# PengjieRen/CaSE_RG

Measured on AMD Instinct MI355X. Metric: train tokens/sec (query+passage) CaSE model, higher is better.
Workload: dtype bf16; 1 GPU; CaSE train step fwd+bwd+allreduce+clip+Adam+EMA, d_model=512, 6 encoder layers, 10 passages x 384 tok, query 64, answer 40, vocab 30522, per-GPU batch 32, dropout on; global_batch=32, parallelism=dp1

## Files before the change

case_rg_amd/_abi.py:

```python
import ctypes as C
import os

import torch

_HERE = os.path.dirname(os.path.abspath(__file__))
LIB_PATH = os.environ.get("CASE_HIP_LIB") or os.path.join(_HERE, "csrc", "libcase_hip.so")

ABI_VERSION = 600
F32, BF16 = 0, 1
WS_ATTENTION_SPLITKV, WS_ATTENTION_BWD, WS_OPTIM_SUMSQ, WS_ENCODER_CHAIN_PACK, WS_GEMM_DW_SLABS = 1, 2, 3, 4, 5
(FEAT_GEMM_256, FEAT_GEMM_SMALL, FEAT_ENCODER_CHAIN, FEAT_ATTN_SCORES, FEAT_ATTN_DECODE, FEAT_OPTIM, FEAT_ATTN_RESIDENT, FEAT_RESERVED_CUS,
 FEAT_GEMM_DW_SLABS, FEAT_DECODER_CHAIN, FEAT_ATTN_DECODE_MQA, FEAT_POINTER_DECODE, FEAT_POINTER_HEAD, FEAT_GEMM_LN, FEAT_STEP_STATE,
 FEAT_INTERACTION, FEAT_ATTN_DECODE_APPEND, FEAT_LINEAR_SKINNY, FEAT_BEAM_DECODE, FEAT_SAMPLE_DECODE, FEAT_POINTER_SCORE, FEAT_CONSENSUS, FEAT_NGRAM_BAN,
 FEAT_NGRAM_COUNTS, FEAT_RANK_METRICS, FEAT_POINTER_HEAD_WIDE, FEAT_DECODE_RULES, FEAT_TOKEN_LABELS) = (1 << i for i in range(28))
EPI_BIAS_COL, EPI_BIAS_ROW, EPI_GELU, EPI_RELU = 1, 2, 4, 8
EPI_RESIDUAL, EPI_MUL_DGELU, EPI_MUL_DRELU, EPI_ATOMIC, EPI_DROPOUT = 16, 32, 64, 128, 256

i32, i64, u64, f32, f64, ptr = C.c_int32, C.c_int64, C.c_uint64, C.c_float, C.c_double, C.c_void_p


class GemmDesc(C.Structure):
    _fields_ = [(n, i64) for n in ("M", "N", "K", "lda", "ldb", "ldc", "ld_aux", "batch1", "batch2",
                                   "sa1", "sa2", "sb1", "sb2", "sc1", "sc2", "saux1", "saux2")] + \
               [(n, i32) for n in ("a_kmajor", "b_kmajor", "in_dtype", "out_dtype", "epilogue", "split_k", "tile")] + \
               [("alpha", f32), ("drop_p", f32), ("seed", u64), ("offset", u64), ("state", ptr)]


class StepState(C.Structure):
    _fields_ = [("rng_base", u64), ("step_size", f32), ("bc2_sqrt", f32), ("lr", f32), ("step", i32), ("reserved", u64 * 5)]


class EncoderChainDesc(C.Structure):
    _fields_ = [("rows", i64), ("width", i32), ("variant", i32), ("eps_ln2", f32), ("eps_ln1_next", f32)]


class SoftmaxDesc(C.Structure):
    _fields_ = [("outer", i64), ("inner", i64), ("R", i64), ("C", i64), ("causal", i32), ("in_dtype", i32),
                ("out_dtype", i32), ("drop_p", f32), ("seed", u64), ("offset", u64), ("state", ptr)]


class AttnDesc(C.Structure):
    _fields_ = [(n, i64) for n in ("N", "heads", "Lq", "Lk", "head_dim", "ldq", "ldk", "ldv", "sq", "sk", "sv", "ldo", "so")] + \
               [("causal", i32), ("scale", f32), ("drop_p", f32), ("seed", u64), ("offset", u64), ("state", ptr)]


class InteractionDesc(C.Structure):
    _fields_ = [(n, i64) for n in ("n", "Lp", "Lq", "H", "eq_div")] + [("dtype", i32)]


class AttnProductDesc(C.Structure):
    _fields_ = [(n, i64) for n in ("N", "heads", "M", "Kc", "head_dim", "lda", "sa_seq", "sa_head", "ldb", "sb_seq", "sb_head",
                                   "ldc", "sc_seq", "sc_head")] + [("a_transposed", i32), ("alpha", f32)]


_RULE = [i64, i32, ptr, i32, i64, i64]

SIGNATURES = {
    "case_gemm": [C.POINTER(GemmDesc), ptr, ptr, ptr, ptr, ptr, ptr, ptr, ptr],
    "case_gemm_dw_bias": [C.POINTER(GemmDesc), ptr, ptr, ptr, ptr, ptr],
    "case_gemm_dw_slabs": [C.POINTER(GemmDesc), ptr, ptr, ptr, ptr, ptr, i64, ptr],
    "case_embed_pos_fwd": [ptr, ptr, ptr, ptr, i64, i64, i64, i64, f32, f32, u64, u64, ptr, i32, ptr],
    "case_embed_pos_bwd": [ptr, ptr, ptr, i64, i64, i64, f32, f32, u64, u64, ptr, i32, ptr],
    "case_scale_add_rows": [ptr, ptr, ptr, i64, i64, i64, f32, i32, ptr],
    "case_layernorm_fwd": [ptr, ptr, ptr, ptr, ptr, ptr, ptr, i64, i64, f32, i32, ptr],
    "case_layernorm_bwd": [ptr, ptr, ptr, ptr, ptr, ptr, ptr, ptr, ptr, ptr, i64, i64, i32, ptr],
    "case_layernorm_bwd_dropout": [ptr, ptr, ptr, ptr, ptr, ptr, ptr, ptr, ptr, i64, i64, f32, u64, u64, ptr, i32, ptr],
    "case_layernorm_bwd_concat5": [ptr] * 15 + [i64, i64, i32, ptr],
    "case_softmax_fwd": [C.POINTER(SoftmaxDesc), ptr, ptr, ptr, ptr, ptr, ptr],
    "case_softmax_bwd": [C.POINTER(SoftmaxDesc), ptr, ptr, ptr, ptr],
    "case_attention_supported": [i64],
    "case_attention_fwd": [C.POINTER(AttnDesc), ptr, ptr, ptr, ptr, ptr, ptr, ptr],
    "case_attention_splitkv_workspace": [C.POINTER(AttnDesc), i32, C.POINTER(i64)],
    "case_attention_fwd_splitkv": [C.POINTER(AttnDesc), ptr, ptr, ptr, ptr, ptr, ptr, ptr, i64, i32, ptr],
    "case_attention_bwd_supported": [i64],
    "case_attention_decode_supported": [i64],
    "case_attention_decode": [C.POINTER(AttnDesc), ptr, ptr, ptr, ptr, ptr, ptr],
    "case_attention_decode_append": [C.POINTER(AttnDesc), ptr, ptr, ptr, ptr, ptr, i64, i64, ptr, ptr, ptr],
    "case_attention_bwd": [C.POINTER(AttnDesc), ptr, ptr, ptr, ptr, ptr, ptr, ptr, ptr, ptr, ptr, ptr, ptr],
    "case_attention_scores_supported": [C.POINTER(AttnDesc)],
    "case_attention_scores_fwd": [C.POINTER(AttnDesc), ptr, ptr, ptr, ptr, ptr, ptr],
    "case_attention_scores_bwd": [C.POINTER(AttnDesc), ptr, ptr, ptr, ptr, ptr],
    "case_attention_product_supported": [C.POINTER(AttnProductDesc)],
    "case_attention_product": [C.POINTER(AttnProductDesc), ptr, ptr, ptr, ptr],
    "case_add": [ptr, ptr, ptr, i64, i32, ptr],
    "case_add_n": [C.POINTER(ptr), i32, ptr, i64, i32, ptr],
    "case_dropout": [ptr, ptr, i64, f32, u64, u64, ptr, i32, ptr],
    "case_mask_rows": [ptr, ptr, ptr, i64, i64, i32, ptr],
    "case_colsum": [ptr, ptr, i64, i64, i32, ptr],
    "case_cast": [ptr, ptr, i64, i32, i32, ptr],
    "case_scale_cols": [ptr, ptr, ptr, i64, i64, i32, ptr],
    "case_scale_cols_bwd": [ptr, ptr, ptr, ptr, ptr, i64, i64, i32, ptr],
    "case_rowdot_fwd": [ptr, ptr, ptr, ptr, i64, i64, i32, ptr],
    "case_linear_skinny": [ptr, ptr, i32, ptr, ptr, ptr, i64, i32, i32, ptr],
    "case_rowdot_bwd": [ptr, ptr, ptr, ptr, ptr, ptr, i64, i64, i32, ptr],
    "case_masked_mean_fwd": [ptr, ptr, ptr, i64, i64, i64, i32, ptr],
    "case_masked_mean_bwd": [ptr, ptr, ptr, i64, i64, i64, i32, ptr],
    "case_highway_gate_fwd": [ptr, ptr, i64, i64, i32, ptr],
    "case_highway_gate_bwd": [ptr, ptr, ptr, i64, i64, i32, ptr],
    "case_concat5_fwd": [ptr, ptr, ptr, ptr, ptr, i64, i64, i32, ptr],
    "case_concat5_bwd": [ptr, ptr, ptr, ptr, ptr, ptr, ptr, ptr, i64, i64, i32, ptr],
    "case_max_over_p_fwd": [ptr, ptr, ptr, i64, i64, i64, i32, ptr],
    "case_max_over_p_bwd": [ptr, ptr, ptr, i64, i64, i64, i32, ptr],
    "case_additive_scores_fwd": [ptr, ptr, ptr, ptr, i64, i64, i64, i64, i32, ptr],
    "case_additive_scores_bwd": [ptr, ptr, ptr, ptr, ptr, ptr, ptr, i64, i64, i64, i64, i32, ptr],
    "case_copy_scatter_fwd": [ptr, ptr, ptr, i64, i64, i64, i64, ptr],
    "case_copy_scatter_bwd": [ptr, ptr, ptr, i64, i64, i64, i64, ptr],
    "case_source_sort": [ptr, ptr, i64, i64, i64, ptr],
    "case_copy_scatter_sorted_fwd": [ptr, ptr, ptr, i64, i64, i64, i64, ptr],
    "case_nll_gather_fwd": [ptr, ptr, ptr, i64, i64, ptr],
    "case_nll_gather_bwd": [ptr, ptr, ptr, ptr, i64, i64, ptr],
    "case_row_argmax": [ptr, ptr, ptr, i64, i64, i64, ptr],
    "case_sentence_compact": [ptr, ptr, ptr, i64, i64, i64, i64, i64, ptr],
    "case_encoder_chain_pack": [ptr, ptr, ptr, ptr, ptr, ptr],
    "case_encoder_chain": [C.POINTER(EncoderChainDesc)] + [ptr] * 14,
    "case_set_reserved_cus": [i32],
    "case_attention_decode_mqa": [ptr, ptr, ptr, ptr, i64, i64, i64, i32, ptr, i64, ptr],
    "case_additive_key_exp": [ptr, ptr, i64, ptr],
    "case_pointer_attend_decode": [ptr] * 11 + [i64, i64, i64, ptr],
    "case_pointer_head_decode": [ptr] * 5 + [i32] + [ptr] * 4 + [i64, i64, i64, ptr],
    "case_pointer_head_beam": [ptr] * 5 + [i32] + [ptr] * 4 + [i64, i64, i64, i32, ptr],
    "case_pointer_head_sample": [ptr] * 5 + [i32] + [ptr] * 7 + [i64, i64, i64, f32, i32, f32, u64, u64, ptr, i64, i64, i64, i32, i32, ptr],
    "case_pointer_head_decode_wide": [ptr] * 5 + [i32] + [ptr] * 4 + [i64, i64, i64, ptr, i64, ptr, i64, i64, i32, i64, ptr],
    "case_pointer_head_beam_wide": [ptr] * 5 + [i32] + [ptr] * 4 + [i64, i64, i64, i32, ptr, i64, ptr, i64, i64, i32, i64, ptr],
    "case_pointer_head_sample_wide": [ptr] * 5 + [i32] + [ptr] * 7 + [i64, i64, i64, f32, i32, f32, u64, u64, ptr, i64, i64, i64, i32, i32,
                                      ptr, i64, ptr, i64, i64, i32, ptr],
    "case_pointer_head_score": [ptr] * 3 + [i64, ptr, ptr, i32, ptr, i64, ptr, ptr, i64, i64, i64, ptr],
    "case_beam_advance": [ptr] * 12 + [i64, i64, i64, i32, i64, ptr],
    "case_pointer_head_decode_ban": [ptr] * 5 + [i32] + [ptr] * 4 + [i64, i64, i64, ptr, i64, i64, i32, i64, ptr],
    "case_pointer_head_beam_ban": [ptr] * 5 + [i32] + [ptr] * 4 + [i64, i64, i64, i32, ptr, i64, i64, i32, i64, ptr],
    "case_pointer_head_sample_ban": [ptr] * 5 + [i32] + [ptr] * 7 + [i64, i64, i64, f32, i32, f32, u64, u64, ptr, i64, i64, i64, i32, i32,
                                     ptr, i64, i64, i32, ptr],
    "case_beam_advance_ban": [ptr] * 12 + [i64, i64, i64, i32, i64, ptr, ptr, i64, ptr],
    "case_ngram_ban": [ptr, ptr, ptr, i64, i64, i64, i64, i32, i64, ptr],
    "case_remove_duplicate_ids": [ptr, ptr, i64, i64, i32, i64, ptr],
    "case_pointer_head_decode_rules": [ptr] * 5 + [i32] + [ptr] * 4 + [i64, i64, i64, ptr, i64, i64, i32, i64] + _RULE + [ptr],
    "case_pointer_head_beam_rules": [ptr] * 5 + [i32] + [ptr] * 4 + [i64, i64, i64, i32, ptr, i64, i64, i32, i64] + _RULE + [ptr],
    "case_pointer_head_sample_rules": [ptr] * 5 + [i32] + [ptr] * 7 + [i64, i64, i64, f32, i32, f32, u64, u64, ptr, i64, i64, i64, i32, i32,
                                       ptr, i64, i64, i32] + _RULE + [ptr],
    "case_pointer_head_decode_wide_rules": [ptr] * 5 + [i32] + [ptr] * 4 + [i64, i64, i64, ptr, i64, ptr, i64, i64, i32, i64] + _RULE + [ptr],
    "case_pointer_head_beam_wide_rules": [ptr] * 5 + [i32] + [ptr] * 4 + [i64, i64, i64, i32, ptr, i64, ptr, i64, i64, i32, i64] + _RULE + [ptr],
    "case_pointer_head_sample_wide_rules": [ptr] * 5 + [i32] + [ptr] * 7 + [i64, i64, i64, f32, i32, f32, u64, u64, ptr, i64, i64, i64, i32, i32,
                                            ptr, i64, ptr, i64, i64, i32] + _RULE + [ptr],
    "case_row_rules": [ptr, ptr, i64, i64, i64] + _RULE + [ptr],
    "case_beam_advance_rules": [ptr] * 12 + [i64, i64, i64, i32, i64, ptr, ptr, i64, f32, ptr],
    "case_beam_gather": [ptr, ptr, i32, ptr, ptr, ptr, i64, i32, i64, i64, i64, ptr],
    "case_beam_backtrack": [ptr] * 8 + [i64, i32, i64, ptr],
    "case_lcs_pairs": [ptr] * 6 + [i64, i64, i64, i64, i64, ptr],
    "case_consensus_pick": [ptr] * 7 + [i64, i64, i64, ptr],
    "case_ngram_counts": [ptr] * 9 + [i64, i64, i64, i64, i64, i32, ptr],
    "case_bleu_scores": [ptr] * 7 + [i64, i64, i64, i32, i32, ptr],
    "case_rank_metrics": [ptr] * 8 + [i64, i64, i64, ptr],
    "case_token_labels": [ptr, ptr, ptr, i32, ptr, ptr, i64, i64, i64, i64, i64, i64, ptr],
    "case_token_select": [ptr] * 7 + [i64, i64, i32, ptr],
    "case_gemm_ln": [C.POINTER(GemmDesc), ptr, ptr, ptr, f32, ptr, ptr, ptr, ptr, ptr, ptr],
    "case_optim_sumsq": [ptr, ptr, i64, ptr, ptr, ptr],
    "case_optim_adam_ema": [ptr, ptr, i64, ptr, f32, f64, f64, f64, f64, ptr, ptr],
    "case_step_advance": [ptr, u64, f64, f64, ptr],
    "case_interaction_supported": [C.POINTER(InteractionDesc)],
    "case_interaction_fwd": [C.POINTER(InteractionDesc), ptr, ptr, ptr, ptr, ptr, ptr, ptr, ptr, ptr, ptr],
}


def _load():
    if not os.path.exists(LIB_PATH):
        raise ImportError(
            "case_rg_amd: %s is missing. Build it with `python -c 'import __graft_entry__ as g; g.build()'` "
            "(or `make -C case_rg_amd/csrc`). There is no CPU or eager fallback." % LIB_PATH)
    lib = C.CDLL(LIB_PATH)
    lib.case_version.restype = C.c_int
    if lib.case_version() != ABI_VERSION:
        raise ImportError("case_rg_amd: %s is ABI generation %d, this package binds %d -- rebuild it (make -C case_rg_amd/csrc)"
                          % (LIB_PATH, lib.case_version(), ABI_VERSION))
    for name, args in SIGNATURES.items():
        fn = getattr(lib, name)
        fn.argtypes = args
        fn.restype = C.c_int
    lib.case_optim_chunk_elems.restype = C.c_int
    lib.case_optim_chunk_elems.argtypes = []
    lib.case_encoder_chain_packed_bytes.restype = C.c_int64
    lib.case_encoder_chain_packed_bytes.argtypes = []
    lib.case_attention_bwd_scratch_floats.restype = C.c_int64
    lib.case_attention_bwd_scratch_floats.argtypes = [C.POINTER(AttnDesc)]
    lib.case_attention_decode_mqa_workspace.restype = C.c_int64
    lib.case_attention_decode_mqa_workspace.argtypes = [i64, i64, i32]
    lib.case_attention_decode_mqa_splits.restype = C.c_int32
    lib.case_attention_decode_mqa_splits.argtypes = [i64, i64]
    lib.case_abi_features.restype = C.c_uint32
# ... 30 lines not shown
```

case_rg_amd/csrc/api.hip:

```cpp
#include <stdarg.h>
#include <stdio.h>
#include <stdlib.h>

#include "common.h"

static thread_local char g_err[512] = "";

int case_set_error(int code, const char* fmt, ...) {
  va_list ap;
  va_start(ap, fmt);
  vsnprintf(g_err, sizeof(g_err), fmt, ap);
  va_end(ap);
  return code;
}

int case_check_launch(const char* what) {
  const hipError_t e = hipGetLastError();
  if (e == hipSuccess) return CASE_OK;
  return case_set_error(CASE_E_LAUNCH, "%s: %s", what, hipGetErrorString(e));
}

extern "C" int case_version(void) { return CASE_ABI_VERSION; }
extern "C" uint32_t case_abi_features(void) {
  return CASE_FEAT_GEMM_256 | CASE_FEAT_GEMM_SMALL | CASE_FEAT_ENCODER_CHAIN | CASE_FEAT_ATTN_SCORES | CASE_FEAT_ATTN_DECODE | CASE_FEAT_OPTIM |
         CASE_FEAT_ATTN_RESIDENT | CASE_FEAT_RESERVED_CUS | CASE_FEAT_GEMM_DW_SLABS | CASE_FEAT_ATTN_DECODE_MQA | CASE_FEAT_POINTER_DECODE | CASE_FEAT_POINTER_HEAD | CASE_FEAT_GEMM_LN | CASE_FEAT_STEP_STATE | CASE_FEAT_INTERACTION | CASE_FEAT_ATTN_DECODE_APPEND | CASE_FEAT_LINEAR_SKINNY |
         CASE_FEAT_BEAM_DECODE | CASE_FEAT_SAMPLE_DECODE | CASE_FEAT_POINTER_SCORE | CASE_FEAT_CONSENSUS | CASE_FEAT_NGRAM_BAN | CASE_FEAT_NGRAM_COUNTS | CASE_FEAT_RANK_METRICS | CASE_FEAT_POINTER_HEAD_WIDE |
         CASE_FEAT_DECODE_RULES | CASE_FEAT_TOKEN_LABELS;
}
extern "C" const char* case_last_error(void) { return g_err; }

static int g_reserved_cus = [] {
  const char* e = getenv("CASE_RESERVE_CUS");
  return e ? atoi(e) : 0;
}();
extern "C" int case_set_reserved_cus(int n) {
  if (n < 0 || n > 128) return case_set_error(CASE_E_ARG, "case_set_reserved_cus: %d out of range (0 .. 128)", n);
  g_reserved_cus = n;
  return CASE_OK;
}
extern "C" int case_get_reserved_cus(void) { return g_reserved_cus; }
int case_device_cus() {
  static int cus = 0;
  if (!cus) {
    int dev = 0, n = 0;
    (void)hipGetDevice(&dev);
    (void)hipDeviceGetAttribute(&n, hipDeviceAttributeMultiprocessorCount, dev);
    cus = n > 0 ? n : 256;
  }
  return cus;
}
int case_persistent_cus() {
  int c = case_device_cus() - g_reserved_cus;
  c = c / 8 * 8;
  return c > 8 ? c : 8;
}
extern "C" int case_sizeof_opt_tensor(void) { return (int)sizeof(CaseOptTensor); }
```

case_rg_amd/csrc/attn_pointer.hip:

```cpp
#include "common.h"

namespace {

template <bool FAST>
__device__ __forceinline__ float tanh_t(float x) {
  if constexpr (FAST) {
    const float e = __expf(2.f * x);
    return 1.f - __fdividef(2.f, e + 1.f);
  } else {
    return tanhf(x);
  }
}

constexpr float TANH_PRESCALE = 2.8853900817779268f;
constexpr float EXP2_CLAMP = 62.f;
__device__ __forceinline__ float exp2_factor(float xs) { return __builtin_amdgcn_exp2f(fminf(fmaxf(xs, -EXP2_CLAMP), EXP2_CLAMP)); }
__device__ __forceinline__ float half_sigmoid_prod(float ew, float eu) { return __builtin_amdgcn_rcpf(fmaf(ew, eu, 1.f)); }

constexpr int AJ = 64;
constexpr int AH = 64;
constexpr int ATW = 8;

template <typename T, bool FAST>
__global__ __launch_bounds__(256) void additive_fwd_kernel(const float* __restrict__ wq, const T* __restrict__ uh,
                                                           const float* __restrict__ v, float* __restrict__ s, int64_t Tn,
                                                           int64_t S, int64_t H) {
  __shared__ float U[AJ][AH + 1];
  __shared__ float W[4 * ATW][AH];
  __shared__ float V[AH];
  const int64_t b = blockIdx.y, j0 = (int64_t)blockIdx.x * AJ;
  const int lane = threadIdx.x & 63, wave = threadIdx.x >> 6;
  for (int64_t tc = (int64_t)blockIdx.z * 4 * ATW; tc < Tn; tc += (int64_t)gridDim.z * 4 * ATW) {
    constexpr float PS = FAST ? TANH_PRESCALE : 1.f;
    float acc[ATW];
#pragma unroll
    for (int i = 0; i < ATW; ++i) acc[i] = 0.f;
    float vsum = 0.f;
    for (int64_t hc = 0; hc < H; hc += AH) {
      __syncthreads();
      for (int e = threadIdx.x; e < AJ * AH; e += 256) {
        const int jj = e / AH, hh = e % AH;
        const int64_t j = j0 + jj, h = hc + hh;
        const float uv = (j < S && h < H) ? PS * Elem<T>::ld(uh + (b * S + j) * H + h) : 0.f;
        U[jj][hh] = FAST ? exp2_factor(uv) : uv;
      }
      for (int e = threadIdx.x; e < 4 * ATW * AH; e += 256) {
        const int tt = e / AH, hh = e % AH;
        const int64_t t = tc + tt, h = hc + hh;
        const float wv = (t < Tn && h < H) ? PS * wq[(b * Tn + t) * H + h] : 0.f;
        W[tt][hh] = FAST ? exp2_factor(wv) : wv;
      }
      if (threadIdx.x < AH) V[threadIdx.x] = (hc + threadIdx.x < H) ? v[hc + threadIdx.x] : 0.f;
      __syncthreads();
#pragma unroll 4
      for (int hh = 0; hh < AH; ++hh) {
        const float u = U[lane][hh], vv = V[hh];
        if constexpr (FAST) {
          vsum += vv;
#pragma unroll
          for (int i = 0; i < ATW; ++i) acc[i] += vv * half_sigmoid_prod(W[wave * ATW + i][hh], u);
        } else {
#pragma unroll
          for (int i = 0; i < ATW; ++i) acc[i] += vv * tanh_t<FAST>(W[wave * ATW + i][hh] + u);
        }
      }
    }
    const int64_t j = j0 + lane;
    if (j < S) {
#pragma unroll
      for (int i = 0; i < ATW; ++i) {
        const int64_t t = tc + wave * ATW + i;
        if (t < Tn) s[(b * Tn + t) * S + j] = FAST ? vsum - 2.f * acc[i] : acc[i];
      }
    }
  }
}

template <typename T, bool FAST, int TT, int NCH>
__global__ __launch_bounds__(256) void additive_fwd_rowwise_kernel(const float* __restrict__ wq, const T* __restrict__ uh,
                                                                   const float* __restrict__ v, float* __restrict__ s,
                                                                   int64_t Tn, int64_t S, int64_t H) {
  constexpr int E = Vec16<T>::N;
  const int64_t b = blockIdx.y;
  const int lane = threadIdx.x & 63;
  const int64_t wave = (int64_t)blockIdx.x * 4 + (threadIdx.x >> 6), nwaves = (int64_t)gridDim.x * 4;
  float wreg[NCH][TT][E], vreg[NCH][E];
#pragma unroll
  for (int c = 0; c < NCH; ++c) {
    const int64_t h0 = ((int64_t)c * 64 + lane) * E;
#pragma unroll
    for (int e = 0; e < E; ++e) {
      vreg[c][e] = h0 < H ? v[h0 + e] : 0.f;
#pragma unroll
      for (int t = 0; t < TT; ++t) wreg[c][t][e] = (h0 < H && t < Tn) ? wq[(b * Tn + t) * H + h0 + e] : 0.f;
    }
  }
  for (int64_t j = wave; j < S; j += nwaves) {
    float acc[TT];
#pragma unroll
    for (int t = 0; t < TT; ++t) acc[t] = 0.f;
#pragma unroll
    for (int c = 0; c < NCH; ++c) {
      const int64_t h0 = ((int64_t)c * 64 + lane) * E;
      if (h0 < H) {
        float u[E];
        Vec16<T>::load(uh + (b * S + j) * H + h0, u);
#pragma unroll
        for (int e = 0; e < E; ++e)
#pragma unroll
          for (int t = 0; t < TT; ++t) acc[t] += vreg[c][e] * tanh_t<FAST>(wreg[c][t][e] + u[e]);
      }
    }
#pragma unroll
    for (int t = 0; t < TT; ++t) {
      const float r = wave_sum(acc[t]);
      if (lane == 0 && t < Tn) s[(b * Tn + t) * S + j] = r;
    }
  }
}

constexpr int BJ = 16;
constexpr int BTC = 32;

template <typename T, bool FAST>
__global__ __launch_bounds__(256) void additive_bwd_uh_kernel(const float* __restrict__ ds, const float* __restrict__ wq,
                                                              const T* __restrict__ uh, const float* __restrict__ v,
                                                              float* __restrict__ d_uh, float* __restrict__ d_v, int64_t Tn,
                                                              int64_t S, int64_t H) {
  __shared__ float DS[BTC][BJ];
  const int64_t b = blockIdx.z, j0 = (int64_t)blockIdx.x * BJ, h = (int64_t)blockIdx.y * 256 + threadIdx.x;
  const bool h_ok = h < H;
  float u[BJ], acc[BJ];
#pragma unroll
  for (int jj = 0; jj < BJ; ++jj) {
    const int64_t j = j0 + jj;
    u[jj] = (h_ok && j < S) ? (FAST ? TANH_PRESCALE : 1.f) * Elem<T>::ld(uh + (b * S + j) * H + h) : 0.f;
    if constexpr (FAST) u[jj] = exp2_factor(u[jj]);
    acc[jj] = 0.f;
  }
  float dv = 0.f, gsum = 0.f;
  for (int64_t tc = 0; tc < Tn; tc += BTC) {
    __syncthreads();
    for (int e = threadIdx.x; e < BTC * BJ; e += 256) {
      const int tt = e / BJ, jj = e % BJ;
      const int64_t t = tc + tt, j = j0 + jj;
      DS[tt][jj] = (t < Tn && j < S) ? ds[(b * Tn + t) * S + j] : 0.f;
    }
    __syncthreads();
    const int tmax = (int)((Tn - tc) < BTC ? (Tn - tc) : BTC);
    for (int tt = 0; tt < tmax; ++tt) {
      float w = h_ok ? (FAST ? TANH_PRESCALE : 1.f) * wq[(b * Tn + tc + tt) * H + h] : 0.f;
      if constexpr (FAST) w = exp2_factor(w);
#pragma unroll
      for (int jj = 0; jj < BJ; ++jj) {
        const float g = DS[tt][jj];
        if constexpr (FAST) {
          const float r = half_sigmoid_prod(w, u[jj]);
          const float gr = g * r;
          acc[jj] += gr - gr * r;
          dv += gr;
          gsum += g;
        } else {
          const float th = tanh_t<FAST>(w + u[jj]);
          acc[jj] += g * (1.f - th * th);
          dv += g * th;
        }
      }
    }
  }
  if (h_ok) {
    const float vh = FAST ? 4.f * v[h] : v[h];
#pragma unroll
    for (int jj = 0; jj < BJ; ++jj) {
      const int64_t j = j0 + jj;
      if (j < S) d_uh[(b * S + j) * H + h] = vh * acc[jj];
    }
    atomicAdd(d_v + h, FAST ? gsum - 2.f * dv : dv);
  }
}

constexpr int CT = 8;
constexpr int CJC = 64;

template <typename T, bool FAST>
__global__ __launch_bounds__(256) void additive_bwd_wq_kernel(const float* __restrict__ ds, const float* __restrict__ wq,
                                                              const T* __restrict__ uh, const float* __restrict__ v,
                                                              float* __restrict__ d_wq, int64_t Tn, int64_t S, int64_t H,
                                                              int tblocks, int64_t j_per) {
  __shared__ float DS[CT][CJC];
  const int64_t b = blockIdx.z, t0 = (int64_t)(blockIdx.x % tblocks) * CT, h = (int64_t)blockIdx.y * 256 + threadIdx.x;
  const int64_t j_begin = (int64_t)(blockIdx.x / tblocks) * j_per, j_end = (j_begin + j_per < S) ? j_begin + j_per : S;
  const bool split = j_per < S;
  const bool h_ok = h < H;
  float w[CT], acc[CT];
#pragma unroll
  for (int tt = 0; tt < CT; ++tt) {
    const int64_t t = t0 + tt;
    w[tt] = (h_ok && t < Tn) ? (FAST ? TANH_PRESCALE : 1.f) * wq[(b * Tn + t) * H + h] : 0.f;
    if constexpr (FAST) w[tt] = exp2_factor(w[tt]);
    acc[tt] = 0.f;
  }
  for (int64_t jc = j_begin; jc < j_end; jc += CJC) {
    __syncthreads();
    for (int e = threadIdx.x; e < CT * CJC; e += 256) {
      const int tt = e / CJC, jj = e % CJC;
      const int64_t t = t0 + tt, j = jc + jj;
      DS[tt][jj] = (t < Tn && j < j_end) ? ds[(b * Tn + t) * S + j] : 0.f;
    }
    __syncthreads();
    const int jmax = (int)((j_end - jc) < CJC ? (j_end - jc) : CJC);
    for (int jj = 0; jj < jmax; ++jj) {
      float u = h_ok ? (FAST ? TANH_PRESCALE : 1.f) * Elem<T>::ld(uh + (b * S + jc + jj) * H + h) : 0.f;
      if constexpr (FAST) u = exp2_factor(u);
#pragma unroll
      for (int tt = 0; tt < CT; ++tt) {
        if constexpr (FAST) {
          const float r = half_sigmoid_prod(w[tt], u);
          const float gr = DS[tt][jj] * r;
          acc[tt] += gr - gr * r;
        } else {
          const float th = tanh_t<FAST>(w[tt] + u);
          acc[tt] += DS[tt][jj] * (1.f - th * th);
        }
      }
    }
  }
  if (h_ok) {
    const float vh = FAST ? 4.f * v[h] : v[h];
#pragma unroll
    for (int tt = 0; tt < CT; ++tt) {
      const int64_t t = t0 + tt;
      if (t < Tn) {
        if (split) atomicAdd(d_wq + (b * Tn + t) * H + h, vh * acc[tt]);
        else d_wq[(b * Tn + t) * H + h] = vh * acc[tt];
      }
    }
  }
}

constexpr float EXP_CLAMP = 43.f;
constexpr int PA_WAVES = 16, PA_H = 512;

__global__ __launch_bounds__(256) void additive_key_exp_kernel(const float* __restrict__ uh, bf16_t* __restrict__ eu, int64_t n8) {
  for (int64_t i = (int64_t)blockIdx.x * 256 + threadIdx.x; i < n8; i += (int64_t)gridDim.x * 256) {
    const float4 a = reinterpret_cast<const float4*>(uh)[2 * i], b = reinterpret_cast<const float4*>(uh)[2 * i + 1];
    const float x[8] = {a.x, a.y, a.z, a.w, b.x, b.y, b.z, b.w};
    float y[8];
#pragma unroll
    for (int e = 0; e < 8; ++e) y[e] = __expf(fminf(fmaxf(2.f * x[e], -EXP_CLAMP), EXP_CLAMP));
    Vec16<bf16_t>::store(eu + 8 * i, y);
  }
}

__device__ __forceinline__ float row_sum4(float r0, float r1, float r2, float r3) {
  const auto a = __builtin_amdgcn_permlane32_swap(__float_as_uint(r0), __float_as_uint(r2), false, false);
  const auto b = __builtin_amdgcn_permlane32_swap(__float_as_uint(r1), __float_as_uint(r3), false, false);
  const float A = __uint_as_float(a[0]) + __uint_as_float(a[1]);
  const float B = __uint_as_float(b[0]) + __uint_as_float(b[1]);
  const auto c = __builtin_amdgcn_permlane16_swap(__float_as_uint(A), __float_as_uint(B), false, false);
  float t = __uint_as_float(c[0]) + __uint_as_float(c[1]);
  t += __uint_as_float(__builtin_amdgcn_update_dpp(0, __float_as_uint(t), 0x128, 0xf, 0xf, false));
  t += __uint_as_float(__builtin_amdgcn_update_dpp(0, __float_as_uint(t), 0x124, 0xf, 0xf, false));
  t += __uint_as_float(__builtin_amdgcn_update_dpp(0, __float_as_uint(t), 0x122, 0xf, 0xf, false));
  t += __uint_as_float(__builtin_amdgcn_update_dpp(0, __float_as_uint(t), 0x121, 0xf, 0xf, false));
  return t;
}

#ifndef CASE_STREAM_DEFAULT_POLICY
typedef unsigned int pa_u32x4 __attribute__((ext_vector_type(4)));
__device__ __forceinline__ uint4 pa_nt_load(const void* p) {
  const pa_u32x4 v = __builtin_nontemporal_load(reinterpret_cast<const pa_u32x4*>(p));
  return make_uint4(v[0], v[1], v[2], v[3]);
}
#define PA_STREAM_LOAD(P) pa_nt_load(P)
#else
#define PA_STREAM_LOAD(P) (*reinterpret_cast<const uint4*>(P))
#endif
__global__ __launch_bounds__(64 * PA_WAVES) void pointer_attend_decode_kernel(
    const float* __restrict__ wq, const float* __restrict__ wq_add, const bf16_t* __restrict__ eu, const float* __restrict__ v, const bf16_t* __restrict__ mem,
    const uint8_t* __restrict__ col_valid, const uint8_t* __restrict__ row_valid, const float* __restrict__ prior, bf16_t* __restrict__ ctx,
    float* __restrict__ p_out, float* __restrict__ copy_out, const int64_t S) {
  extern __shared__ __attribute__((aligned(16))) float pa_smem[];
  float* sc = pa_smem;
  float* red = pa_smem + ((S + 3) & ~(int64_t)3);
  const int lane = threadIdx.x & 63, wave = threadIdx.x >> 6;
  const int64_t b = blockIdx.x;
  const uint8_t* cv = col_valid ? col_valid + b * S : nullptr;
  const bool row_ok = row_valid ? row_valid[b] != 0 : true;
  float ew[8], vv[8];
  {
    float w8[8];
    Vec16<float>::load(wq + b * PA_H + 8 * lane, *reinterpret_cast<float(*)[4]>(w8));
    Vec16<float>::load(wq + b * PA_H + 8 * lane + 4, *reinterpret_cast<float(*)[4]>(w8 + 4));
    if (wq_add) {
      float c8[8];
      Vec16<float>::load(wq_add + b * PA_H + 8 * lane, *reinterpret_cast<float(*)[4]>(c8));
      Vec16<float>::load(wq_add + b * PA_H + 8 * lane + 4, *reinterpret_cast<float(*)[4]>(c8 + 4));
#pragma unroll
      for (int e = 0; e < 8; ++e) w8[e] += c8[e];
    }
    Vec16<float>::load(v + 8 * lane, *reinterpret_cast<float(*)[4]>(vv));
    Vec16<float>::load(v + 8 * lane + 4, *reinterpret_cast<float(*)[4]>(vv + 4));
#pragma unroll
    for (int e = 0; e < 8; ++e) ew[e] = __expf(fminf(fmaxf(2.f * w8[e], -EXP_CLAMP), EXP_CLAMP));
  }
  float vs = 0.f;
#pragma unroll
  for (int e = 0; e < 8; ++e) vs += vv[e];
  vs = wave_sum(vs);
  const bf16_t* eub = eu + b * S * PA_H + 8 * lane;
  uint4 raw[4], nxt[4];
  bool ok[4], nok[4];
#define PA_LOAD(R, OK, J0)                                                     \
  _Pragma("unroll") for (int u = 0; u < 4; ++u) {                              \
    const int64_t j = (J0) + u * PA_WAVES;                                     \
    OK[u] = j < S && (!cv || cv[j]);                         \
    if (OK[u]) R[u] = PA_STREAM_LOAD(eub + j * PA_H);                          \
  }
  PA_LOAD(raw, ok, (int64_t)wave)
// ... 895 lines not shown
    __threadfence_block();
    __syncthreads();
  }
}

__global__ void nll_fwd_kernel(const float* __restrict__ dist, const int64_t* __restrict__ target,
                               float* __restrict__ per_row, int64_t rows, int64_t V) {
  for (int64_t r = (int64_t)blockIdx.x * blockDim.x + threadIdx.x; r < rows; r += (int64_t)gridDim.x * blockDim.x) {
    const int64_t y = target[r];
    per_row[r] = (y > 0 && y < V) ? -logf(dist[r * V + y] + 1e-8f) : 0.f;
  }
}

__global__ void nll_bwd_kernel(const float* __restrict__ dist, const int64_t* __restrict__ target,
                               const float* __restrict__ g_row, float* __restrict__ d_dist, int64_t rows, int64_t V) {
  for (int64_t r = (int64_t)blockIdx.x * blockDim.x + threadIdx.x; r < rows; r += (int64_t)gridDim.x * blockDim.x) {
    const int64_t y = target[r];
    if (y > 0 && y < V) d_dist[r * V + y] = -g_row[r] / (dist[r * V + y] + 1e-8f);
  }
}

__global__ __launch_bounds__(256) void row_argmax_kernel(const float* __restrict__ x, int64_t* __restrict__ idx,
                                                         float* __restrict__ val, int64_t rows, int64_t cols, int64_t ld) {
  __shared__ float sv[4];
  __shared__ int64_t si[4];
  for (int64_t r = blockIdx.x; r < rows; r += gridDim.x) {
    float best = -INFINITY;
    int64_t bi = cols;
    for (int64_t c = threadIdx.x; c < cols; c += 256) {
      const float vv = x[r * ld + c];
      if (vv > best || (vv == best && c < bi)) {
        best = vv;
        bi = c;
      }
    }
#pragma unroll
    for (int o = 32; o > 0; o >>= 1) {
      const float ob = __shfl_xor(best, o, 64);
      const int64_t oi = __shfl_xor(bi, o, 64);
      if (ob > best || (ob == best && oi < bi)) {
        best = ob;
        bi = oi;
      }
    }
    __syncthreads();
    if ((threadIdx.x & 63) == 0) {
      sv[threadIdx.x >> 6] = best;
      si[threadIdx.x >> 6] = bi;
    }
    __syncthreads();
    if (threadIdx.x == 0) {
      for (int w = 1; w < 4; ++w)
        if (sv[w] > best || (sv[w] == best && si[w] < bi)) {
          best = sv[w];
          bi = si[w];
        }
      idx[r] = bi < cols ? bi : 0;
      if (val) val[r] = best;
    }
  }
}

}

extern "C" int case_additive_scores_fwd(const float* wq, const void* uh, const float* v, float* s, int64_t B, int64_t T,
                                        int64_t S, int64_t H, int32_t dtype, case_stream_t stream) {
  CASE_REQUIRE(wq && uh && v && s && B > 0 && T > 0 && S > 0 && H > 0 && B < 65536, "case_additive_scores_fwd: bad argument");
  hipStream_t st = (hipStream_t)stream;
  const int ev = dtype == CASE_F32 ? 4 : 8;
  if (T <= 2 && H % ev == 0 && H <= 2 * 64 * ev && (uintptr_t)uh % 16 == 0) {
    const dim3 g((unsigned)((S + 15) / 16 < 64 ? (S + 15) / 16 : 64), (unsigned)B);
    const bool one = H <= 64 * ev;
#define ROWWISE(TY, FAST, TT, NCH) hipLaunchKernelGGL((additive_fwd_rowwise_kernel<TY, FAST, TT, NCH>), g, dim3(256), 0, st, wq, (const TY*)uh, v, s, T, S, H)
    if (dtype == CASE_F32) {
      if (T == 1) { if (one) ROWWISE(float, false, 1, 1); else ROWWISE(float, false, 1, 2); }
      else { if (one) ROWWISE(float, false, 2, 1); else ROWWISE(float, false, 2, 2); }
    } else {
      if (T == 1) { if (one) ROWWISE(bf16_t, true, 1, 1); else ROWWISE(bf16_t, true, 1, 2); }
      else { if (one) ROWWISE(bf16_t, true, 2, 1); else ROWWISE(bf16_t, true, 2, 2); }
    }
#undef ROWWISE
    return case_check_launch("case_additive_scores_fwd");
  }
  const int64_t jb = (S + AJ - 1) / AJ, tchunks = (T + 4 * ATW - 1) / (4 * ATW);
  const dim3 grid((unsigned)jb, (unsigned)B, (unsigned)(jb * B < 512 ? tchunks : 1));
  if (dtype == CASE_F32)
    hipLaunchKernelGGL((additive_fwd_kernel<float, false>), grid, dim3(256), 0, st, wq, (const float*)uh, v, s, T, S, H);
  else
    hipLaunchKernelGGL((additive_fwd_kernel<bf16_t, true>), grid, dim3(256), 0, st, wq, (const bf16_t*)uh, v, s, T, S, H);
  return case_check_launch("case_additive_scores_fwd");
}

extern "C" int case_additive_scores_bwd(const float* ds, const float* wq, const void* uh, const float* v, float* d_wq,
                                        float* d_uh, float* d_v, int64_t B, int64_t T, int64_t S, int64_t H, int32_t dtype,
                                        case_stream_t stream) {
  CASE_REQUIRE(ds && wq && uh && v && d_wq && d_uh && d_v && B > 0 && T > 0 && S > 0 && H > 0 && B < 65536,
               "case_additive_scores_bwd: bad argument");
  const unsigned hb = (unsigned)((H + 255) / 256);
  const int tblocks = (int)((T + CT - 1) / CT);
  const int64_t base_wgs = (int64_t)tblocks * hb * B, j_chunks = (S + CJC - 1) / CJC;
  int64_t sch = base_wgs >= 2048 ? 1 : (2048 + base_wgs - 1) / base_wgs;
  if (sch > j_chunks) sch = j_chunks;
  const int64_t j_per = ((j_chunks + sch - 1) / sch) * CJC;
  sch = (S + j_per - 1) / j_per;
  const dim3 g1((unsigned)((S + BJ - 1) / BJ), hb, (unsigned)B), g2((unsigned)(tblocks * sch), hb, (unsigned)B);
  hipStream_t st = (hipStream_t)stream;
  if (sch > 1 && hipMemsetAsync(d_wq, 0, (size_t)(B * T * H) * sizeof(float), st) != hipSuccess)
    return case_set_error(CASE_E_LAUNCH, "case_additive_scores_bwd: hipMemsetAsync failed");
  if (dtype == CASE_F32) {
    hipLaunchKernelGGL((additive_bwd_uh_kernel<float, false>), g1, dim3(256), 0, st, ds, wq, (const float*)uh, v, d_uh, d_v, T, S, H);
    hipLaunchKernelGGL((additive_bwd_wq_kernel<float, false>), g2, dim3(256), 0, st, ds, wq, (const float*)uh, v, d_wq, T, S, H, tblocks, j_per);
  } else {
    hipLaunchKernelGGL((additive_bwd_uh_kernel<bf16_t, true>), g1, dim3(256), 0, st, ds, wq, (const bf16_t*)uh, v, d_uh, d_v, T, S, H);
    hipLaunchKernelGGL((additive_bwd_wq_kernel<bf16_t, true>), g2, dim3(256), 0, st, ds, wq, (const bf16_t*)uh, v, d_wq, T, S, H, tblocks, j_per);
  }
  return case_check_launch("case_additive_scores_bwd");
}

extern "C" int case_additive_key_exp(const float* uh, void* eu, int64_t n, case_stream_t stream) {
  CASE_REQUIRE(uh && eu && n > 0 && n % 8 == 0 && (uintptr_t)uh % 16 == 0 && (uintptr_t)eu % 16 == 0, "case_additive_key_exp: bad argument");
  hipLaunchKernelGGL(additive_key_exp_kernel, dim3(grid_for(n / 8, 256, 1, 256 * 32)), dim3(256), 0, (hipStream_t)stream, uh,
                     reinterpret_cast<bf16_t*>(eu), n / 8);
  return case_check_launch("case_additive_key_exp");
}

extern "C" int case_pointer_attend_decode(const float* wq, const float* wq_add, const void* eu, const float* v, const void* value, const uint8_t* col_valid,
                                          const uint8_t* row_valid, const float* prior, void* ctx, float* p, float* copy, int64_t B, int64_t S,
                                          int64_t H, case_stream_t stream) {
  CASE_REQUIRE(wq && eu && v && value && ctx && p && B > 0 && S > 0 && B < (1ll << 31) && (copy != nullptr) == (prior != nullptr),
               "case_pointer_attend_decode: bad argument");
  if (H != PA_H || S > 28000)
    return case_set_error(CASE_E_UNSUPPORTED, "case_pointer_attend_decode: built for H = %d and S <= 28000 (run case_additive_scores_fwd + "
                                              "case_softmax_fwd + case_gemm)", PA_H);
  for (const void* q : {(const void*)wq, (const void*)wq_add, eu, (const void*)v, value})
    CASE_REQUIRE((reinterpret_cast<uintptr_t>(q) & 15) == 0, "case_pointer_attend_decode: tensors must be 16-byte aligned");
  const size_t lds = (size_t)(((S + 3) & ~(int64_t)3) + PA_WAVES * PA_H) * sizeof(float);
  static bool attr = false;
  if (!attr) {
    if (hipFuncSetAttribute(reinterpret_cast<const void*>(&pointer_attend_decode_kernel), hipFuncAttributeMaxDynamicSharedMemorySize, 160 * 1024) !=
        hipSuccess)
      return case_set_error(CASE_E_LAUNCH, "case_pointer_attend_decode: cannot reserve LDS");
    attr = true;
  }
  hipLaunchKernelGGL(pointer_attend_decode_kernel, dim3((unsigned)B), dim3(64 * PA_WAVES), lds, (hipStream_t)stream, wq, wq_add,
                     reinterpret_cast<const bf16_t*>(eu), v, reinterpret_cast<const bf16_t*>(value), col_valid, row_valid, prior,
                     reinterpret_cast<bf16_t*>(ctx), p, copy, S);
  return case_check_launch("case_pointer_attend_decode");
}

template <typename Args>
static int pointer_head_fill(Args& a, const char* who, const float* logits, const float* mix_logits, const uint32_t* keys, const float* const* copies,
                             const int64_t* lens, int32_t nmem, int64_t R, int64_t V, int64_t S, int64_t max_v, const char* instead) {
  CASE_REQUIRE(logits && mix_logits && keys && copies && lens && R > 0 && V > 0 && S > 0 && nmem >= 1 && R < (1ll << 31), "%s: bad argument", who);
  if (nmem > PH_MAX_MEM || V > max_v || S > 32768)
    return case_set_error(CASE_E_UNSUPPORTED, "%s: built for <= %d memories, V <= %lld, S <= 32768%s", who, PH_MAX_MEM, (long long)max_v, instead);
  a.logits = logits;
  a.mix_logits = mix_logits;
  a.keys = keys;
  int64_t total = 0;
  for (int m = 0; m < PH_MAX_MEM; ++m) {
    a.copy[m] = m < nmem ? copies[m] : nullptr;
    a.len[m] = m < nmem ? lens[m] : 0;
    total += a.len[m];
    CASE_REQUIRE(m >= nmem || (copies[m] && lens[m] > 0), "%s: null copy weights", who);
  }
  CASE_REQUIRE(total == S, "%s: the memories hold %lld positions, the source map %lld", who, (long long)total, (long long)S);
  a.V = V;
  a.S = S;
  a.nmem = nmem;
  return CASE_OK;
}

constexpr int64_t PH_MAX_V = 36000, PS_MAX_V = 131071;
constexpr int64_t PW_MAX_DIST_V = 1ll << 24;

static int pointer_head_args(HeadArgs& a, const char* who, const float* logits, const float* mix_logits, const uint32_t* keys,
                             const float* const* copies, const int64_t* lens, int32_t nmem, float* gen, float* dist, int64_t B, int64_t V, int64_t S,
                             bool wide = false) {
  const int rc = pointer_head_fill(a, who, logits, mix_logits, keys, copies, lens, nmem, B, V, S, wide ? PS_MAX_V : PH_MAX_V,
                                   wide ? "" : " (run the softmax / scatter / argmax launches)");
  if (rc != CASE_OK) return rc;
  a.gen = gen;
  a.dist = dist;
  a.ids = nullptr;
  a.top = nullptr;
  a.row_ws = nullptr;
  a.row_stride = 0;
  return CASE_OK;
}

static size_t pointer_head_lds(int64_t V) { return (size_t)(((V + 3) & ~(int64_t)3) + (PH_THREADS + 4) + PH_THREADS + 64) * 4; }

static int pointer_head_workspace(HeadArgs& a, const char* who, float* row_ws, int64_t row_stride, int64_t V) {
  CASE_REQUIRE(row_ws && row_stride >= V && row_stride % 4 == 0 && (reinterpret_cast<uintptr_t>(row_ws) & 15) == 0,
               "%s: the row workspace must be 16-byte aligned f32 [rows, row_stride], row_stride >= V and a multiple of 4", who);
  a.row_ws = row_ws;
  a.row_stride = row_stride;
  return CASE_OK;
}
// ... 550 lines not shown
```

case_rg_amd/csrc/common.h:

```cpp
#pragma once
#include <hip/hip_runtime.h>
#include <stdint.h>

#include "case_hip.h"

typedef unsigned short bf16_t;

int case_set_error(int code, const char* fmt, ...);
int case_check_launch(const char* what);
int case_device_cus();
int case_persistent_cus();

#define CASE_REQUIRE(cond, ...)                          \
  do {                                                   \
    if (!(cond)) return case_set_error(CASE_E_ARG, __VA_ARGS__); \
  } while (0)

__device__ __forceinline__ float bf16_to_f32(bf16_t v) { return __uint_as_float(((uint32_t)v) << 16); }
typedef float case_f32x2 __attribute__((ext_vector_type(2)));
typedef __bf16 case_bf16x2 __attribute__((ext_vector_type(2)));
__device__ __forceinline__ uint32_t f32x2_to_bf16x2(float lo, float hi) {
  const case_f32x2 v = {lo, hi};
  const case_bf16x2 b = __builtin_convertvector(v, case_bf16x2);
  return *reinterpret_cast<const uint32_t*>(&b);
// ... 25 lines not shown
    *reinterpret_cast<float4*>(p) = make_float4(v[0], v[1], v[2], v[3]);
  }
};
template <> struct Vec16<bf16_t> {
  static constexpr int N = 8;
  typedef uint4 raw;
  static __device__ __forceinline__ void unpack(const uint4& t, float (&v)[8]) {
    const uint32_t w[4] = {t.x, t.y, t.z, t.w};
#pragma unroll
    for (int i = 0; i < 4; ++i) {
      v[2 * i] = __uint_as_float(w[i] << 16);
      v[2 * i + 1] = __uint_as_float(w[i] & 0xffff0000u);
    }
  }
#ifdef CASE_VEC16_NT
  static __device__ __forceinline__ void load(const bf16_t* p, float (&v)[8]) {
    typedef unsigned int u32x4_nt __attribute__((ext_vector_type(4)));
    const u32x4_nt t = __builtin_nontemporal_load(reinterpret_cast<const u32x4_nt*>(p));
    unpack(make_uint4(t[0], t[1], t[2], t[3]), v);
  }
#else
  static __device__ __forceinline__ void load(const bf16_t* p, float (&v)[8]) { unpack(*reinterpret_cast<const uint4*>(p), v); }
#endif
  static __device__ __forceinline__ void store(bf16_t* p, const float (&v)[8]) {
    uint32_t w[4];
#pragma unroll
    for (int i = 0; i < 4; ++i) w[i] = f32x2_to_bf16x2(v[2 * i], v[2 * i + 1]);
    *reinterpret_cast<uint4*>(p) = make_uint4(w[0], w[1], w[2], w[3]);
  }
};

template <typename T> struct Vec8;
template <> struct Vec8<bf16_t> {
  static constexpr int N = 4;
  typedef uint2 raw;
  static __device__ __forceinline__ void unpack(const uint2& t, float (&v)[4]) {
    v[0] = __uint_as_float(t.x << 16); v[1] = __uint_as_float(t.x & 0xffff0000u);
    v[2] = __uint_as_float(t.y << 16); v[3] = __uint_as_float(t.y & 0xffff0000u);
  }
  static __device__ __forceinline__ void load(const bf16_t* p, float (&v)[4]) { unpack(*reinterpret_cast<const uint2*>(p), v); }
  static __device__ __forceinline__ void store(bf16_t* p, const float (&v)[4]) {
    *reinterpret_cast<uint2*>(p) = make_uint2(f32x2_to_bf16x2(v[0], v[1]), f32x2_to_bf16x2(v[2], v[3]));
  }
};

__device__ __forceinline__ float wave_sum(float v) {
#pragma unroll
  for (int o = 32; o > 0; o >>= 1) v += __shfl_xor(v, o, 64);
  return v;
}
__device__ __forceinline__ float wave_max(float v) {
#pragma unroll
  for (int o = 32; o > 0; o >>= 1) v = fmaxf(v, __shfl_xor(v, o, 64));
  return v;
}

__device__ __forceinline__ float block_sum(float v, float* red) {
  const int lane = threadIdx.x & 63, w = threadIdx.x >> 6, nw = (blockDim.x + 63) >> 6;
  v = wave_sum(v);
  __syncthreads();
  if (lane == 0) red[w] = v;
  __syncthreads();
  float t = (lane < nw) ? red[lane] : 0.f;
  t = wave_sum(t);
  return t;
}
__device__ __forceinline__ float block_max(float v, float* red) {
  const int lane = threadIdx.x & 63, w = threadIdx.x >> 6, nw = (blockDim.x + 63) >> 6;
  v = wave_max(v);
  __syncthreads();
  if (lane == 0) red[w] = v;
  __syncthreads();
  float t = (lane < nw) ? red[lane] : -INFINITY;
  t = wave_max(t);
  return t;
}

__device__ __forceinline__ uint64_t rng_base_of(const CaseStepState* st) {
  if (st == nullptr) return 0;
  typedef const __attribute__((address_space(4))) uint64_t* const_u64_ptr;
  return *(const_u64_ptr)(uintptr_t)st;
}

__device__ __forceinline__ uint32_t rng_hash(uint64_t seed, uint64_t pair) {
  const uint32_t lo = (uint32_t)pair, hi = (uint32_t)(pair >> 32);
  uint32_t h = lo ^ ((hi << 16) | (hi >> 16)) ^ (uint32_t)seed;
  h *= 0x9E3779B1u;
  h ^= (h >> 15) ^ (uint32_t)(seed >> 32);
  h *= 0x85EBCA77u;
  h ^= h >> 13;
  return h;
}
__device__ __forceinline__ float rng_uniform(uint64_t seed, uint64_t idx) {
  const uint32_t h = rng_hash(seed, idx >> 1);
  return (float)((idx & 1) ? (h >> 16) : (h & 0xffffu)) * (1.0f / 65536.0f);
}
__device__ __forceinline__ void rng_uniform2(uint64_t seed, uint64_t idx_even, float& u0, float& u1) {
  const uint32_t h = rng_hash(seed, idx_even >> 1);
  u0 = (float)(h & 0xffffu) * (1.0f / 65536.0f);
  u1 = (float)(h >> 16) * (1.0f / 65536.0f);
}
__device__ __forceinline__ float rng_uniform24(uint64_t seed, uint64_t counter) {
  return (float)(rng_hash(seed, counter) >> 8) * (1.0f / 16777216.0f);
}
__device__ __forceinline__ void dropout8(float (&x)[8], uint64_t seed, uint64_t idx0, float p, float scale) {
  if ((idx0 & 1) == 0) {
#pragma unroll
    for (int e = 0; e < 8; e += 2) {
      float u0, u1;
      rng_uniform2(seed, idx0 + e, u0, u1);
      x[e] = u0 >= p ? x[e] * scale : 0.f;
      x[e + 1] = u1 >= p ? x[e + 1] * scale : 0.f;
    }
  } else {
#pragma unroll
    for (int e = 0; e < 8; ++e) x[e] = rng_uniform(seed, idx0 + e) >= p ? x[e] * scale : 0.f;
  }
}

constexpr uint32_t RNG_C1 = 0x9E3779B1u, RNG_C2 = 0x85EBCA77u;
__device__ __forceinline__ uint32_t rng_row_key(uint64_t seed, uint64_t offset_plus_row) { return rng_hash(seed, offset_plus_row); }
__device__ __forceinline__ uint32_t rng_pair_bits_pre(uint32_t key, uint32_t jc1) {
  const uint32_t h = (key ^ jc1) * RNG_C2;
  return h ^ (h >> 16);
}
__device__ __forceinline__ uint32_t rng_pair_bits(uint32_t key, uint32_t pair) { return rng_pair_bits_pre(key, pair * RNG_C1); }
__device__ __forceinline__ uint32_t rng_threshold(float p) { return (uint32_t)ceilf(p * 65536.f); }
__device__ __forceinline__ bool attn_keep(uint32_t key, uint32_t col, uint32_t thr) {
  const uint32_t h = rng_pair_bits(key, col >> 1);
  return ((col & 1) ? (h >> 16) : (h & 0xffffu)) >= thr;
}
__device__ __forceinline__ void attn_dropout8(float (&x)[8], uint32_t key, uint32_t c0, uint32_t thr, float scale) {
#pragma unroll
  for (int e = 0; e < 8; e += 2) {
    const uint32_t h = rng_pair_bits(key, (c0 + e) >> 1);
    x[e] = (h & 0xffffu) >= thr ? x[e] * scale : 0.f;
    x[e + 1] = (h >> 16) >= thr ? x[e + 1] * scale : 0.f;
  }
}

struct GeluTerms {
  float cdf, pdf;
};
__device__ __forceinline__ GeluTerms gelu_terms(float x) {
  const float z = fabsf(x) * 0.70710678118654752f;
  const float t = __builtin_amdgcn_rcpf(fmaf(0.3275911f, z, 1.f));
  const float e = __expf(-z * z);
  float p = fmaf(1.061405429f, t, -1.453152027f);
  p = fmaf(p, t, 1.421413741f);
  p = fmaf(p, t, -0.284496736f);
  p = fmaf(p, t, 0.254829592f);
  const float q = 0.5f * p * t * e;
  GeluTerms r;
  r.cdf = x >= 0.f ? 1.f - q : q;
  r.pdf = 0.39894228040143268f * e;
  return r;
}
__device__ __forceinline__ float gelu_f(float x) { return x * gelu_terms(x).cdf; }
__device__ __forceinline__ float dgelu_f(float x) {
  const GeluTerms g = gelu_terms(x);
  return g.cdf + x * g.pdf;
}

static inline int grid_for(int64_t n, int block, int per_thread = 1, int cap = 256 * 8) {
  int64_t g = (n + (int64_t)block * per_thread - 1) / ((int64_t)block * per_thread);
  if (g < 1) g = 1;
  if (g > cap) g = cap;
  return (int)g;
}
```

case_rg_amd/csrc/elementwise.hip:

```cpp
#include "common.h"

namespace {

constexpr int EW_THREADS = 256;

template <typename T>
__global__ void add_kernel(const T* __restrict__ a, const T* __restrict__ b, T* __restrict__ o, int64_t n) {
  for (int64_t i = (int64_t)blockIdx.x * blockDim.x + threadIdx.x; i < n; i += (int64_t)gridDim.x * blockDim.x)
    Elem<T>::st(o + i, Elem<T>::ld(a + i) + Elem<T>::ld(b + i));
}

template <typename T>
__global__ void dropout_kernel(const T* __restrict__ x, T* __restrict__ y, int64_t n, float p, uint64_t seed,
                               uint64_t offset, const CaseStepState* state) {
  offset += rng_base_of(state);
  const float scale = 1.f / (1.f - p);
  for (int64_t i = (int64_t)blockIdx.x * blockDim.x + threadIdx.x; i < n; i += (int64_t)gridDim.x * blockDim.x)
    Elem<T>::st(y + i, rng_uniform(seed, offset + (uint64_t)i) >= p ? Elem<T>::ld(x + i) * scale : 0.f);
}

template <typename T>
__global__ void mask_rows_kernel(const T* __restrict__ x, const uint8_t* __restrict__ valid, T* __restrict__ y,
                                 int64_t rows, int64_t cols) {
  const int64_t n = rows * cols;
  const bool in_place = x == y;
  for (int64_t i = (int64_t)blockIdx.x * blockDim.x + threadIdx.x; i < n; i += (int64_t)gridDim.x * blockDim.x) {
    const bool ok = valid[i / cols] != 0;
    if (in_place) {
      if (!ok) Elem<T>::st(y + i, 0.f);
    } else {
      Elem<T>::st(y + i, ok ? Elem<T>::ld(x + i) : 0.f);
    }
  }
}

template <typename T>
__global__ __launch_bounds__(256) void colsum_kernel(const T* __restrict__ x, float* __restrict__ out, int64_t rows,
                                                     int64_t cols, int row_splits) {
  __shared__ float part[4][64];
  const int cx = threadIdx.x & 63, ry = threadIdx.x >> 6;
  const int64_t col = (int64_t)(blockIdx.x / row_splits) * 64 + cx;
  const int split = blockIdx.x % row_splits;
  float s = 0.f;
  if (col < cols)
    for (int64_t r = (int64_t)split * 4 + ry; r < rows; r += (int64_t)row_splits * 4) s += Elem<T>::ld(x + r * cols + col);
  part[ry][cx] = s;
  __syncthreads();
  if (ry == 0 && col < cols) atomicAdd(out + col, part[0][cx] + part[1][cx] + part[2][cx] + part[3][cx]);
}

template <typename T>
__global__ __launch_bounds__(256) void colsum_vec_kernel(const T* __restrict__ x, float* __restrict__ out, int64_t rows,
                                                         int64_t cols, int row_splits) {
  constexpr int E = Vec16<T>::N;
  __shared__ float part[8][32 * E + 1];
  const int cx = threadIdx.x & 31, ry = threadIdx.x >> 5;
  const int64_t col = ((int64_t)(blockIdx.x / row_splits) * 32 + cx) * E;
  const int split = blockIdx.x % row_splits;
  float s[E];
#pragma unroll
  for (int e = 0; e < E; ++e) s[e] = 0.f;
  if (col < cols)
    for (int64_t r = (int64_t)split * 8 + ry; r < rows; r += (int64_t)row_splits * 8) {
      float v[E];
      Vec16<T>::load(x + r * cols + col, v);
#pragma unroll
      for (int e = 0; e < E; ++e) s[e] += v[e];
    }
#pragma unroll
  for (int e = 0; e < E; ++e) part[ry][cx * E + e] = s[e];
  __syncthreads();
  for (int c = threadIdx.x; c < 32 * E; c += 256) {
    const int64_t gc = (int64_t)(blockIdx.x / row_splits) * 32 * E + c;
    if (gc < cols) {
      float t = 0.f;
#pragma unroll
      for (int r = 0; r < 8; ++r) t += part[r][c];
      atomicAdd(out + gc, t);
    }
  }
}

template <typename T>
__global__ void add_vec_kernel(const T* __restrict__ a, const T* __restrict__ b, T* __restrict__ o, int64_t nvec) {
  constexpr int E = Vec16<T>::N;
  for (int64_t i = (int64_t)blockIdx.x * blockDim.x + threadIdx.x; i < nvec; i += (int64_t)gridDim.x * blockDim.x) {
    float x[E], y[E];
    Vec16<T>::load(a + i * E, x);
    Vec16<T>::load(b + i * E, y);
#pragma unroll
    for (int e = 0; e < E; ++e) x[e] += y[e];
    Vec16<T>::store(o + i * E, x);
  }
}

struct AddNArgs {
  const void* src[8];
  int n;
};
template <typename T>
__global__ void add_n_vec_kernel(const AddNArgs a, T* __restrict__ o, int64_t nvec) {
  constexpr int E = Vec16<T>::N;
  for (int64_t i = (int64_t)blockIdx.x * blockDim.x + threadIdx.x; i < nvec; i += (int64_t)gridDim.x * blockDim.x) {
    float acc[E], y[E];
    Vec16<T>::load(reinterpret_cast<const T*>(a.src[0]) + i * E, acc);
#pragma unroll
    for (int j = 1; j < 8; ++j) {
      if (j < a.n) {
        Vec16<T>::load(reinterpret_cast<const T*>(a.src[j]) + i * E, y);
#pragma unroll
        for (int e = 0; e < E; ++e) acc[e] += y[e];
      }
    }
    Vec16<T>::store(o + i * E, acc);
  }
}

template <typename T>
__global__ void dropout_vec_kernel(const T* __restrict__ x, T* __restrict__ y, int64_t nvec, float p, uint64_t seed,
                                   uint64_t offset, const CaseStepState* state) {
  offset += rng_base_of(state);
  constexpr int E = Vec16<T>::N;
  const float scale = 1.f / (1.f - p);
  for (int64_t i = (int64_t)blockIdx.x * blockDim.x + threadIdx.x; i < nvec; i += (int64_t)gridDim.x * blockDim.x) {
    float v[E];
    Vec16<T>::load(x + i * E, v);
    const uint64_t idx0 = offset + (uint64_t)(i * E);
    if ((idx0 & 1) == 0) {
#pragma unroll
      for (int e = 0; e < E; e += 2) {
        float u0, u1;
        rng_uniform2(seed, idx0 + e, u0, u1);
        v[e] = u0 >= p ? v[e] * scale : 0.f;
        v[e + 1] = u1 >= p ? v[e + 1] * scale : 0.f;
      }
    } else {
#pragma unroll
      for (int e = 0; e < E; ++e) v[e] = rng_uniform(seed, idx0 + e) >= p ? v[e] * scale : 0.f;
    }
    Vec16<T>::store(y + i * E, v);
  }
}

template <typename T>
__global__ void mask_rows_vec_kernel(const T* __restrict__ x, const uint8_t* __restrict__ valid, T* __restrict__ y,
                                     int64_t rows, int64_t cols) {
  constexpr int E = Vec16<T>::N;
  const int64_t vpr = cols / E, nvec = rows * vpr;
  const bool in_place = x == y;
  for (int64_t i = (int64_t)blockIdx.x * blockDim.x + threadIdx.x; i < nvec; i += (int64_t)gridDim.x * blockDim.x) {
    const bool ok = valid[i / vpr] != 0;
    if (in_place && ok) continue;
    float v[E];
    if (ok) Vec16<T>::load(x + i * E, v);
    else {
#pragma unroll
      for (int e = 0; e < E; ++e) v[e] = 0.f;
    }
    Vec16<T>::store(y + i * E, v);
  }
}

template <typename T>
__global__ __launch_bounds__(256) void rowdot_fwd_kernel(const T* __restrict__ x, const float* __restrict__ w,
                                                         const float* __restrict__ b, float* __restrict__ y, int64_t rows,
                                                         int64_t cols) {
  const int lane = threadIdx.x & 63;
  const int64_t wave = (int64_t)blockIdx.x * 4 + (threadIdx.x >> 6), nwaves = (int64_t)gridDim.x * 4;
  for (int64_t r = wave; r < rows; r += nwaves) {
    float acc = 0.f;
    for (int64_t c = lane; c < cols; c += 64) acc += Elem<T>::ld(x + r * cols + c) * w[c];
    acc = wave_sum(acc);
    if (lane == 0) y[r] = acc + (b ? b[0] : 0.f);
  }
}

struct SkinnyArgs {
  const void* x[4];
  int64_t width[4];
  const float* w; const float* b; float* y;
  int64_t rows, cols;
  int nseg, nout;
};
template <typename T, bool VEC>
__global__ __launch_bounds__(256) void linear_skinny_kernel(const SkinnyArgs a) {
  const int lane = threadIdx.x & 63;
  const int64_t wave = (int64_t)blockIdx.x * 4 + (threadIdx.x >> 6), nwaves = (int64_t)gridDim.x * 4;
  constexpr int NV = Vec16<T>::N;
  for (int64_t r = wave; r < a.rows; r += nwaves) {
    float acc[8] = {0.f, 0.f, 0.f, 0.f, 0.f, 0.f, 0.f, 0.f};
    int64_t off = 0;
#pragma unroll
    for (int k = 0; k < 4; ++k) {
      if (k < a.nseg) {
        const T* xr = reinterpret_cast<const T*>(a.x[k]) + r * a.width[k];
        if constexpr (VEC) {
#pragma unroll 2
          for (int64_t c = (int64_t)lane * NV; c < a.width[k]; c += 64 * NV) {
            float xv[NV];
            Vec16<T>::load(xr + c, xv);
#pragma unroll
            for (int o = 0; o < 8; ++o) {
              if (o < a.nout) {
                const float* wr = a.w + o * a.cols + off + c;
#pragma unroll
                for (int q = 0; q < NV / 4; ++q) {
                  const float4 wv = *reinterpret_cast<const float4*>(wr + 4 * q);
                  acc[o] = fmaf(xv[4 * q], wv.x, acc[o]);
                  acc[o] = fmaf(xv[4 * q + 1], wv.y, acc[o]);
                  acc[o] = fmaf(xv[4 * q + 2], wv.z, acc[o]);
                  acc[o] = fmaf(xv[4 * q + 3], wv.w, acc[o]);
                }
              }
            }
          }
        } else {
          for (int64_t c = lane; c < a.width[k]; c += 64) {
            const float xv = Elem<T>::ld(xr + c);
#pragma unroll
            for (int o = 0; o < 8; ++o)
              if (o < a.nout) acc[o] = fmaf(xv, a.w[o * a.cols + off + c], acc[o]);
// ... 24 lines not shown
  float s = 0.f, sb = 0.f;
  if (col < cols) {
    const float wc = w[col];
    for (int64_t r = (int64_t)split * 4 + ry; r < rows; r += (int64_t)row_splits * 4) {
      const float gr = g[r];
      s += gr * Elem<T>::ld(x + r * cols + col);
      sb += gr;
      if (dx) Elem<T>::st(dx + r * cols + col, gr * wc);
    }
  }
  part[ry][cx] = s;
  __syncthreads();
  if (ry == 0 && col < cols) atomicAdd(dw + col, part[0][cx] + part[1][cx] + part[2][cx] + part[3][cx]);
  if (db && col == 0) {
    __syncthreads();
    part[ry][0] = sb;
    __syncthreads();
    if (ry == 0 && cx == 0) atomicAdd(db, part[0][0] + part[1][0] + part[2][0] + part[3][0]);
  }
}

static inline bool al16(const void* p) { return ((uintptr_t)p % 16) == 0; }

template <typename TS, typename TD>
__global__ void cast_kernel(const TS* __restrict__ x, TD* __restrict__ y, int64_t n) {
  for (int64_t i = (int64_t)blockIdx.x * blockDim.x + threadIdx.x; i < n; i += (int64_t)gridDim.x * blockDim.x)
    Elem<TD>::st(y + i, Elem<TS>::ld(x + i));
}

template <typename T>
__global__ void scale_cols_kernel(const T* __restrict__ x, const float* __restrict__ w, T* __restrict__ y, int64_t rows,
                                  int64_t cols) {
  const int64_t n = rows * cols;
  for (int64_t i = (int64_t)blockIdx.x * blockDim.x + threadIdx.x; i < n; i += (int64_t)gridDim.x * blockDim.x)
    Elem<T>::st(y + i, Elem<T>::ld(x + i) * w[i % cols]);
}

template <typename T>
__global__ __launch_bounds__(256) void scale_cols_bwd_kernel(const T* __restrict__ dy, const T* __restrict__ x,
                                                             const float* __restrict__ w, T* __restrict__ dx,
                                                             float* __restrict__ dw, int64_t rows, int64_t cols,
                                                             int row_splits) {
  __shared__ float part[4][64];
  const int cx = threadIdx.x & 63, ry = threadIdx.x >> 6;
  const int64_t col = (int64_t)(blockIdx.x / row_splits) * 64 + cx;
  const int split = blockIdx.x % row_splits;
  float s = 0.f;
  if (col < cols) {
    const float wc = w[col];
    for (int64_t r = (int64_t)split * 4 + ry; r < rows; r += (int64_t)row_splits * 4) {
      const float g = Elem<T>::ld(dy + r * cols + col);
      s += g * Elem<T>::ld(x + r * cols + col);
      Elem<T>::st(dx + r * cols + col, g * wc);
    }
  }
  part[ry][cx] = s;
  __syncthreads();
  if (ry == 0 && col < cols) atomicAdd(dw + col, part[0][cx] + part[1][cx] + part[2][cx] + part[3][cx]);
}

template <typename T>
__global__ void scale_add_rows_kernel(const T* __restrict__ x, const float* __restrict__ pe, T* __restrict__ y,
                                      int64_t rows, int64_t seq_len, int64_t H, float scale) {
  const int64_t n = rows * H;
  for (int64_t i = (int64_t)blockIdx.x * blockDim.x + threadIdx.x; i < n; i += (int64_t)gridDim.x * blockDim.x) {
    const int64_t r = i / H, c = i % H;
    Elem<T>::st(y + i, Elem<T>::ld(x + i) * scale + (pe ? pe[(r % seq_len) * H + c] : 0.f));
  }
}

template <typename T>
__global__ void embed_pos_fwd_kernel(const int64_t* __restrict__ ids, const float* __restrict__ table,
                                     const float* __restrict__ pe, T* __restrict__ out, int64_t rows, int64_t seq_len,
                                     int64_t H, int64_t vocab, float scale, float drop_p, uint64_t seed, uint64_t offset,
                                     const CaseStepState* state) {
  offset += rng_base_of(state);
  const int64_t n = rows * H;
  const float ks = drop_p > 0.f ? 1.f / (1.f - drop_p) : 1.f;
  for (int64_t i = (int64_t)blockIdx.x * blockDim.x + threadIdx.x; i < n; i += (int64_t)gridDim.x * blockDim.x) {
    const int64_t r = i / H, c = i % H;
    int64_t id = ids[r];
    if (id < 0 || id >= vocab) id = 0;
    float v = table[id * H + c] * scale + pe[(r % seq_len) * H + c];
    if (drop_p > 0.f) v = rng_uniform(seed, offset + (uint64_t)i) >= drop_p ? v * ks : 0.f;
    Elem<T>::st(out + i, v);
  }
}

template <typename T>
__global__ __launch_bounds__(256) void embed_pos_fwd_vec_kernel(const int64_t* __restrict__ ids, const float* __restrict__ table,
                                                                const float* __restrict__ pe, T* __restrict__ out, unsigned chunks,
                                                                unsigned seq_len, unsigned H8, int64_t vocab, float scale, float drop_p,
                                                                uint64_t seed, uint64_t offset, const CaseStepState* state) {
  offset += rng_base_of(state);
  const float ks = drop_p > 0.f ? 1.f / (1.f - drop_p) : 1.f;
  for (unsigned ci = blockIdx.x * 256u + threadIdx.x; ci < chunks; ci += gridDim.x * 256u) {
    const unsigned r = ci / H8, c = (ci - r * H8) * 8u;
    int64_t id = ids[r];
    if (id < 0 || id >= vocab) id = 0;
    const float* tp = table + id * (int64_t)(H8 * 8u) + c;
    const float* pp = pe + (int64_t)(r % seq_len) * (H8 * 8u) + c;
    const float4 t0 = *reinterpret_cast<const float4*>(tp), t1 = *reinterpret_cast<const float4*>(tp + 4);
    const float4 p0 = *reinterpret_cast<const float4*>(pp), p1 = *reinterpret_cast<const float4*>(pp + 4);
    float v[8] = {fmaf(t0.x, scale, p0.x), fmaf(t0.y, scale, p0.y), fmaf(t0.z, scale, p0.z), fmaf(t0.w, scale, p0.w),
                  fmaf(t1.x, scale, p1.x), fmaf(t1.y, scale, p1.y), fmaf(t1.z, scale, p1.z), fmaf(t1.w, scale, p1.w)};
    if (drop_p > 0.f) dropout8(v, seed, offset + (uint64_t)r * (H8 * 8u) + c, drop_p, ks);
    T* op = out + (int64_t)r * (H8 * 8u) + c;
    if constexpr (sizeof(T) == 2) {
      uint4 w;
      w.x = f32x2_to_bf16x2(v[0], v[1]); w.y = f32x2_to_bf16x2(v[2], v[3]);
      w.z = f32x2_to_bf16x2(v[4], v[5]); w.w = f32x2_to_bf16x2(v[6], v[7]);
      *reinterpret_cast<uint4*>(op) = w;
    } else {
      *reinterpret_cast<float4*>(op) = make_float4(v[0], v[1], v[2], v[3]);
      *reinterpret_cast<float4*>(op + 4) = make_float4(v[4], v[5], v[6], v[7]);
    }
  }
}

template <typename T>
__global__ void embed_pos_bwd_kernel(const int64_t* __restrict__ ids, const T* __restrict__ d_out,
                                     float* __restrict__ d_table, int64_t rows, int64_t H, int64_t vocab, float scale,
                                     float drop_p, uint64_t seed, uint64_t offset, const CaseStepState* state) {
  offset += rng_base_of(state);
  const int64_t n = rows * H;
  const float ks = drop_p > 0.f ? 1.f / (1.f - drop_p) : 1.f;
  for (int64_t i = (int64_t)blockIdx.x * blockDim.x + threadIdx.x; i < n; i += (int64_t)gridDim.x * blockDim.x) {
    const int64_t r = i / H, c = i % H;
    const int64_t id = ids[r];
    if (id <= 0 || id >= vocab) continue;
    float g = Elem<T>::ld(d_out + i);
    if (drop_p > 0.f) g = rng_uniform(seed, offset + (uint64_t)i) >= drop_p ? g * ks : 0.f;
    atomicAdd(d_table + id * H + c, g * scale);
  }
}

template <typename T>
__global__ void masked_mean_fwd_kernel(const T* __restrict__ x, const uint8_t* __restrict__ valid, T* __restrict__ out,
                                       int64_t n, int64_t L, int64_t H) {
  const int64_t total = n * H;
  for (int64_t i = (int64_t)blockIdx.x * blockDim.x + threadIdx.x; i < total; i += (int64_t)gridDim.x * blockDim.x) {
    const int64_t s = i / H, c = i % H;
    float acc = 0.f, cnt = 0.f;
    for (int64_t l = 0; l < L; ++l)
      if (valid[s * L + l]) {
        acc += Elem<T>::ld(x + (s * L + l) * H + c);
        cnt += 1.f;
      }
    Elem<T>::st(out + i, acc / cnt);
  }
}

template <typename T>
__global__ void masked_mean_bwd_kernel(const T* __restrict__ d_out, const uint8_t* __restrict__ valid,
                                       T* __restrict__ dx, int64_t n, int64_t L, int64_t H) {
  const int64_t total = n * L * H;
  for (int64_t i = (int64_t)blockIdx.x * blockDim.x + threadIdx.x; i < total; i += (int64_t)gridDim.x * blockDim.x) {
    const int64_t c = i % H, sl = i / H, s = sl / L;
    float cnt = 0.f;
    for (int64_t l = 0; l < L; ++l) cnt += valid[s * L + l] ? 1.f : 0.f;
    Elem<T>::st(dx + i, valid[sl] ? Elem<T>::ld(d_out + s * H + c) / cnt : 0.f);
  }
}

template <typename T>
__global__ __launch_bounds__(256) void masked_mean_fwd_vec_kernel(const T* __restrict__ x, const uint8_t* __restrict__ valid,
                                                                  T* __restrict__ out, int64_t L, int64_t H) {
  constexpr int E = Vec16<T>::N;
  __shared__ float part[4][64][E + 1];
  __shared__ float cnts[4];
  const int lane = threadIdx.x & 63, w = threadIdx.x >> 6;
  const int64_t s = blockIdx.x, c0 = ((int64_t)blockIdx.y * 64 + lane) * E;
  const bool in = c0 < H;
  float acc[E];
#pragma unroll
  for (int e = 0; e < E; ++e) acc[e] = 0.f;
  float cnt = 0.f;
  for (int64_t l = w; l < L; l += 4) {
    if (!valid[s * L + l]) continue;
    cnt += 1.f;
    if (in) {
      float v[E];
      Vec16<T>::load(x + (s * L + l) * H + c0, v);
#pragma unroll
      for (int e = 0; e < E; ++e) acc[e] += v[e];
    }
  }
#pragma unroll
  for (int e = 0; e < E; ++e) part[w][lane][e] = acc[e];
  if (lane == 0) cnts[w] = cnt;
  __syncthreads();
  if (w == 0 && in) {
    const float n = cnts[0] + cnts[1] + cnts[2] + cnts[3];
    float v[E];
#pragma unroll
    for (int e = 0; e < E; ++e) v[e] = (part[0][lane][e] + part[1][lane][e] + part[2][lane][e] + part[3][lane][e]) / n;
    Vec16<T>::store(out + s * H + c0, v);
  }
}

template <typename T>
__global__ __launch_bounds__(256) void masked_mean_bwd_vec_kernel(const T* __restrict__ d_out, const uint8_t* __restrict__ valid,
                                                                  T* __restrict__ dx, int64_t L, int64_t H) {
  constexpr int E = Vec16<T>::N;
  __shared__ float red[32];
  const int lane = threadIdx.x & 63, w = threadIdx.x >> 6;
  const int64_t s = blockIdx.x, c0 = ((int64_t)blockIdx.y * 64 + lane) * E;
  float cnt = 0.f;
  for (int64_t l = threadIdx.x; l < L; l += 256) cnt += valid[s * L + l] ? 1.f : 0.f;
  cnt = block_sum(cnt, red);
  if (c0 >= H) return;
  float g[E], z[E];
  Vec16<T>::load(d_out + s * H + c0, g);
#pragma unroll
  for (int e = 0; e < E; ++e) { g[e] /= cnt; z[e] = 0.f; }
// ... 437 lines not shown
```

case_rg_amd/csrc/gemm8w.inc:

```
namespace gemm_t8w {

using gemm_w4::Epilogue;

constexpr int TM = 256, TN = 256, BKE = 64, NTHR = 512;
constexpr int OPB = 32768, STAGE = 2 * OPB, EXTRA = 32768, LDS_BYTES = 2 * STAGE + EXTRA;
constexpr int STRIP = 8192;

#pragma clang diagnostic push
#pragma clang diagnostic ignored "-Winline-asm"
typedef __attribute__((ext_vector_type(4))) int i32x4;
__device__ __forceinline__ void dma16(i32x4 rsrc, unsigned voff, unsigned soff, unsigned lds_addr) {
  asm volatile("s_mov_b32 m0, %0\n\ts_nop 0\n\tbuffer_load_dwordx4 %1, %2, %3 offen lds" ::"s"(lds_addr), "v"(voff), "s"(rsrc),
               "s"(soff)
               : "memory", "m0");
}
#pragma clang diagnostic pop
__device__ __forceinline__ i32x4 make_rsrc(const void* p) {
  i32x4 r;
  r[0] = __builtin_amdgcn_readfirstlane((int)(size_t)p);
  r[1] = __builtin_amdgcn_readfirstlane((int)(((size_t)p) >> 32) & 0xffff);
  r[2] = -1;
  r[3] = 0x00020000;
  return r;
}
// ... 26 lines not shown
      v1 = (unsigned)(r1 * ld * 2 + (((l & 7) ^ ((r1 >> 1) & 7)) * 16));
    } else {
      const int j = l >> 3, f = ((j >> 1) & 1) + 2 * (wave & 1);
      v0 = (unsigned)((wave * 8 + j) * ld * 2 + (((l & 7) ^ (2 * f)) * 16));
      v1 = v0 + 128;
    }
  }
  static __device__ __forceinline__ unsigned half_goff(int64_t ld) { return KMAJOR ? 256u : (unsigned)(128 * ld * 2); }
  static __device__ __forceinline__ unsigned kt_goff(int64_t ld) { return KMAJOR ? (unsigned)(64 * ld * 2) : 128u; }
  static __device__ __forceinline__ unsigned piece0(unsigned wv) { return KMAJOR ? wv * 1024 : wv * 2048; }
  static __device__ __forceinline__ unsigned piece1(unsigned wv) { return KMAJOR ? 8192 + wv * 1024 : wv * 2048 + 1024; }
  static __device__ __forceinline__ const char* origin(const bf16_t* op, int64_t ld, int64_t mn0, int64_t k0) {
    return reinterpret_cast<const char*>(KMAJOR ? op + k0 * ld + mn0 : op + mn0 * ld + k0);
  }

  int base[KMAJOR ? 4 : 2];
  __device__ __forceinline__ void init(int l) {
    if constexpr (!KMAJOR) {
      const int r = l & 15, s = r >> 1;
      base[0] = r * 128 + ((((l >> 4) + 0) ^ s) * 16);
      base[1] = r * 128 + ((((l >> 4) + 4) ^ s) * 16);
    } else {
      const int g = l >> 4, q = (l & 15) >> 2, t = l & 3, f = (q >> 1) + 2 * (g & 1);
#pragma unroll
      for (int x = 0; x < 4; ++x) base[x] = g * 1024 + q * 128 + (((x ^ f) * 2 + (t >> 1)) * 16) + (t & 1) * 8;
    }
  }
  __device__ __forceinline__ bf16x8 frag_at(const char* img, int lane_base, int c, int kh) const {
    if constexpr (!KMAJOR) {
      return *reinterpret_cast<const bf16x8*>(img + c * 2048 + base[kh]);
    } else {
      typedef __attribute__((address_space(3))) s16x4 lds_s16x4;
      const char* p = img + kh * 4096 + lane_base;
      const s16x4 lo = __builtin_amdgcn_ds_read_tr16_b64_v4i16((lds_s16x4*)(p));
      const s16x4 hi = __builtin_amdgcn_ds_read_tr16_b64_v4i16((lds_s16x4*)(p + 512));
      bf16x8 r;
      r[0] = lo[0]; r[1] = lo[1]; r[2] = lo[2]; r[3] = lo[3];
      r[4] = hi[0]; r[5] = hi[1]; r[6] = hi[2]; r[7] = hi[3];
      return r;
    }
  }
  __device__ __forceinline__ int lane_base_of(bool upper, int i) const {
    if constexpr (!KMAJOR) return 0;
    else return upper ? base[2 + i] : base[i];
  }
  __device__ __forceinline__ bf16x8 frag(const char* img, int c, int kh) const {
    if constexpr (!KMAJOR) {
      return *reinterpret_cast<const bf16x8*>(img + c * 2048 + base[kh]);
    } else {
      typedef __attribute__((address_space(3))) s16x4 lds_s16x4;
      const char* p = img + ((c >> 2) & 1) * 8192 + kh * 4096 + base[c & 3];
      const s16x4 lo = __builtin_amdgcn_ds_read_tr16_b64_v4i16((lds_s16x4*)(p));
      const s16x4 hi = __builtin_amdgcn_ds_read_tr16_b64_v4i16((lds_s16x4*)(p + 512));
      bf16x8 r;
      r[0] = lo[0]; r[1] = lo[1]; r[2] = lo[2]; r[3] = lo[3];
      r[4] = hi[0]; r[5] = hi[1]; r[6] = hi[2]; r[7] = hi[3];
      return r;
    }
  }
};


struct Tile {
  int64_t m0, n0;
  int kt_begin, kt_end, split;
};

#define G8_FENCE() { asm volatile("" ::: "memory"); __builtin_amdgcn_sched_barrier(0); }
#define G8_BARRIER() { G8_FENCE() __builtin_amdgcn_s_barrier(); G8_FENCE() }

#ifndef CASE_STREAM_DEFAULT_POLICY
#define G8_AUX_POLICY 2
#else
#define G8_AUX_POLICY 0
#endif
template <int ECT, typename OutT>
__device__ __forceinline__ void drain_pass(const Args& g, const int epi_rt, const float* strip, const int le, const int p,
                                           const int64_t row_w, const int64_t col_w, const float (&bc)[8], const u32x4 (&ax)[4],
                                           const __amdgpu_buffer_rsrc_t rc, const __amdgpu_buffer_rsrc_t ro) {
  const int E = ECT >= 0 ? ECT : epi_rt;
  const int cc = (le & 7) * 8;
  const bool need_aux = E & (CASE_EPI_RESIDUAL | CASE_EPI_MUL_DGELU | CASE_EPI_MUL_DRELU);
  const float drop_scale = (E & CASE_EPI_DROPOUT) ? 1.f / (1.f - g.drop_p) : 1.f;
  const int vc = (int)(((le >> 3) * g.ldc + cc) * (int64_t)sizeof(OutT));
  const int va = (int)(((le >> 3) * g.ld_aux + cc) * 2);
  float v[4][8];
#pragma unroll
  for (int s = 0; s < 4; ++s) {
    const int rr = s * 8 + (le >> 3);
    const int s0 = ((le & 7) * 2) ^ (rr & 15), s1 = ((le & 7) * 2 + 1) ^ (rr & 15);
    const f32x4 lo = *reinterpret_cast<const f32x4*>(strip + rr * 64 + s0 * 4);
    const f32x4 hi = *reinterpret_cast<const f32x4*>(strip + rr * 64 + s1 * 4);
    v[s][0] = lo[0]; v[s][1] = lo[1]; v[s][2] = lo[2]; v[s][3] = lo[3];
    v[s][4] = hi[0]; v[s][5] = hi[1]; v[s][6] = hi[2]; v[s][7] = hi[3];
  }
#pragma unroll
  for (int s = 0; s < 4; ++s) {
    const int rb = p * 32 + s * 8;
    const int64_t row = row_w + rb + (le >> 3);
    float* x = v[s];
    float a8[8];
    if (need_aux) {
#pragma unroll
      for (int i = 0; i < 4; ++i) {
        a8[2 * i] = __uint_as_float(ax[s][i] << 16);
        a8[2 * i + 1] = __uint_as_float(ax[s][i] & 0xffff0000u);
      }
    }
    const float br = (E & CASE_EPI_BIAS_ROW) ? g.bias_row[row] : 0.f;
#pragma unroll
    for (int e = 0; e < 8; ++e) x[e] = g.alpha * x[e] + ((E & CASE_EPI_BIAS_COL) ? bc[e] : 0.f) + br;
    if (E & CASE_EPI_GELU) {
      if (g.aux_out) {
        u32x4 w;
#pragma unroll
        for (int i = 0; i < 4; ++i) w[i] = f32x2_to_bf16x2(x[2 * i], x[2 * i + 1]);
        __builtin_amdgcn_raw_buffer_store_b128(w, ro, va + (int)(rb * g.ld_aux * 2), 0, G8_AUX_POLICY);
      }
#pragma unroll
      for (int e = 0; e < 8; ++e) x[e] = gelu_f(x[e]);
    }
    if (E & CASE_EPI_RELU) {
#pragma unroll
      for (int e = 0; e < 8; ++e) x[e] = fmaxf(x[e], 0.f);
    }
    if (E & CASE_EPI_MUL_DGELU) {
#pragma unroll
      for (int e = 0; e < 8; ++e) x[e] *= dgelu_f(a8[e]);
    }
    if (E & CASE_EPI_MUL_DRELU) {
#pragma unroll
      for (int e = 0; e < 8; ++e) x[e] = a8[e] > 0.f ? x[e] : 0.f;
    }
    if (E & CASE_EPI_DROPOUT) {
      const uint64_t idx0 = g.offset + rng_base_of(g.state) + (uint64_t)(row * g.N + col_w + cc);
      dropout8(v[s], g.seed, idx0, g.drop_p, drop_scale);
    }
    if (E & CASE_EPI_RESIDUAL) {
#pragma unroll
      for (int e = 0; e < 8; ++e) x[e] += a8[e];
    }
    const int sc = (int)(rb * g.ldc * (int64_t)sizeof(OutT));
    if constexpr (sizeof(OutT) == 2) {
      u32x4 w;
#pragma unroll
      for (int i = 0; i < 4; ++i) w[i] = f32x2_to_bf16x2(x[2 * i], x[2 * i + 1]);
      __builtin_amdgcn_raw_buffer_store_b128(w, rc, vc + sc, 0, 0);
    } else {
      u32x4 w0, w1;
#pragma unroll
      for (int i = 0; i < 4; ++i) { w0[i] = __float_as_uint(x[i]); w1[i] = __float_as_uint(x[4 + i]); }
      __builtin_amdgcn_raw_buffer_store_b128(w0, rc, vc + sc, 0, 0);
      __builtin_amdgcn_raw_buffer_store_b128(w1, rc, vc + sc + 16, 0, 0);
    }
  }
}

template <int ECT, typename OutT>
__device__ __forceinline__ void epilogue_tile(const Args& g, const int epi_rt, float* strip, const int le, const int64_t row_w,
                                              const int64_t col_w, const f32x4 (&acc)[8][4], void* const cbase) {
  const int E = ECT >= 0 ? ECT : epi_rt;
  const bool need_aux = E & (CASE_EPI_RESIDUAL | CASE_EPI_MUL_DGELU | CASE_EPI_MUL_DRELU);
  float bc[8] = {0.f, 0.f, 0.f, 0.f, 0.f, 0.f, 0.f, 0.f};
  if (E & CASE_EPI_BIAS_COL) Epilogue<bf16_t, OutT>::load8(g.bias_col + col_w + (le & 7) * 8, bc);
  const __amdgpu_buffer_rsrc_t rc =
      __builtin_amdgcn_make_buffer_rsrc(uniform_ptr(reinterpret_cast<OutT*>(cbase) + row_w * g.ldc + col_w), 0, -1, 0x00020000);
  const bf16_t* auxp = g.aux ? (const bf16_t*)uniform_ptr(reinterpret_cast<const bf16_t*>(g.aux) + row_w * g.ld_aux + col_w) : nullptr;
  bf16_t* auxo = g.aux_out ? (bf16_t*)uniform_ptr(reinterpret_cast<bf16_t*>(g.aux_out) + row_w * g.ld_aux + col_w) : nullptr;
  const __amdgpu_buffer_rsrc_t ra = __builtin_amdgcn_make_buffer_rsrc((void*)auxp, 0, auxp ? -1 : 0, 0x00020000);
  const __amdgpu_buffer_rsrc_t ro = __builtin_amdgcn_make_buffer_rsrc((void*)auxo, 0, auxo ? -1 : 0, 0x00020000);
  const int va = (int)(((le >> 3) * g.ld_aux + (le & 7) * 8) * 2);
  const int lr = le & 15, lg = le >> 4;
#pragma unroll
  for (int p = 0; p < 4; ++p) {
    u32x4 ax[4];
    if (need_aux) {
#pragma unroll
      for (int s = 0; s < 4; ++s) ax[s] = __builtin_amdgcn_raw_buffer_load_b128(ra, va + (int)((p * 32 + s * 8) * g.ld_aux * 2), 0, G8_AUX_POLICY);
    }
#pragma unroll
    for (int ii = 0; ii < 2; ++ii)
#pragma unroll
      for (int j = 0; j < 4; ++j)
        *reinterpret_cast<f32x4*>(strip + (ii * 16 + lr) * 64 + (((j * 4 + lg) ^ lr) * 4)) = acc[2 * p + ii][j];
    asm volatile("" ::: "memory");
    __builtin_amdgcn_sched_barrier(0);
    drain_pass<ECT, OutT>(g, epi_rt, strip, le, p, row_w, col_w, bc, ax, rc, ro);
    asm volatile("" ::: "memory");
    __builtin_amdgcn_sched_barrier(0);
  }
}

template <int ECT, typename OutT>
__device__ __forceinline__ void epilogue_regs(const Args& g, const int epi_rt, const int le, const int64_t row_w, const int64_t col_w,
                                              const f32x4 (&acc)[8][4], void* const cbase) {
  const int E = ECT >= 0 ? ECT : epi_rt;
  const bool need_aux = E & (CASE_EPI_RESIDUAL | CASE_EPI_MUL_DGELU | CASE_EPI_MUL_DRELU);
  const float drop_scale = (E & CASE_EPI_DROPOUT) ? 1.f / (1.f - g.drop_p) : 1.f;
  const int lr = le & 15, lg = le >> 4;
  const int c0 = ((lg & 1) << 4) | ((lg >> 1) << 3);
  float bc[2][8];
#pragma unroll
  for (int p = 0; p < 2; ++p) {
    if (E & CASE_EPI_BIAS_COL) Epilogue<bf16_t, OutT>::load8(g.bias_col + col_w + c0 + 32 * p, bc[p]);
    else {
#pragma unroll
      for (int e = 0; e < 8; ++e) bc[p][e] = 0.f;
    }
  }
  const __amdgpu_buffer_rsrc_t rc =
      __builtin_amdgcn_make_buffer_rsrc(uniform_ptr(reinterpret_cast<OutT*>(cbase) + row_w * g.ldc + col_w), 0, -1, 0x00020000);
  const bf16_t* auxp = g.aux ? (const bf16_t*)uniform_ptr(reinterpret_cast<const bf16_t*>(g.aux) + row_w * g.ld_aux + col_w) : nullptr;
  bf16_t* auxo = g.aux_out ? (bf16_t*)uniform_ptr(reinterpret_cast<bf16_t*>(g.aux_out) + row_w * g.ld_aux + col_w) : nullptr;
  const __amdgpu_buffer_rsrc_t ra = __builtin_amdgcn_make_buffer_rsrc((void*)auxp, 0, auxp ? -1 : 0, 0x00020000);
  const __amdgpu_buffer_rsrc_t ro = __builtin_amdgcn_make_buffer_rsrc((void*)auxo, 0, auxo ? -1 : 0, 0x00020000);
  const int vc = (int)((lr * g.ldc + c0) * (int64_t)sizeof(OutT));
  const int va = (int)((lr * g.ld_aux + c0) * 2);
  u32x4 ax[4];
#define G8_AUX_LOAD(DST, IB)                                                                                          \
  _Pragma("unroll") for (int q = 0; q < 4; ++q)                                                                       \
    DST[q] = __builtin_amdgcn_raw_buffer_load_b128(ra, va + (int)((((IB) + (q >> 1)) * 16 * g.ld_aux + 32 * (q & 1)) * 2), 0, 0);
#pragma unroll
  for (int ib = 0; ib < 8; ib += 2) {
    if (need_aux) { G8_AUX_LOAD(ax, ib) }
#pragma unroll
    for (int q = 0; q < 4; ++q) {
      const int i = ib + (q >> 1), p = q & 1;
      float x[8];
#pragma unroll
      for (int e = 0; e < 4; ++e) {
        const auto sw = __builtin_amdgcn_permlane16_swap(__float_as_uint(acc[i][2 * p][e]), __float_as_uint(acc[i][2 * p + 1][e]), false, false);
        x[e] = __uint_as_float(sw[0]);
        x[4 + e] = __uint_as_float(sw[1]);
      }
      const int64_t row = row_w + 16 * i + lr;
      const int cc = c0 + 32 * p;
      float a8[8];
      if (need_aux) {
#pragma unroll
        for (int t = 0; t < 4; ++t) {
          a8[2 * t] = __uint_as_float(ax[q][t] << 16);
          a8[2 * t + 1] = __uint_as_float(ax[q][t] & 0xffff0000u);
        }
      }
      const float br = (E & CASE_EPI_BIAS_ROW) ? g.bias_row[row] : 0.f;
#pragma unroll
      for (int e = 0; e < 8; ++e) x[e] = g.alpha * x[e] + ((E & CASE_EPI_BIAS_COL) ? bc[p][e] : 0.f) + br;
      const int so = (int)((16 * i * g.ld_aux + 32 * p) * 2);
      if (E & CASE_EPI_GELU) {
        if (g.aux_out) {
          u32x4 w;
#pragma unroll
          for (int t = 0; t < 4; ++t) w[t] = f32x2_to_bf16x2(x[2 * t], x[2 * t + 1]);
          __builtin_amdgcn_raw_buffer_store_b128(w, ro, va + so, 0, 0);
        }
#pragma unroll
        for (int e = 0; e < 8; ++e) x[e] = gelu_f(x[e]);
      }
      if (E & CASE_EPI_RELU) {
#pragma unroll
        for (int e = 0; e < 8; ++e) x[e] = fmaxf(x[e], 0.f);
      }
      if (E & CASE_EPI_MUL_DGELU) {
#pragma unroll
        for (int e = 0; e < 8; ++e) x[e] *= dgelu_f(a8[e]);
      }
      if (E & CASE_EPI_MUL_DRELU) {
#pragma unroll
        for (int e = 0; e < 8; ++e) x[e] = a8[e] > 0.f ? x[e] : 0.f;
      }
      if (E & CASE_EPI_DROPOUT) {
        const uint64_t idx0 = g.offset + rng_base_of(g.state) + (uint64_t)(row * g.N + col_w + cc);
        dropout8(x, g.seed, idx0, g.drop_p, drop_scale);
      }
      if (E & CASE_EPI_RESIDUAL) {
#pragma unroll
        for (int e = 0; e < 8; ++e) x[e] += a8[e];
      }
      const int sc = (int)((16 * i * g.ldc + 32 * p) * (int64_t)sizeof(OutT));
      if constexpr (sizeof(OutT) == 2) {
        u32x4 w;
#pragma unroll
        for (int t = 0; t < 4; ++t) w[t] = f32x2_to_bf16x2(x[2 * t], x[2 * t + 1]);
        __builtin_amdgcn_raw_buffer_store_b128(w, rc, vc + sc, 0, 0);
      } else {
        u32x4 w0, w1;
#pragma unroll
        for (int t = 0; t < 4; ++t) { w0[t] = __float_as_uint(x[t]); w1[t] = __float_as_uint(x[4 + t]); }
        __builtin_amdgcn_raw_buffer_store_b128(w0, rc, vc + sc, 0, 0);
        __builtin_amdgcn_raw_buffer_store_b128(w1, rc, vc + sc + 16, 0, 0);
      }
    }
  }
#undef G8_AUX_LOAD
}

#ifdef G8_CLOCK_STAMPS
__device__ unsigned long long g_clock_stamps[4];
#endif
template <typename OutT, bool AK, bool BK_, int ATOMIC>
__global__ __launch_bounds__(NTHR, 2) void gemm8w_kernel(const Args g, const int epi, const int tiles_m, const int tiles_n,
                                                         const int ntiles) {
  extern __shared__ __attribute__((aligned(16))) char smem[];
  const int tid = threadIdx.x, l = tid & 63, wave = tid >> 6, wr = wave >> 2, wc = wave & 3;
  const unsigned lds0 = (unsigned)(size_t)(__attribute__((address_space(3))) char*)smem;
  const unsigned wv = __builtin_amdgcn_readfirstlane(wave);

  const int xcd = blockIdx.x & 7, idx = blockIdx.x >> 3;
  const int nwx = ((int)gridDim.x - xcd + 7) >> 3;
  const int q = ntiles >> 3, r = ntiles & 7;
  const int first = xcd < r ? xcd * (q + 1) : r * (q + 1) + (xcd - r) * q, count = q + (xcd < r ? 1 : 0);
  if (idx >= count) return;
#ifdef G8_CLOCK_STAMPS
  if (blockIdx.x == 0 && tid == 0) {
    g_clock_stamps[0] = __builtin_amdgcn_s_memtime();
    g_clock_stamps[1] = __builtin_amdgcn_s_memrealtime();
  }
#endif

  const int kt_total = (int)(g.K / BKE);
  auto decode = [&](int pid) {
    Tile t;
    const int per_slab = tiles_m * tiles_n;
    const int in_slab = pid % per_slab, split = pid / per_slab;
    constexpr int GM = 4;
    const int group = in_slab / (GM * tiles_n), first_m = group * GM, gm = min(GM, tiles_m - first_m);
    const int tm = first_m + (in_slab - group * GM * tiles_n) % gm, tn = (in_slab - group * GM * tiles_n) / gm;
    t.m0 = (int64_t)tm * TM;
    t.n0 = (int64_t)tn * TN;
    t.split = split;
    t.kt_begin = split * g.k_tiles_per_split;
    t.kt_end = min(t.kt_begin + g.k_tiles_per_split, kt_total);
    return t;
  };

  unsigned va0, va1, vb0, vb1;
  Op<AK>::dma_voff(wave, l, g.lda, va0, va1);
  Op<BK_>::dma_voff(wave, l, g.ldb, vb0, vb1);
  const unsigned hga = Op<AK>::half_goff(g.lda), hgb = Op<BK_>::half_goff(g.ldb);
  const unsigned kga = Op<AK>::kt_goff(g.lda), kgb = Op<BK_>::kt_goff(g.ldb);
  const unsigned pa0 = Op<AK>::piece0(wv), pa1 = Op<AK>::piece1(wv), pb0 = Op<BK_>::piece0(wv), pb1 = Op<BK_>::piece1(wv);
  const bf16_t* Ag = reinterpret_cast<const bf16_t*>(g.A);
  const bf16_t* Bg = reinterpret_cast<const bf16_t*>(g.B);
  Op<AK> fa;
  Op<BK_> fb;
  fa.init(l);
  fb.init(l);

#ifdef G8_TIMING_ONLY_L2_RESIDENT
#define G8_KT(KT) ((KT) & 7)
#else
#define G8_KT(KT) (KT)
#endif
#define ISSUE_A(S, H, KT)                                                       \
  {                                                                             \
    const unsigned sb = lds0 + (S) * STAGE + (H) * 16384;                       \
// ... 293 lines not shown
```

case_rg_amd/csrc/gemm_impl.inc:

```
namespace GEMM_NS {

constexpr int BM = 128, BN = 128, NTHREADS = GEMM_NTHREADS;
constexpr int CHUNKS = 1024 / NTHREADS;
constexpr int MI = 512 / NTHREADS;
constexpr int MIN_WAVES = NTHREADS / 128;
constexpr int ROWB = 128;
constexpr int RM_STRIDE = ROWB + 16;
constexpr int OP_BYTES = 20480;
constexpr int STAGE_BYTES = 2 * OP_BYTES;

template <typename T> struct KM;
template <> struct KM<bf16_t> { static constexpr int row_stride = 256 + 64; };
template <> struct KM<float> { static constexpr int row_stride = 512 + 16; };


template <typename T, bool VEC>
__device__ __forceinline__ u32x4 load_chunk(const T* __restrict__ base, int64_t ld, int64_t lead, int64_t lead_max,
                                            int64_t c0, int64_t c_max, bool& ok) {
  constexpr int EPT = 16 / sizeof(T);
  ok = lead < lead_max && c0 < c_max;
  if constexpr (VEC) {
    return *reinterpret_cast<const u32x4*>(base + (ok ? lead * ld + c0 : 0));
  } else {
    T tmp[EPT];
// ... 166 lines not shown
#pragma unroll
        for (int i = 0; i < MI; ++i)
#pragma unroll
          for (int j = 0; j < 2; ++j)
            acc[i][j] = __builtin_amdgcn_mfma_f32_32x32x2f32(a[i][e], b[j][e], acc[i][j], 0, 0, 0);
    }
  }
}

template <typename T, bool AK, bool BK_, bool VEC, bool FULL>
__device__ __forceinline__ void k_loop(f32x16 (&acc)[MI][2], char* smem, const T* __restrict__ A, const T* __restrict__ B,
                                       const Args& g, int64_t m0, int64_t n0, int kt_begin, int kt_end, int wr, int wc) {
  constexpr int BKE = ROWB / sizeof(T);
  u32x4 ra0[CHUNKS], rb0[CHUNKS], ra1[CHUNKS], rb1[CHUNKS];
  unsigned oka0, okb0, oka1 = 0, okb1 = 0;
  Loader<T, AK> lda_;
  Loader<T, BK_> ldb_;
  if constexpr (VEC) {
    lda_.init(A, g.lda, m0, g.M, (int64_t)kt_begin * BKE);
    ldb_.init(B, g.ldb, n0, g.N, (int64_t)kt_begin * BKE);
  }
#define LOAD_A(R, KT) (VEC ? lda_.template load<FULL>(R, (int64_t)(KT) * BKE, g.K) : stage_load<T, AK, false>(R, A, g.lda, m0, g.M, (int64_t)(KT) * BKE, g.K))
#define LOAD_B(R, KT) (VEC ? ldb_.template load<FULL>(R, (int64_t)(KT) * BKE, g.K) : stage_load<T, BK_, false>(R, B, g.ldb, n0, g.N, (int64_t)(KT) * BKE, g.K))
  oka0 = LOAD_A(ra0, kt_begin);
  okb0 = LOAD_B(rb0, kt_begin);
  stage_store<T, AK, FULL>(ra0, oka0, smem);
  stage_store<T, BK_, FULL>(rb0, okb0, smem + OP_BYTES);
  if (kt_begin + 1 < kt_end) {
    oka0 = LOAD_A(ra0, kt_begin + 1);
    okb0 = LOAD_B(rb0, kt_begin + 1);
  }
  __syncthreads();
  int cur = 0;
#define GEMM_STEP(KT, FARC, NEXTC, WAITN, RA_NEXT, RB_NEXT, OKA_NEXT, OKB_NEXT, RA_FAR, RB_FAR, OKA_FAR, OKB_FAR)  \
  {                                                                                                                \
    if (FARC) {                                                                                                    \
      OKA_FAR = LOAD_A(RA_FAR, (KT) + 2);                                                                          \
      OKB_FAR = LOAD_B(RB_FAR, (KT) + 2);                                                                          \
    }                                                                                                              \
    const char* la = smem + cur * STAGE_BYTES;                                                                     \
    mma_tile<T, AK, BK_>(acc, la, la + OP_BYTES, wr, wc);                                                          \
    if (NEXTC) {                                                                                                   \
      char* nx = smem + (cur ^ 1) * STAGE_BYTES;                                                                   \
      stage_store<T, AK, FULL>(RA_NEXT, OKA_NEXT, nx);                                                             \
      stage_store<T, BK_, FULL>(RB_NEXT, OKB_NEXT, nx + OP_BYTES);                                                 \
    }                                                                                                              \
    __syncthreads();                                                                                               \
    cur ^= 1;                                                                                                      \
  }
  int kt = kt_begin;
  for (; kt + 3 < kt_end; kt += 2) {
    GEMM_STEP(kt, true, true, 8, ra0, rb0, oka0, okb0, ra1, rb1, oka1, okb1)
    GEMM_STEP(kt + 1, true, true, 8, ra1, rb1, oka1, okb1, ra0, rb0, oka0, okb0)
  }
  const int left = kt_end - kt;
  if (left == 3) {
    GEMM_STEP(kt, true, true, 8, ra0, rb0, oka0, okb0, ra1, rb1, oka1, okb1)
    GEMM_STEP(kt + 1, false, true, 0, ra1, rb1, oka1, okb1, ra0, rb0, oka0, okb0)
    GEMM_STEP(kt + 2, false, false, 0, ra0, rb0, oka0, okb0, ra1, rb1, oka1, okb1)
  } else if (left == 2) {
    GEMM_STEP(kt, false, true, 0, ra0, rb0, oka0, okb0, ra1, rb1, oka1, okb1)
    GEMM_STEP(kt + 1, false, false, 0, ra1, rb1, oka1, okb1, ra0, rb0, oka0, okb0)
  } else if (left == 1) {
    GEMM_STEP(kt, false, false, 0, ra0, rb0, oka0, okb0, ra1, rb1, oka1, okb1)
  }
#undef GEMM_STEP
#undef LOAD_A
#undef LOAD_B
}

constexpr int CT_STRIDE = 132;
static_assert(BM * CT_STRIDE * 4 <= 2 * STAGE_BYTES, "staged C tile must fit in the K-loop buffers");

__device__ __forceinline__ void stage_acc(float* ctile, const f32x16& a, int r0, int c0) {
  float* base = ctile + r0 * CT_STRIDE + c0;
#pragma unroll
  for (int e = 0; e < 16; ++e) base[((e & 3) + 8 * (e >> 2)) * CT_STRIDE] = a[e];
}

template <typename T, typename OutT>
struct Epilogue {
  OutT* C; const T* aux; T* aux_out; const float* bias_row; const float* bias_col;
  int64_t ldc, ld_aux, M, N;
  float alpha, drop_p, drop_scale;
  uint64_t seed, rng_base;
  int epi;
  __device__ __forceinline__ void emit(float accv, int64_t row, int64_t col, float bias_c) const {
    if (row >= M || col >= N) return;
    float v = alpha * accv + bias_c;
    if (epi & CASE_EPI_BIAS_ROW) v += bias_row[row];
    if (epi & CASE_EPI_GELU) {
      if (aux_out) Elem<T>::st(aux_out + row * ld_aux + col, v);
      v = gelu_f(v);
    }
    if (epi & CASE_EPI_RELU) v = fmaxf(v, 0.f);
    if (epi & CASE_EPI_MUL_DGELU) v *= dgelu_f(Elem<T>::ld(aux + row * ld_aux + col));
    if (epi & CASE_EPI_MUL_DRELU) v = Elem<T>::ld(aux + row * ld_aux + col) > 0.f ? v : 0.f;
    if (epi & CASE_EPI_DROPOUT) v = rng_uniform(seed, rng_base + (uint64_t)(row * N + col)) >= drop_p ? v * drop_scale : 0.f;
    if (epi & CASE_EPI_RESIDUAL) v += Elem<T>::ld(aux + row * ld_aux + col);
    OutT* dst = C + row * ldc + col;
    if constexpr (sizeof(OutT) == 4) {
      if (epi & CASE_EPI_ATOMIC) atomicAdd(reinterpret_cast<float*>(dst), v);
      else *reinterpret_cast<float*>(dst) = v;
    } else {
      Elem<OutT>::st(dst, v);
    }
  }
  __device__ __forceinline__ void tile(const f32x16& a, int64_t row0, int64_t col) const {
    const float bc = ((epi & CASE_EPI_BIAS_COL) && col < N) ? bias_col[col] : 0.f;
    emit(a[0], row0 + 0, col, bc);   emit(a[1], row0 + 1, col, bc);   emit(a[2], row0 + 2, col, bc);   emit(a[3], row0 + 3, col, bc);
    emit(a[4], row0 + 8, col, bc);   emit(a[5], row0 + 9, col, bc);   emit(a[6], row0 + 10, col, bc);  emit(a[7], row0 + 11, col, bc);
    emit(a[8], row0 + 16, col, bc);  emit(a[9], row0 + 17, col, bc);  emit(a[10], row0 + 18, col, bc); emit(a[11], row0 + 19, col, bc);
    emit(a[12], row0 + 24, col, bc); emit(a[13], row0 + 25, col, bc); emit(a[14], row0 + 26, col, bc); emit(a[15], row0 + 27, col, bc);
  }
  __device__ __forceinline__ void chunk8(float (&v)[8], int64_t row, int64_t col, bool vec) const {
    const bool full = vec && col + 8 <= N;
    if (full) {
      float ax[8];
      const bool need_aux = epi & (CASE_EPI_RESIDUAL | CASE_EPI_MUL_DGELU | CASE_EPI_MUL_DRELU);
      if (need_aux) load8(aux + row * ld_aux + col, ax);
      float bc[8];
      if (epi & CASE_EPI_BIAS_COL) {
        const f32x4 b0 = *reinterpret_cast<const f32x4*>(bias_col + col), b1 = *reinterpret_cast<const f32x4*>(bias_col + col + 4);
        bc[0] = b0[0]; bc[1] = b0[1]; bc[2] = b0[2]; bc[3] = b0[3]; bc[4] = b1[0]; bc[5] = b1[1]; bc[6] = b1[2]; bc[7] = b1[3];
      }
      const float br = (epi & CASE_EPI_BIAS_ROW) ? bias_row[row] : 0.f;
#pragma unroll
      for (int e = 0; e < 8; ++e) v[e] = alpha * v[e] + ((epi & CASE_EPI_BIAS_COL) ? bc[e] : 0.f) + br;
      if (epi & CASE_EPI_GELU) {
        if (aux_out) store8(aux_out + row * ld_aux + col, v);
#pragma unroll
        for (int e = 0; e < 8; ++e) v[e] = gelu_f(v[e]);
      }
      if (epi & CASE_EPI_RELU) {
#pragma unroll
        for (int e = 0; e < 8; ++e) v[e] = fmaxf(v[e], 0.f);
      }
      if (epi & CASE_EPI_MUL_DGELU) {
#pragma unroll
        for (int e = 0; e < 8; ++e) v[e] *= dgelu_f(ax[e]);
      }
      if (epi & CASE_EPI_MUL_DRELU) {
#pragma unroll
        for (int e = 0; e < 8; ++e) v[e] = ax[e] > 0.f ? v[e] : 0.f;
      }
      if (epi & CASE_EPI_DROPOUT) {
        dropout8(v, seed, rng_base + (uint64_t)(row * N + col), drop_p, drop_scale);
      }
      if (epi & CASE_EPI_RESIDUAL) {
#pragma unroll
        for (int e = 0; e < 8; ++e) v[e] += ax[e];
      }
      store8(C + row * ldc + col, v);
    } else {
#pragma unroll
      for (int e = 0; e < 8; ++e)
        emit(v[e], row, col + e, ((epi & CASE_EPI_BIAS_COL) && col + e < N) ? bias_col[col + e] : 0.f);
    }
  }
  __device__ __forceinline__ void store_tile(const float* ctile, int64_t m0, int64_t n0, bool vec) const {
#pragma unroll 2
    for (int i = 0; i < 2048 / NTHREADS; ++i) {
      const int c = threadIdx.x + i * NTHREADS;
      const int r = c >> 4, cc = (c & 15) * 8;
      const int64_t row = m0 + r, col = n0 + cc;
      if (row >= M || col >= N) continue;
      const f32x4 lo = *reinterpret_cast<const f32x4*>(ctile + r * CT_STRIDE + cc);
      const f32x4 hi = *reinterpret_cast<const f32x4*>(ctile + r * CT_STRIDE + cc + 4);
      float v[8] = {lo[0], lo[1], lo[2], lo[3], hi[0], hi[1], hi[2], hi[3]};
      chunk8(v, row, col, vec);
    }
  }
  static __device__ __forceinline__ void load8(const float* p, float (&o)[8]) {
    const f32x4 a = *reinterpret_cast<const f32x4*>(p), b = *reinterpret_cast<const f32x4*>(p + 4);
    o[0] = a[0]; o[1] = a[1]; o[2] = a[2]; o[3] = a[3]; o[4] = b[0]; o[5] = b[1]; o[6] = b[2]; o[7] = b[3];
  }
  static __device__ __forceinline__ void load8(const bf16_t* p, float (&o)[8]) {
    const u32x4 w = *reinterpret_cast<const u32x4*>(p);
#pragma unroll
    for (int i = 0; i < 4; ++i) {
      o[2 * i] = __uint_as_float(w[i] << 16);
      o[2 * i + 1] = __uint_as_float(w[i] & 0xffff0000u);
    }
  }
  static __device__ __forceinline__ void store8(float* p, const float (&v)[8]) {
    f32x4 a = {v[0], v[1], v[2], v[3]}, b = {v[4], v[5], v[6], v[7]};
    *reinterpret_cast<f32x4*>(p) = a;
    *reinterpret_cast<f32x4*>(p + 4) = b;
  }
  static __device__ __forceinline__ void store8(bf16_t* p, const float (&v)[8]) {
    u32x4 w;
#pragma unroll
    for (int i = 0; i < 4; ++i) w[i] = f32x2_to_bf16x2(v[2 * i], v[2 * i + 1]);
    *reinterpret_cast<u32x4*>(p) = w;
  }
};

template <typename T, typename OutT, bool AK, bool BK_, bool VEC>
__global__ __launch_bounds__(NTHREADS, MIN_WAVES) void gemm_kernel(const Args g, const int epi) {
  extern __shared__ __attribute__((aligned(16))) char smem[];
  constexpr int BKE = ROWB / sizeof(T);

  int pid = blockIdx.x;
  {
    const int nwg = g.nwg, q = nwg >> 3, r = nwg & 7, xcd = pid & 7, idx = pid >> 3;
    pid = (xcd < r ? xcd * (q + 1) : r * (q + 1) + (xcd - r) * q) + idx;
  }
  const int per_slab = g.tiles_m * g.tiles_n;
  const int in_slab = pid % per_slab;
  int rest = pid / per_slab;
  constexpr int GM = 8;
  const int group = in_slab / (GM * g.tiles_n);
  const int first_m = group * GM;
  const int gm = min(GM, g.tiles_m - first_m);
  const int tm = first_m + (in_slab - group * GM * g.tiles_n) % gm;
  const int tn = (in_slab - group * GM * g.tiles_n) / gm;
  const int split = rest % g.split_k;
  const int64_t batch = rest / g.split_k;
  const int64_t b1 = batch / g.batch2, b2 = batch % g.batch2;

  const T* A = reinterpret_cast<const T*>(g.A) + b1 * g.sa1 + b2 * g.sa2;
  const T* B = reinterpret_cast<const T*>(g.B) + b1 * g.sb1 + b2 * g.sb2;
  const int64_t m0 = (int64_t)tm * BM, n0 = (int64_t)tn * BN;
  const int kt_begin = split * g.k_tiles_per_split;
  const int kt_total = (int)((g.K + BKE - 1) / BKE);
  int kt_end = kt_begin + g.k_tiles_per_split;
  if (kt_end > kt_total) kt_end = kt_total;

  const int wave = threadIdx.x >> 6, wr = wave >> 1, wc = wave & 1;
  f32x16 acc[MI][2];
#pragma unroll
  for (int i = 0; i < MI; ++i)
#pragma unroll
    for (int j = 0; j < 2; ++j)
#pragma unroll
      for (int e = 0; e < 16; ++e) acc[i][j][e] = 0.f;

  if (kt_begin < kt_end) {
    const bool full = VEC && (m0 + BM <= g.M) && (n0 + BN <= g.N) && (g.K % BKE == 0) &&
                      (uint64_t)g.lda * (uint64_t)(AK ? BKE : BM) * sizeof(T) < (1ull << 32) &&
                      (uint64_t)g.ldb * (uint64_t)(BK_ ? BKE : BN) * sizeof(T) < (1ull << 32);
    if (full) k_loop<T, AK, BK_, VEC, true>(acc, smem, A, B, g, m0, n0, kt_begin, kt_end, wr, wc);
    else k_loop<T, AK, BK_, VEC, false>(acc, smem, A, B, g, m0, n0, kt_begin, kt_end, wr, wc);
  }

  const int lane = threadIdx.x & 63;
  Epilogue<T, OutT> ep;
  ep.C = reinterpret_cast<OutT*>(g.C) + b1 * g.sc1 + b2 * g.sc2;
  ep.aux = g.aux ? reinterpret_cast<const T*>(g.aux) + b1 * g.saux1 + b2 * g.saux2 : nullptr;
  ep.aux_out = g.aux_out ? reinterpret_cast<T*>(g.aux_out) + b1 * g.saux1 + b2 * g.saux2 : nullptr;
  ep.bias_row = g.bias_row ? g.bias_row + batch * g.M : nullptr;
  ep.bias_col = g.bias_col;
  ep.ldc = g.ldc; ep.ld_aux = g.ld_aux; ep.M = g.M; ep.N = g.N;
  ep.alpha = g.alpha; ep.drop_p = g.drop_p; ep.seed = g.seed;
  ep.rng_base = g.offset + rng_base_of(g.state) + (uint64_t)(batch * g.M * g.N);
  ep.drop_scale = (epi & CASE_EPI_DROPOUT) ? 1.f / (1.f - g.drop_p) : 1.f;
  ep.epi = (split == 0) ? epi : (epi & ~(CASE_EPI_BIAS_COL | CASE_EPI_BIAS_ROW));
  if (epi & CASE_EPI_ATOMIC) {
    const int64_t col_base = n0 + wc * 64 + (lane & 31), row_base = m0 + wr * (32 * MI) + 4 * (lane >> 5);
    ep.tile(acc[0][0], row_base, col_base);
    ep.tile(acc[0][1], row_base, col_base + 32);
    if constexpr (MI == 2) {
      ep.tile(acc[MI - 1][0], row_base + 32, col_base);
      ep.tile(acc[MI - 1][1], row_base + 32, col_base + 32);
    }
    return;
  }
  float* ctile = reinterpret_cast<float*>(smem);
  {
    const int c0 = wc * 64 + (lane & 31), r0 = wr * (32 * MI) + 4 * (lane >> 5);
    stage_acc(ctile, acc[0][0], r0, c0);
    stage_acc(ctile, acc[0][1], r0, c0 + 32);
    if constexpr (MI == 2) {
      stage_acc(ctile, acc[MI - 1][0], r0 + 32, c0);
      stage_acc(ctile, acc[MI - 1][1], r0 + 32, c0 + 32);
    }
  }
  __syncthreads();
  ep.store_tile(ctile, m0, n0, g.vec_c != 0);
}

template <typename T, typename OutT>
int launch(const Args& a, int epi, bool ak, bool bk, hipStream_t s) {
  const dim3 grid(a.nwg), block(NTHREADS);
  const size_t lds = 2 * STAGE_BYTES;
#define GO1(AKV, BKV, VV)                                                                                  \
  do {                                                                                                     \
    static bool attr_set = false;                                                                          \
    if (!attr_set) {                                                                                       \
      (void)hipFuncSetAttribute(reinterpret_cast<const void*>(&gemm_kernel<T, OutT, AKV, BKV, VV>),        \
                                hipFuncAttributeMaxDynamicSharedMemorySize, (int)lds);                     \
      attr_set = true;                                                                                     \
    }                                                                                                      \
    hipLaunchKernelGGL((gemm_kernel<T, OutT, AKV, BKV, VV>), grid, block, lds, s, a, epi);                 \
  } while (0)
#define GO(AKV, BKV)                                                                                       \
  do {                                                                                                     \
    if (a.vec_a && a.vec_b) GO1(AKV, BKV, true);                                                           \
    else GO1(AKV, BKV, false);                                                                             \
  } while (0)
  if (!ak && !bk) GO(false, false);
  else if (!ak && bk) GO(false, true);
  else if (ak && !bk) GO(true, false);
  else GO(true, true);
#undef GO1
#undef GO
  return case_check_launch("case_gemm");
}

}
```

case_rg_amd/csrc/gemm_small.inc:

```
namespace gemm_sm {

using gemm_t8w::dma16;
using gemm_t8w::i32x4;
using gemm_t8w::make_rsrc;
using gemm_t8w::Op;

constexpr int TM = 64, TN = 64, BKE = 64, NTHR = 256, MAXKT = 10;
constexpr int IMG = 8192, KT_BYTES = 2 * IMG;

template <bool KMAJOR>
__device__ __forceinline__ void piece_voff(int p, int l, int64_t ld, unsigned& v) {
  if constexpr (!KMAJOR) {
    const int r = p * 8 + (l >> 3);
    v = (unsigned)(r * ld * 2 + (((l & 7) ^ ((r >> 1) & 7)) * 16));
  } else {
    const int j = l >> 3, f = ((j >> 1) & 1) + 2 * (p & 1);
    v = (unsigned)((p * 8 + j) * ld * 2 + (((l & 7) ^ (2 * f)) * 16));
  }
}

template <typename OutT, bool AK, bool BK_, bool LN = false>
__global__ __launch_bounds__(NTHR) void gemm_small_kernel(const Args g, const int epi, const int tiles_m, const int tiles_n) {
  extern __shared__ __attribute__((aligned(16))) char smem[];
  const int tid = threadIdx.x, l = tid & 63, wave = tid >> 6, wr = wave >> 1, wc = wave & 1;
// ... 53 lines not shown
#pragma unroll
    for (int u = 0; u < 16; ++u) {
      const int kt = 2 * qd + (u >> 3), c = u & 7;
      Vec16<bf16_t>::load(reinterpret_cast<const bf16_t*>(smem + kt * KT_BYTES + r * 128 + ((c ^ sw) << 4)), v[u]);
#pragma unroll
      for (int e = 0; e < 8; ++e) sum += v[u][e];
    }
    sum += __shfl_xor(sum, 1, 64);
    sum += __shfl_xor(sum, 2, 64);
    const float mu = sum * (1.f / 512.f);
    float sq = 0.f;
#pragma unroll
    for (int u = 0; u < 16; ++u)
#pragma unroll
      for (int e = 0; e < 8; ++e) sq += (v[u][e] - mu) * (v[u][e] - mu);
    sq += __shfl_xor(sq, 1, 64);
    sq += __shfl_xor(sq, 2, 64);
    const float rs = rsqrtf(sq * (1.f / 512.f) + g.ln_eps);
    bf16_t* lo = (tn == 0 && g.ln_out) ? reinterpret_cast<bf16_t*>(g.ln_out) + (m0 + r) * 512 : nullptr;
#pragma unroll
    for (int u = 0; u < 16; ++u) {
      const int kt = 2 * qd + (u >> 3), c = u & 7, f = kt * 64 + c * 8;
      float gm[8], bt[8], o[8];
      Vec16<float>::load(gb + f, *reinterpret_cast<float(*)[4]>(gm));
      Vec16<float>::load(gb + f + 4, *reinterpret_cast<float(*)[4]>(gm + 4));
      Vec16<float>::load(gb + 512 + f, *reinterpret_cast<float(*)[4]>(bt));
      Vec16<float>::load(gb + 512 + f + 4, *reinterpret_cast<float(*)[4]>(bt + 4));
#pragma unroll
      for (int e = 0; e < 8; ++e) o[e] = (v[u][e] - mu) * rs * gm[e] + bt[e];
      Vec16<bf16_t>::store(reinterpret_cast<bf16_t*>(smem + kt * KT_BYTES + r * 128 + ((c ^ sw) << 4)), o);
      if (lo) Vec16<bf16_t>::store(lo + f, o);
    }
    __builtin_amdgcn_s_waitcnt(0xc07f);
  }
  for (int kt = 0; kt < nk; ++kt) {
    if constexpr (LN) {
      if (kt == 0) {
        asm volatile("" ::: "memory");
        __builtin_amdgcn_sched_barrier(0);
        __builtin_amdgcn_s_barrier();
        asm volatile("" ::: "memory");
        __builtin_amdgcn_sched_barrier(0);
      }
    } else
    switch (nk - 1 - kt) {
      case 0: __builtin_amdgcn_s_waitcnt(0x0f70); break;
      case 1: __builtin_amdgcn_s_waitcnt(0x0f74); break;
      case 2: __builtin_amdgcn_s_waitcnt(0x0f78); break;
      case 3: __builtin_amdgcn_s_waitcnt(0x0f7c); break;
      case 4: __builtin_amdgcn_s_waitcnt(0x4f70); break;
      case 5: __builtin_amdgcn_s_waitcnt(0x4f74); break;
      case 6: __builtin_amdgcn_s_waitcnt(0x4f78); break;
      case 7: __builtin_amdgcn_s_waitcnt(0x4f7c); break;
      case 8: __builtin_amdgcn_s_waitcnt(0x8f70); break;
      default: __builtin_amdgcn_s_waitcnt(0x8f74); break;
    }
    if constexpr (!LN) {
      asm volatile("" ::: "memory");
      __builtin_amdgcn_sched_barrier(0);
      __builtin_amdgcn_s_barrier();
      asm volatile("" ::: "memory");
      __builtin_amdgcn_sched_barrier(0);
    }
    const char* st = smem + kt * KT_BYTES;
    bf16x8 a[2][2], b[2][2];
#pragma unroll
    for (int i = 0; i < 2; ++i)
#pragma unroll
      for (int kh = 0; kh < 2; ++kh) {
        a[i][kh] = fa.frag_at(st, la[i], wr * 2 + i, kh);
        b[i][kh] = fb.frag_at(st + IMG, lb[i], wc * 2 + i, kh);
      }
#pragma unroll
    for (int kh = 0; kh < 2; ++kh)
#pragma unroll
      for (int i = 0; i < 2; ++i)
#pragma unroll
        for (int j = 0; j < 2; ++j) acc[i][j] = __builtin_amdgcn_mfma_f32_16x16x32_bf16(a[i][kh], b[j][kh], acc[i][j], 0, 0, 0);
  }

  gemm_w4::Epilogue<bf16_t, OutT> E;
  E.C = reinterpret_cast<OutT*>(g.C); E.aux = reinterpret_cast<const bf16_t*>(g.aux); E.aux_out = reinterpret_cast<bf16_t*>(g.aux_out);
  E.bias_row = g.bias_row; E.bias_col = g.bias_col; E.ldc = g.ldc; E.ld_aux = g.ld_aux; E.M = g.M; E.N = g.N;
  E.alpha = g.alpha; E.drop_p = g.drop_p; E.drop_scale = (epi & CASE_EPI_DROPOUT) ? 1.f / (1.f - g.drop_p) : 1.f;
  E.seed = g.seed; E.rng_base = g.offset + rng_base_of(g.state); E.epi = epi;
#pragma unroll
  for (int i = 0; i < 2; ++i)
#pragma unroll
    for (int j = 0; j < 2; ++j) {
      const int64_t col = n0 + wc * 32 + j * 16 + (l & 15);
      const float bc = (epi & CASE_EPI_BIAS_COL) ? g.bias_col[col] : 0.f;
#pragma unroll
      for (int e = 0; e < 4; ++e) E.emit(acc[i][j][e], m0 + wr * 32 + i * 16 + 4 * (l >> 4) + e, col, bc);
    }
}

template <typename OutT, bool LN>
int launch(const Args& a, int epi, bool ak, bool bk, hipStream_t s) {
  const int tiles_m = (int)(a.M / TM), tiles_n = (int)(a.N / TN);
  const int64_t nwg = (int64_t)tiles_m * tiles_n * a.split_k;
  const int lds = a.k_tiles_per_split * KT_BYTES + (LN ? 4096 : 0);
  const dim3 grid((unsigned)nwg), block(NTHR);
#define GO(AKV, BKV)                                                                                       \
  do {                                                                                                     \
    if (lds > 65536 && hipFuncSetAttribute(reinterpret_cast<const void*>(&gemm_small_kernel<OutT, AKV, BKV, LN>), \
                                           hipFuncAttributeMaxDynamicSharedMemorySize, LN ? 8 * KT_BYTES + 4096 : MAXKT * KT_BYTES) != hipSuccess) \
      return case_set_error(CASE_E_LAUNCH, "case_gemm: cannot reserve %d bytes of LDS", LN ? 8 * KT_BYTES + 4096 : MAXKT * KT_BYTES); \
    hipLaunchKernelGGL((gemm_small_kernel<OutT, AKV, BKV, LN>), grid, block, lds, s, a, epi, tiles_m, tiles_n); \
  } while (0)
  if constexpr (LN) {
    if (!bk) GO(false, false);
    else GO(false, true);
  } else {
    if (!ak && !bk) GO(false, false);
    else if (!ak && bk) GO(false, true);
    else if (ak && !bk) GO(true, false);
    else GO(true, true);
  }
#undef GO
  return case_check_launch("case_gemm");
}

}
```

case_rg_amd/csrc/rowops.hip:

```cpp
#include <stdlib.h>

#ifndef CASE_STREAM_DEFAULT_POLICY
#define CASE_VEC16_NT
#endif
#include "common.h"

namespace {

constexpr int LN_THREADS = 256;
constexpr int LN_MAXPT = 16;

template <typename T>
__global__ __launch_bounds__(LN_THREADS) void ln_fwd_kernel(const T* __restrict__ x, const T* __restrict__ x2,
                                                            const float* __restrict__ gamma,
                                                            const float* __restrict__ beta, T* __restrict__ y,
                                                            float* __restrict__ mean, float* __restrict__ rstd,
                                                            int64_t rows, int64_t cols, float eps) {
  __shared__ float red[32];
  for (int64_t r = blockIdx.x; r < rows; r += gridDim.x) {
    const T* xr = x + r * cols;
    const T* x2r = x2 ? x2 + r * cols : nullptr;
    float s = 0.f;
    for (int64_t c = threadIdx.x; c < cols; c += LN_THREADS) s += Elem<T>::ld(xr + c) + (x2r ? Elem<T>::ld(x2r + c) : 0.f);
    const float mu = block_sum(s, red) / (float)cols;
// ... 182 lines not shown
    for (int i = 0; i < NV; ++i) {
      const int64_t c = ((int64_t)i * 64 + lane) * E;
      if (c < cols) {
        float o[E];
#pragma unroll
        for (int e = 0; e < E; ++e) o[e] = rs * (gy[i][e] - m1 - xh[i][e] * m2);
        if (dx_add) {
          float w[E];
          Vec16<T>::load(dx_add + r * cols + c, w);
#pragma unroll
          for (int e = 0; e < E; ++e) o[e] += w[e];
        }
        Vec16<T>::store(dx + r * cols + c, o);
      }
    }
  }
  for (int w = 1; w < 4; ++w) {
    if (wid == w) {
#pragma unroll
      for (int i = 0; i < NV; ++i) {
        const int64_t c = ((int64_t)i * 64 + lane) * E;
        if (c < cols) {
#pragma unroll
          for (int e = 0; e < E; ++e) {
            part[c + e] = ag[i][e];
            part[cols + c + e] = ab[i][e];
          }
        }
      }
    }
    __syncthreads();
    if (wid == 0) {
#pragma unroll
      for (int i = 0; i < NV; ++i) {
        const int64_t c = ((int64_t)i * 64 + lane) * E;
        if (c < cols) {
#pragma unroll
          for (int e = 0; e < E; ++e) {
            ag[i][e] += part[c + e];
            ab[i][e] += part[cols + c + e];
          }
        }
      }
    }
    __syncthreads();
  }
  if (wid == 0) {
#pragma unroll
    for (int i = 0; i < NV; ++i) {
      const int64_t c = ((int64_t)i * 64 + lane) * E;
      if (c < cols) {
#pragma unroll
        for (int e = 0; e < E; ++e) {
          atomicAdd(d_gamma + c + e, ag[i][e]);
          atomicAdd(d_beta + c + e, ab[i][e]);
        }
      }
    }
  }
}

struct LnDrop {
  void* out;
  float p;
  uint64_t seed, offset;
  const CaseStepState* state;
};
template <typename T, typename V = Vec16<T>>
__device__ __forceinline__ void ln_store_dropped(const LnDrop& dr, int64_t idx, const float (&o)[V::N]) {
  constexpr int E = V::N;
  float q[E];
  if constexpr (sizeof(T) == 2) {
#pragma unroll
    for (int i = 0; i < E; i += 2) {
      const uint32_t w = f32x2_to_bf16x2(o[i], o[i + 1]);
      q[i] = __uint_as_float(w << 16);
      q[i + 1] = __uint_as_float(w & 0xffff0000u);
    }
  } else {
#pragma unroll
    for (int e = 0; e < E; ++e) q[e] = o[e];
  }
  const float scale = 1.f / (1.f - dr.p);
#pragma unroll
  for (int e = 0; e < E; e += 2) {
    float u0, u1;
    rng_uniform2(dr.seed, dr.offset + rng_base_of(dr.state) + (uint64_t)(idx + e), u0, u1);
    q[e] = u0 >= dr.p ? q[e] * scale : 0.f;
    q[e + 1] = u1 >= dr.p ? q[e + 1] * scale : 0.f;
  }
  V::store(reinterpret_cast<T*>(dr.out) + idx, q);
}

template <typename T, int NV, bool HAS_X2, bool HAS_ADD, bool DROP2 = false, typename V = Vec16<T>>
__global__ __launch_bounds__(256) void ln_bwd_vec_kernel(const T* __restrict__ dy, const T* __restrict__ x,
                                                         const T* __restrict__ x2, const float* __restrict__ gamma,
                                                         const float* __restrict__ mean, const float* __restrict__ rstd,
                                                         T* __restrict__ dx, const T* __restrict__ dx_add,
                                                         float* __restrict__ d_gamma, float* __restrict__ d_beta, int64_t rows,
                                                         int64_t cols, const LnDrop dr = LnDrop()) {
  constexpr int E = V::N;
  typedef typename V::raw raw_t;
  extern __shared__ float part[];
  const int lane = threadIdx.x & 63, wid = threadIdx.x >> 6;
  const int64_t wave = (int64_t)blockIdx.x * 4 + wid, nwaves = (int64_t)gridDim.x * 4;
  float ag[NV][E], ab[NV][E], g[NV][E];
#pragma unroll
  for (int i = 0; i < NV; ++i) {
    const int64_t c = ((int64_t)i * 64 + lane) * E;
#pragma unroll
    for (int e = 0; e < E; ++e) {
      ag[i][e] = ab[i][e] = 0.f;
      g[i][e] = gamma[c + e];
    }
  }
  struct Raw {
    raw_t x[NV], d[NV], x2[HAS_X2 ? NV : 1], add[HAS_ADD ? NV : 1];
    float mu, rs;
  };
  auto request = [&](Raw& w, int64_t r) {
    const int64_t base = r * cols + (int64_t)lane * E;
    w.mu = mean[r];
    w.rs = rstd[r];
#pragma unroll
    for (int i = 0; i < NV; ++i) {
      const int64_t o = base + (int64_t)i * 64 * E;
      w.x[i] = *reinterpret_cast<const raw_t*>(x + o);
      w.d[i] = *reinterpret_cast<const raw_t*>(dy + o);
      if constexpr (HAS_X2) w.x2[i] = *reinterpret_cast<const raw_t*>(x2 + o);
      if constexpr (HAS_ADD) w.add[i] = *reinterpret_cast<const raw_t*>(dx_add + o);
    }
  };
  auto normalised = [&](const Raw& w, int i, float (&xh)[E]) {
    V::unpack(w.x[i], xh);
    if constexpr (HAS_X2) {
      float t[E];
      V::unpack(w.x2[i], t);
#pragma unroll
      for (int e = 0; e < E; ++e) xh[e] += t[e];
    }
#pragma unroll
    for (int e = 0; e < E; ++e) xh[e] = (xh[e] - w.mu) * w.rs;
  };
  Raw cur, nxt;
  request(cur, wave < rows ? wave : rows - 1);
  for (int64_t r = wave; r < rows; r += nwaves) {
    request(nxt, r + nwaves < rows ? r + nwaves : rows - 1);
    float s1 = 0.f, s2 = 0.f;
#pragma unroll
    for (int i = 0; i < NV; ++i) {
      float xh[E], d[E];
      normalised(cur, i, xh);
      V::unpack(cur.d[i], d);
#pragma unroll
      for (int e = 0; e < E; ++e) {
        const float gy = d[e] * g[i][e];
        s1 += gy;
        s2 = fmaf(gy, xh[e], s2);
        ag[i][e] = fmaf(d[e], xh[e], ag[i][e]);
        ab[i][e] += d[e];
      }
    }
    const float m1 = wave_sum(s1) / (float)cols, m2 = wave_sum(s2) / (float)cols;
#pragma unroll
    for (int i = 0; i < NV; ++i) {
      float xh[E], d[E], o[E];
      normalised(cur, i, xh);
      V::unpack(cur.d[i], d);
#pragma unroll
      for (int e = 0; e < E; ++e) o[e] = cur.rs * fmaf(-xh[e], m2, fmaf(d[e], g[i][e], -m1));
      if constexpr (HAS_ADD) {
        float w[E];
// ... 773 lines not shown
```

case_rg_amd/ops.py:

```python
import collections
import math
import ctypes as C
import os

import torch
from torch.autograd import Function

from . import _abi as A
from . import config, paramcache

_DT = {torch.float32: A.F32, torch.bfloat16: A.BF16}


def _code(t):
    try:
        return _DT[t.dtype]
    except KeyError:
        raise TypeError("case_rg_amd: unsupported activation dtype %s" % t.dtype)


_raw_stream, _cur_device = getattr(torch._C, "_cuda_getCurrentRawStream", None), getattr(torch._C, "_cuda_getDevice", None)


def _stream():
# ... 1500 lines not shown
        dEq_parts.append(bg(a, dA1t, Lq, H, Lp, Lq, H, xk=True, yk=True))
        dEp_parts.append(bg(bt, dB1t, Lp, H, Lq, Lp, H, xk=True, yk=True))
        dUa = torch.empty(n, Lp, Lq, dtype=torch.float32, device=dev)
        sd = _softmax_desc(n, 1, Lp, Lq, False, A.F32, _DT[dt], None)
        A.call("case_softmax_bwd", sd, _ptr(dA), _ptr(a), _ptr(dUa), st)
        dUb = torch.empty(n, Lq, Lp, dtype=torch.float32, device=dev)
        sd = _softmax_desc(n, 1, Lq, Lp, False, A.F32, _DT[dt], None)
        A.call("case_softmax_bwd", sd, _ptr(dBt), _ptr(bt), _ptr(dUb), st)
        dU32 = dUa + dUb.transpose(1, 2)
        dU = dU32.to(dt)
        dEpw = bg(dU, Eqx, Lp, H, Lq, Lq, H, yk=True)
        epw = torch.empty_like(Ep3)
        A.call("case_scale_cols", _ptr(Ep3), _ptr(w3), _ptr(epw), n * Lp, H, _code(Ep3), st)
        dEq_parts.append(bg(dU, epw, Lq, H, Lp, Lq, H, xk=True, yk=True))
        dEp_s = torch.empty_like(Ep3)
        dw1, dw2, dw3 = _zeros_like_shapes(dev, (H,), (H,), (H,))
        A.call("case_scale_cols_bwd", _ptr(dEpw), _ptr(Ep3), _ptr(w3), _ptr(dEp_s), _ptr(dw3), n * Lp, H, _code(Ep3), st)
        dEp_parts.append(dEp_s)
        dap, dcq = dU32.sum(dim=2).reshape(-1).contiguous(), dU32.sum(dim=1).reshape(-1).contiguous()
        dEp_r, dEq_r = torch.empty_like(Ep3), torch.empty_like(Eqx)
        A.call("case_rowdot_bwd", _ptr(dap), _ptr(Ep3), _ptr(w2), _ptr(dEp_r), _ptr(dw2), None, n * Lp, H, _code(Ep3), st)
        A.call("case_rowdot_bwd", _ptr(dcq), _ptr(Eqx), _ptr(w1), _ptr(dEq_r), _ptr(dw1), None, n * Lq, H, _code(Eqx), st)
        dEp_parts.append(dEp_r)
        dEq_parts.append(dEq_r)
        dEp = add_n(dEp_parts).view(Ep.shape)
        dEq = add_n(dEq_parts).view(B, P, Lq, H)
        if nq != P:
            dEq = dEq.float().sum(dim=1, keepdim=True).to(dt)
        dw = torch.cat([dw1, dw2, dw3]).view(w.shape)
        return dEq, dEp, dw, None, None


def interaction_train_supported(Eq, Ep):
    return INTERACTION_TRAIN and interaction_supported(Eq, Ep, False)


class MaxOverPFn(Function):
    @staticmethod
    def forward(ctx, x):
        B, P = x.shape[0], x.shape[1]
        x = x if x.is_contiguous() else x.contiguous()
        inner = x.numel() // (B * P)
        out = torch.empty(B, 1, *x.shape[2:], dtype=x.dtype, device=x.device)
        arg = torch.empty(B * inner, dtype=torch.int32, device=x.device)
        A.call("case_max_over_p_fwd", _ptr(x), _ptr(out), _ptr(arg), B, P, inner, _code(x), _stream())
        ctx.save_for_backward(arg)
        ctx.shape = x.shape
        return out

    @staticmethod
    def backward(ctx, g):
        (arg,) = ctx.saved_tensors
        B, P = ctx.shape[0], ctx.shape[1]
        g = g if g.is_contiguous() else g.contiguous()
        dx = torch.empty(ctx.shape, dtype=g.dtype, device=g.device)
        A.call("case_max_over_p_bwd", _ptr(g), _ptr(arg), _ptr(dx), B, P, dx.numel() // (B * P), _code(g), _stream())
        return dx


def max_over_p(x):
    return MaxOverPFn.apply(x)


class AdditiveScoresFn(Function):
    @staticmethod
    def forward(ctx, wq, uh, v):
        B, T, H = wq.shape
        S = uh.shape[1]
        wq = wq.float().contiguous()
        uh = uh if uh.is_contiguous() else uh.contiguous()
        vv = v.detach().float().contiguous()
        s = torch.empty(B, T, S, dtype=torch.float32, device=wq.device)
        A.call("case_additive_scores_fwd", _ptr(wq), _ptr(uh), _ptr(vv), _ptr(s), B, T, S, H, _code(uh), _stream())
        ctx.save_for_backward(wq, uh, vv)
        return s

    @staticmethod
    def backward(ctx, ds):
        wq, uh, vv = ctx.saved_tensors
        B, T, H = wq.shape
        S = uh.shape[1]
        ds = ds.float().contiguous()
        d_wq = torch.empty_like(wq)
        d_uh = torch.empty(B, S, H, dtype=torch.float32, device=wq.device)
        d_v = _zeros_like_shapes(wq.device, (H,))[0]
        A.call("case_additive_scores_bwd", _ptr(ds), _ptr(wq), _ptr(uh), _ptr(vv), _ptr(d_wq), _ptr(d_uh), _ptr(d_v), B, T, S, H,
               _code(uh), _stream())
        return d_wq, cast(d_uh, uh.dtype), d_v


def additive_scores(wq, uh, v):
    return AdditiveScoresFn.apply(wq, uh, v)


POINTER_FUSED = os.environ.get("CASE_POINTER_FUSED", "auto")
POINTER_FUSED_MIN_BATCH = 96


def pointer_decode_supported(memory):
    return (POINTER_FUSED != "off" and torch.is_tensor(memory) and memory.is_cuda and memory.dtype == torch.bfloat16 and memory.dim() == 3
            and memory.shape[2] == 512 and memory.shape[1] <= 28000 and memory.shape[0] >= POINTER_FUSED_MIN_BATCH
            and not torch.is_grad_enabled()
            and bool(A.lib.case_abi_features() & A.FEAT_POINTER_DECODE))


def additive_key_exp(uh):
    uh = uh.detach()
    uh = uh if uh.is_contiguous() else uh.contiguous()
    eu = torch.empty(uh.shape, dtype=torch.bfloat16, device=uh.device)
    A.call("case_additive_key_exp", _ptr(uh), _ptr(eu), uh.numel(), _stream())
    return eu


def pointer_attend_decode(wq, eu, v, value, col_valid=None, row_valid=None, prior=None, wq_add=None):
    B, S, H = value.shape
    wq = wq.reshape(B, H)
    wq = wq if wq.is_contiguous() else wq.contiguous()
    if wq_add is not None:
        wq_add = wq_add.reshape(B, H)
        if wq_add.dtype != torch.float32 or not wq_add.is_contiguous():
            raise TypeError("pointer_attend_decode: wq_add must be a contiguous f32 [B, H]")
    ctx = torch.empty(B, H, dtype=torch.bfloat16, device=value.device)
    p = torch.empty(B, S, dtype=torch.float32, device=value.device)
    copy = torch.empty_like(p) if prior is not None else None
    if prior is not None:
        prior = prior.reshape(B, S).float()
        prior = prior if prior.is_contiguous() else prior.contiguous()
    A.call("case_pointer_attend_decode", _ptr(wq), _ptr(wq_add), _ptr(eu), _ptr(v), _ptr(value), _ptr(_u8(col_valid)), _ptr(_u8(row_valid)), _ptr(prior),
           _ptr(ctx), _ptr(p), _ptr(copy), B, S, H, _stream())
    return ctx, p, copy


POINTER_HEAD = os.environ.get("CASE_POINTER_HEAD", "auto")
HEAD_LDS_MAX_V = 36000
HEAD_WIDE_MAX_V = 131071
SAMPLE_WIDE_MAX_V = 1 << 24


def pointer_head_wide_supported():
    return bool(A.lib.case_abi_features() & A.FEAT_POINTER_HEAD_WIDE)


def pointer_head_supported(source_map, V, nmem):
    return (POINTER_HEAD != "off" and isinstance(source_map, SortedSource) and 1 <= nmem <= 4
            and (V <= HEAD_LDS_MAX_V or (V <= HEAD_WIDE_MAX_V and pointer_head_wide_supported()))
            and not torch.is_grad_enabled()
            and bool(A.lib.case_abi_features() & A.FEAT_POINTER_HEAD))


def head_row_form(V, row="auto", who="pointer_head"):
    if row not in ("auto", "lds", "global"):
        raise ValueError("%s: row must be 'auto', 'lds' or 'global' (got %r)" % (who, row))
    if row == "lds" and V > HEAD_LDS_MAX_V:
        raise ValueError("%s: row='lds' holds V <= %d in LDS (V %d)" % (who, HEAD_LDS_MAX_V, V))
    if row == "auto":
        row = "lds" if V <= HEAD_LDS_MAX_V else "global"
    if row == "global" and not pointer_head_wide_supported():
        raise RuntimeError("%s: this build of the library lacks the wide heads (CASE_FEAT_POINTER_HEAD_WIDE)" % who)
    return row


def _row_workspace(rows, V, dev):
    stride = (V + 3) & ~3
    return torch.empty(rows, stride, dtype=torch.float32, device=dev), stride


def _ban_operands_wide(ban, rows, who):
    return (None, 0, 0, 0, -1) if ban is None else _ban_operands(ban, rows, who)


LINEAR_SKINNY = os.environ.get("CASE_LINEAR_SKINNY", "auto")
# ... 656 lines not shown
```

include/case_hip.h:

```cpp
#ifndef CASE_HIP_H
#define CASE_HIP_H

#include <stddef.h>
#include <stdint.h>

#ifdef __cplusplus
extern "C" {
#endif

typedef void* case_stream_t;

typedef enum { CASE_F32 = 0, CASE_BF16 = 1 } case_dtype_t;

enum {
  CASE_OK = 0,
  CASE_E_ARG = -1,
  CASE_E_UNSUPPORTED = -2,
  CASE_E_LAUNCH = -3
};

#define CASE_ABI_VERSION 600
int case_version(void);
enum {
  CASE_FEAT_GEMM_256 = 1u << 0,
  CASE_FEAT_GEMM_SMALL = 1u << 1,
  CASE_FEAT_ENCODER_CHAIN = 1u << 2,
  CASE_FEAT_ATTN_SCORES = 1u << 3,
  CASE_FEAT_ATTN_DECODE = 1u << 4,
  CASE_FEAT_OPTIM = 1u << 5,
  CASE_FEAT_ATTN_RESIDENT = 1u << 6,
  CASE_FEAT_RESERVED_CUS = 1u << 7,
  CASE_FEAT_GEMM_DW_SLABS = 1u << 8,
  CASE_FEAT_DECODER_CHAIN = 1u << 9,
  CASE_FEAT_ATTN_DECODE_MQA = 1u << 10,
  CASE_FEAT_POINTER_DECODE = 1u << 11,
  CASE_FEAT_POINTER_HEAD = 1u << 12,
  CASE_FEAT_GEMM_LN = 1u << 13,
  CASE_FEAT_STEP_STATE = 1u << 14,
  CASE_FEAT_INTERACTION = 1u << 15,
  CASE_FEAT_ATTN_DECODE_APPEND = 1u << 16,
  CASE_FEAT_LINEAR_SKINNY = 1u << 17,
  CASE_FEAT_BEAM_DECODE = 1u << 18,
  CASE_FEAT_SAMPLE_DECODE = 1u << 19,
  CASE_FEAT_POINTER_SCORE = 1u << 20,
  CASE_FEAT_CONSENSUS = 1u << 21,
  CASE_FEAT_NGRAM_BAN = 1u << 22,
  CASE_FEAT_NGRAM_COUNTS = 1u << 23,
  CASE_FEAT_RANK_METRICS = 1u << 24,
  CASE_FEAT_POINTER_HEAD_WIDE = 1u << 25,
  CASE_FEAT_DECODE_RULES = 1u << 26,
  CASE_FEAT_TOKEN_LABELS = 1u << 27
};
uint32_t case_abi_features(void);
const char* case_last_error(void);

typedef struct {
  uint64_t rng_base;
  float step_size;
  float bc2_sqrt;
  float lr;
  int32_t step;
  uint64_t reserved[5];
} CaseStepState;
int case_sizeof_step_state(void);
int case_step_advance(CaseStepState* state, uint64_t rng_stride, double beta1, double beta2, case_stream_t stream);

int case_set_reserved_cus(int n);
int case_get_reserved_cus(void);

typedef enum { CASE_WS_ATTENTION_SPLITKV = 1, CASE_WS_ATTENTION_BWD = 2, CASE_WS_OPTIM_SUMSQ = 3, CASE_WS_ENCODER_CHAIN_PACK = 4, CASE_WS_GEMM_DW_SLABS = 5 } case_workspace_kind_t;
int64_t case_workspace_bytes(int32_t kind, const void* desc, int64_t arg);

enum {
  CASE_EPI_BIAS_COL = 1,
  CASE_EPI_BIAS_ROW = 2,
  CASE_EPI_GELU = 4,
  CASE_EPI_RELU = 8,
  CASE_EPI_RESIDUAL = 16,
  CASE_EPI_MUL_DGELU = 32,
  CASE_EPI_MUL_DRELU = 64,
  CASE_EPI_ATOMIC = 128,
  CASE_EPI_DROPOUT = 256
};

typedef struct {
  int64_t M, N, K;
  int64_t lda, ldb, ldc, ld_aux;
  int64_t batch1, batch2;
  int64_t sa1, sa2, sb1, sb2, sc1, sc2, saux1, saux2;
  int32_t a_kmajor, b_kmajor;
  int32_t in_dtype;
  int32_t out_dtype;
  int32_t epilogue;
  int32_t split_k;
  int32_t tile;
  float alpha;
  float drop_p;
  uint64_t seed, offset;
  const CaseStepState* state;
} CaseGemmDesc;

int case_gemm(const CaseGemmDesc* d, const void* A, const void* B, void* C, const float* bias_col,
              const float* bias_row, const void* aux, void* aux_out, case_stream_t stream);
int case_gemm_ln(const CaseGemmDesc* d, const void* A, const float* gamma, const float* beta, float eps, void* ln_out, const void* B, void* C,
                 const float* bias_col, const void* aux, case_stream_t stream);

int case_gemm_dw_bias(const CaseGemmDesc* d, const void* A, const void* B, void* C, float* d_bias, case_stream_t stream);
int case_gemm_dw_slabs(const CaseGemmDesc* d, const void* A, const void* B, void* C, float* d_bias, void* slabs, int64_t slab_bytes,
                       case_stream_t stream);
int64_t case_gemm_dw_slab_bytes(const CaseGemmDesc* d);

int case_gemm_tile_for(const CaseGemmDesc* d, const void* A, const void* B, const void* C, const float* bias_col,
                       const void* aux, const void* aux_out);

int case_embed_pos_fwd(const int64_t* ids, const float* table, const float* pe, void* out, int64_t rows,
                       int64_t seq_len, int64_t H, int64_t vocab, float scale, float drop_p, uint64_t seed,
                       uint64_t offset, const CaseStepState* state, int32_t dtype, case_stream_t stream);
int case_embed_pos_bwd(const int64_t* ids, const void* d_out, float* d_table, int64_t rows, int64_t H,
                       int64_t vocab, float scale, float drop_p, uint64_t seed, uint64_t offset, const CaseStepState* state,
                       int32_t dtype, case_stream_t stream);

int case_scale_add_rows(const void* x, const float* pe, void* y, int64_t rows, int64_t seq_len, int64_t H, float scale,
                        int32_t dtype, case_stream_t stream);

int case_layernorm_fwd(const void* x, const void* x2, const float* gamma, const float* beta, void* y, float* mean,
                       float* rstd, int64_t rows, int64_t cols, float eps, int32_t dtype, case_stream_t stream);
int case_layernorm_bwd(const void* dy, const void* x, const void* x2, const float* gamma, const float* mean,
                       const float* rstd, void* dx, const void* dx_add, float* d_gamma, float* d_beta, int64_t rows,
                       int64_t cols, int32_t dtype, case_stream_t stream);
int case_layernorm_bwd_dropout(const void* dy, const void* x, const float* gamma, const float* mean, const float* rstd, void* dx,
                               void* dx_dropped, float* d_gamma, float* d_beta, int64_t rows, int64_t cols, float p, uint64_t seed,
                               uint64_t offset, const CaseStepState* state, int32_t dtype, case_stream_t stream);
int case_layernorm_bwd_concat5(const void* dy, const void* x, const float* gamma, const float* mean, const float* rstd, const void* dx_add,
                               const void* e, const void* a1, const void* a2, const uint8_t* row_valid, void* de, void* da1, void* da2,
// ... 27 lines not shown
                       void* out, float* lse, case_stream_t stream);
int case_attention_splitkv_workspace(const CaseAttnDesc* d, int32_t ksplit, int64_t* bytes);
int case_attention_fwd_splitkv(const CaseAttnDesc* d, const void* q, const void* k, const void* v, const uint8_t* key_valid,
                               void* out, float* lse, void* workspace, int64_t workspace_bytes, int32_t ksplit,
                               case_stream_t stream);
int case_attention_decode_supported(int64_t head_dim);
int case_attention_decode(const CaseAttnDesc* d, const void* q, const void* k, const void* v, const uint8_t* key_valid,
                          void* out, case_stream_t stream);
int case_attention_decode_append(const CaseAttnDesc* d, const void* q, void* k_cache, void* v_cache, const void* new_k, const void* new_v,
                                 int64_t new_stride, int64_t pos, const uint8_t* key_valid, void* out, case_stream_t stream);
int64_t case_attention_decode_mqa_workspace(int64_t B, int64_t S, int32_t nsplit);
int case_attention_decode_mqa_splits(int64_t B, int64_t S);
int case_attention_decode_mqa(const void* qp, const void* mem, const uint8_t* key_valid, void* out, int64_t B, int64_t S, int64_t ldo,
                              int32_t nsplit, void* workspace, int64_t workspace_bytes, case_stream_t stream);
int case_attention_bwd_supported(int64_t head_dim);
int64_t case_attention_bwd_scratch_floats(const CaseAttnDesc* d);
int case_attention_bwd(const CaseAttnDesc* d, const void* q, const void* k, const void* v, const uint8_t* key_valid,
                       const void* out, const float* lse, const void* dout, float* delta, void* dq, void* dk, void* dv,
                       case_stream_t stream);

int case_attention_scores_supported(const CaseAttnDesc* d);
int case_attention_scores_fwd(const CaseAttnDesc* d, const void* q, const void* k, const uint8_t* key_valid, void* p,
                              void* p_dropped, case_stream_t stream);
int case_attention_scores_bwd(const CaseAttnDesc* d, const void* dout, const void* v, const void* p, void* ds,
                              case_stream_t stream);
typedef struct {
  int64_t N, heads, M, Kc, head_dim;
  int64_t lda, sa_seq, sa_head;
  int64_t ldb, sb_seq, sb_head;
  int64_t ldc, sc_seq, sc_head;
  int32_t a_transposed;
  float alpha;
} CaseAttnProductDesc;
int case_attention_product_supported(const CaseAttnProductDesc* d);
int case_attention_product(const CaseAttnProductDesc* d, const void* a, const void* b, void* c, case_stream_t stream);

int case_add(const void* a, const void* b, void* out, int64_t n, int32_t dtype, case_stream_t stream);
int case_add_n(const void* const* srcs, int32_t count, void* out, int64_t n, int32_t dtype, case_stream_t stream);
int case_dropout(const void* x, void* y, int64_t n, float p, uint64_t seed, uint64_t offset, const CaseStepState* state,
                 int32_t dtype, case_stream_t stream);
int case_mask_rows(const void* x, const uint8_t* row_valid, void* y, int64_t rows, int64_t cols, int32_t dtype,
                   case_stream_t stream);
int case_colsum(const void* x, float* out, int64_t rows, int64_t cols, int32_t dtype, case_stream_t stream);
int case_cast(const void* x, void* y, int64_t n, int32_t src_dtype, int32_t dst_dtype, case_stream_t stream);
int case_scale_cols(const void* x, const float* w, void* y, int64_t rows, int64_t cols, int32_t dtype,
                    case_stream_t stream);
int case_scale_cols_bwd(const void* dy, const void* x, const float* w, void* dx, float* dw, int64_t rows,
                        int64_t cols, int32_t dtype, case_stream_t stream);
int case_rowdot_fwd(const void* x, const float* w, const float* b, float* y, int64_t rows, int64_t cols, int32_t dtype,
                    case_stream_t stream);
int case_rowdot_bwd(const float* g, const void* x, const float* w, void* dx, float* dw, float* db, int64_t rows,
                    int64_t cols, int32_t dtype, case_stream_t stream);
int case_linear_skinny(const void* const* xs, const int64_t* widths, int32_t nseg, const float* w, const float* b, float* y, int64_t rows,
                       int32_t nout, int32_t dtype, case_stream_t stream);
int case_masked_mean_fwd(const void* x, const uint8_t* valid, void* out, int64_t n, int64_t L, int64_t H,
                         int32_t dtype, case_stream_t stream);
int case_masked_mean_bwd(const void* d_out, const uint8_t* valid, void* dx, int64_t n, int64_t L, int64_t H,
                         int32_t dtype, case_stream_t stream);
int case_highway_gate_fwd(const void* gnl, void* y, int64_t rows, int64_t cols, int32_t dtype, case_stream_t stream);
int case_highway_gate_bwd(const void* dy, const void* gnl, void* d_gnl, int64_t rows, int64_t cols, int32_t dtype,
                          case_stream_t stream);

typedef struct {
  int64_t n, Lp, Lq, H, eq_div;
  int32_t dtype;
} CaseInteractionDesc;
int case_interaction_supported(const CaseInteractionDesc* d);
int case_interaction_fwd(const CaseInteractionDesc* d, const void* eq, const void* ep, const uint8_t* q_valid, const uint8_t* p_valid, const float* w,
                         void* a, void* bt, void* g_q_p, void* g_p_q, case_stream_t stream);
int case_concat5_fwd(const void* e, const void* a1, const void* a2, const uint8_t* row_valid, void* out,
                     int64_t rows, int64_t H, int32_t dtype, case_stream_t stream);
int case_concat5_bwd(const void* d_out, const void* e, const void* a1, const void* a2, const uint8_t* row_valid,
                     void* de, void* da1, void* da2, int64_t rows, int64_t H, int32_t dtype, case_stream_t stream);
int case_max_over_p_fwd(const void* x, void* out, int32_t* argmax, int64_t B, int64_t P, int64_t inner, int32_t dtype,
                        case_stream_t stream);
int case_max_over_p_bwd(const void* d_out, const int32_t* argmax, void* dx, int64_t B, int64_t P, int64_t inner,
                        int32_t dtype, case_stream_t stream);

int case_additive_scores_fwd(const float* wq, const void* uh, const float* v, float* s, int64_t B, int64_t T,
                             int64_t S, int64_t H, int32_t dtype, case_stream_t stream);
int case_additive_scores_bwd(const float* ds, const float* wq, const void* uh, const float* v, float* d_wq,
                             float* d_uh, float* d_v, int64_t B, int64_t T, int64_t S, int64_t H, int32_t dtype,
                             case_stream_t stream);

int case_additive_key_exp(const float* uh, void* eu, int64_t n, case_stream_t stream);
int case_pointer_head_decode(const float* logits, const float* mix_logits, const uint32_t* keys, const float* const* copies,
                             const int64_t* lens, int32_t nmem, float* gen, float* dist, int64_t* ids, float* top, int64_t B, int64_t V,
                             int64_t S, case_stream_t stream);
int case_pointer_head_beam(const float* logits, const float* mix_logits, const uint32_t* keys, const float* const* copies, const int64_t* lens,
                           int32_t nmem, float* gen, float* dist, float* cand_p, int64_t* cand_id, int64_t R, int64_t V, int64_t S, int32_t W,
                           case_stream_t stream);
int case_beam_advance(const float* cand_p, const int64_t* cand_id, uint8_t* alive, float* cum, int32_t* len, int32_t* parent, int64_t* token,
                      int32_t* hist_parent, int64_t* hist_token, float* fin_key, int32_t* fin_step, int32_t* fin_slot, int64_t t, int64_t T,
                      int64_t B, int32_t W, int64_t eos, case_stream_t stream);
int case_beam_gather(const void* const* src, void* const* dst, int32_t nlayers, const int32_t* parent, const uint8_t* valid_src,
                     uint8_t* valid_dst, int64_t B, int32_t W, int64_t Tmax, int64_t row_bytes, int64_t t, case_stream_t stream);
int case_beam_backtrack(const int32_t* hist_parent, const int64_t* hist_token, const float* fin_key, const int32_t* fin_step,
                        const int32_t* fin_slot, int64_t* answer, int64_t* beam_answers, float* beam_scores, int64_t B, int32_t W, int64_t T,
                        case_stream_t stream);
int case_pointer_head_sample(const float* logits, const float* mix_logits, const uint32_t* keys, const float* const* copies, const int64_t* lens,
                             int32_t nmem, const float* dist_in, float* gen, float* dist, int64_t* ids, float* prob, uint8_t* ended,
                             const float* uniforms, int64_t R, int64_t V, int64_t S, float temperature, int32_t top_k, float top_p, uint64_t seed,
                             uint64_t offset, const CaseStepState* state, int64_t eos, int64_t unk, int64_t pad, int32_t first, int32_t last,
                             case_stream_t stream);
int case_pointer_head_decode_ban(const float* logits, const float* mix_logits, const uint32_t* keys, const float* const* copies,
                                 const int64_t* lens, int32_t nmem, float* gen, float* dist, int64_t* ids, float* top, int64_t B, int64_t V,
                                 int64_t S, int32_t* hist, int64_t Tmax, int64_t t, int32_t n, int64_t eos, case_stream_t stream);
int case_pointer_head_beam_ban(const float* logits, const float* mix_logits, const uint32_t* keys, const float* const* copies, const int64_t* lens,
                               int32_t nmem, float* gen, float* dist, float* cand_p, int64_t* cand_id, int64_t R, int64_t V, int64_t S, int32_t W,
                               const int32_t* hist, int64_t Tmax, int64_t t, int32_t n, int64_t eos, case_stream_t stream);
int case_pointer_head_sample_ban(const float* logits, const float* mix_logits, const uint32_t* keys, const float* const* copies, const int64_t* lens,
                                 int32_t nmem, const float* dist_in, float* gen, float* dist, int64_t* ids, float* prob, uint8_t* ended,
                                 const float* uniforms, int64_t R, int64_t V, int64_t S, float temperature, int32_t top_k, float top_p, uint64_t seed,
                                 uint64_t offset, const CaseStepState* state, int64_t eos, int64_t unk, int64_t pad, int32_t first, int32_t last,
                                 int32_t* hist, int64_t Tmax, int64_t t, int32_t n, case_stream_t stream);
int case_beam_advance_ban(const float* cand_p, const int64_t* cand_id, uint8_t* alive, float* cum, int32_t* len, int32_t* parent, int64_t* token,
                          int32_t* hist_parent, int64_t* hist_token, float* fin_key, int32_t* fin_step, int32_t* fin_slot, int64_t t, int64_t T,
                          int64_t B, int32_t W, int64_t eos, const int32_t* flat_old, int32_t* flat_new, int64_t Tmax, case_stream_t stream);
int case_ngram_ban(float* dist, const int32_t* hist, const uint8_t* ended, int64_t R, int64_t V, int64_t Tmax, int64_t t, int32_t n, int64_t eos,
                   case_stream_t stream);
int case_pointer_head_decode_rules(const float* logits, const float* mix_logits, const uint32_t* keys, const float* const* copies,
                                   const int64_t* lens, int32_t nmem, float* gen, float* dist, int64_t* ids, float* top, int64_t B, int64_t V,
                                   int64_t S, int32_t* hist, int64_t Tmax, int64_t t, int32_t n, int64_t ban_eos, int64_t eos, int32_t min_length,
                                   const int32_t* banned, int32_t K, int64_t banned_stride, int64_t rows_per_item, case_stream_t stream);
int case_pointer_head_beam_rules(const float* logits, const float* mix_logits, const uint32_t* keys, const float* const* copies, const int64_t* lens,
                                 int32_t nmem, float* gen, float* dist, float* cand_p, int64_t* cand_id, int64_t R, int64_t V, int64_t S, int32_t W,
                                 const int32_t* hist, int64_t Tmax, int64_t t, int32_t n, int64_t ban_eos, int64_t eos, int32_t min_length,
                                 const int32_t* banned, int32_t K, int64_t banned_stride, int64_t rows_per_item, case_stream_t stream);
int case_pointer_head_sample_rules(const float* logits, const float* mix_logits, const uint32_t* keys, const float* const* copies,
                                   const int64_t* lens, int32_t nmem, const float* dist_in, float* gen, float* dist, int64_t* ids, float* prob,
                                   uint8_t* ended, const float* uniforms, int64_t R, int64_t V, int64_t S, float temperature, int32_t top_k,
                                   float top_p, uint64_t seed, uint64_t offset, const CaseStepState* state, int64_t eos, int64_t unk, int64_t pad,
                                   int32_t first, int32_t last, int32_t* hist, int64_t Tmax, int64_t t, int32_t n, int64_t rule_eos,
                                   int32_t min_length, const int32_t* banned, int32_t K, int64_t banned_stride, int64_t rows_per_item,
                                   case_stream_t stream);
int case_pointer_head_decode_wide_rules(const float* logits, const float* mix_logits, const uint32_t* keys, const float* const* copies,
                                        const int64_t* lens, int32_t nmem, float* gen, float* dist, int64_t* ids, float* top, int64_t B, int64_t V,
                                        int64_t S, float* row_ws, int64_t row_stride, int32_t* hist, int64_t Tmax, int64_t t, int32_t n,
                                        int64_t ban_eos, int64_t eos, int32_t min_length, const int32_t* banned, int32_t K, int64_t banned_stride,
                                        int64_t rows_per_item, case_stream_t stream);
int case_pointer_head_beam_wide_rules(const float* logits, const float* mix_logits, const uint32_t* keys, const float* const* copies,
                                      const int64_t* lens, int32_t nmem, float* gen, float* dist, float* cand_p, int64_t* cand_id, int64_t R,
                                      int64_t V, int64_t S, int32_t W, float* row_ws, int64_t row_stride, const int32_t* hist, int64_t Tmax,
                                      int64_t t, int32_t n, int64_t ban_eos, int64_t eos, int32_t min_length, const int32_t* banned, int32_t K,
                                      int64_t banned_stride, int64_t rows_per_item, case_stream_t stream);
int case_pointer_head_sample_wide_rules(const float* logits, const float* mix_logits, const uint32_t* keys, const float* const* copies,
                                        const int64_t* lens, int32_t nmem, const float* dist_in, float* gen, float* dist, int64_t* ids, float* prob,
                                        uint8_t* ended, const float* uniforms, int64_t R, int64_t V, int64_t S, float temperature, int32_t top_k,
                                        float top_p, uint64_t seed, uint64_t offset, const CaseStepState* state, int64_t eos, int64_t unk,
                                        int64_t pad, int32_t first, int32_t last, float* row_ws, int64_t row_stride, int32_t* hist, int64_t Tmax,
                                        int64_t t, int32_t n, int64_t rule_eos, int32_t min_length, const int32_t* banned, int32_t K,
                                        int64_t banned_stride, int64_t rows_per_item, case_stream_t stream);
int case_row_rules(float* dist, const uint8_t* ended, int64_t R, int64_t V, int64_t t, int64_t eos, int32_t min_length, const int32_t* banned,
                   int32_t K, int64_t banned_stride, int64_t rows_per_item, case_stream_t stream);
int case_beam_advance_rules(const float* cand_p, const int64_t* cand_id, uint8_t* alive, float* cum, int32_t* len, int32_t* parent, int64_t* token,
                            int32_t* hist_parent, int64_t* hist_token, float* fin_key, int32_t* fin_step, int32_t* fin_slot, int64_t t, int64_t T,
                            int64_t B, int32_t W, int64_t eos, const int32_t* flat_old, int32_t* flat_new, int64_t Tmax, float length_penalty,
                            case_stream_t stream);
int case_pointer_head_decode_wide(const float* logits, const float* mix_logits, const uint32_t* keys, const float* const* copies,
                                  const int64_t* lens, int32_t nmem, float* gen, float* dist, int64_t* ids, float* top, int64_t B, int64_t V,
                                  int64_t S, float* row_ws, int64_t row_stride, int32_t* hist, int64_t Tmax, int64_t t, int32_t n, int64_t eos,
                                  case_stream_t stream);
int case_pointer_head_beam_wide(const float* logits, const float* mix_logits, const uint32_t* keys, const float* const* copies, const int64_t* lens,
                                int32_t nmem, float* gen, float* dist, float* cand_p, int64_t* cand_id, int64_t R, int64_t V, int64_t S, int32_t W,
                                float* row_ws, int64_t row_stride, const int32_t* hist, int64_t Tmax, int64_t t, int32_t n, int64_t eos,
                                case_stream_t stream);
// ... 86 lines not shown
```

Baseline: 1.300 million tokens/s.

## Fuse additive-attention backward, type its output, adapt fwd tile, narrow dropout RNG

Adds a fused additive-score backward kernel for short target lengths that computes d_uh, d_wq and d_v in one sweep, writing d_uh in the input dtype so the extra fp32 buffer and cast disappear. The forward kernel's target tile size is now a template parameter chosen to reduce padding, and waves with no live rows skip compute. Dropout switches to integer-threshold comparison with a narrow 32-bit hash path for GEMM epilogues. These are several unrelated changes bundled together; the new RNG path may change dropout masks, and the fused kernel's register arrays (up to 64 targets) may limit occupancy.

```diff
diff --git a/case_rg_amd/_abi.py b/case_rg_amd/_abi.py
--- a/case_rg_amd/_abi.py
+++ b/case_rg_amd/_abi.py
@@ -12,7 +12,7 @@
 (FEAT_GEMM_256, FEAT_GEMM_SMALL, FEAT_ENCODER_CHAIN, FEAT_ATTN_SCORES, FEAT_ATTN_DECODE, FEAT_OPTIM, FEAT_ATTN_RESIDENT, FEAT_RESERVED_CUS,
  FEAT_GEMM_DW_SLABS, FEAT_DECODER_CHAIN, FEAT_ATTN_DECODE_MQA, FEAT_POINTER_DECODE, FEAT_POINTER_HEAD, FEAT_GEMM_LN, FEAT_STEP_STATE,
  FEAT_INTERACTION, FEAT_ATTN_DECODE_APPEND, FEAT_LINEAR_SKINNY, FEAT_BEAM_DECODE, FEAT_SAMPLE_DECODE, FEAT_POINTER_SCORE, FEAT_CONSENSUS, FEAT_NGRAM_BAN,
- FEAT_NGRAM_COUNTS, FEAT_RANK_METRICS, FEAT_POINTER_HEAD_WIDE, FEAT_DECODE_RULES, FEAT_TOKEN_LABELS) = (1 << i for i in range(28))
+ FEAT_NGRAM_COUNTS, FEAT_RANK_METRICS, FEAT_POINTER_HEAD_WIDE, FEAT_DECODE_RULES, FEAT_TOKEN_LABELS, FEAT_ADDITIVE_BWD_TYPED) = (1 << i for i in range(29))
 EPI_BIAS_COL, EPI_BIAS_ROW, EPI_GELU, EPI_RELU = 1, 2, 4, 8
 EPI_RESIDUAL, EPI_MUL_DGELU, EPI_MUL_DRELU, EPI_ATOMIC, EPI_DROPOUT = 16, 32, 64, 128, 256
 
@@ -103,6 +103,7 @@
     "case_max_over_p_bwd": [ptr, ptr, ptr, i64, i64, i64, i32, ptr],
     "case_additive_scores_fwd": [ptr, ptr, ptr, ptr, i64, i64, i64, i64, i32, ptr],
     "case_additive_scores_bwd": [ptr, ptr, ptr, ptr, ptr, ptr, ptr, i64, i64, i64, i64, i32, ptr],
+    "case_additive_scores_bwd_typed": [ptr, ptr, ptr, ptr, ptr, ptr, ptr, i64, i64, i64, i64, i32, ptr],
     "case_copy_scatter_fwd": [ptr, ptr, ptr, i64, i64, i64, i64, ptr],
     "case_copy_scatter_bwd": [ptr, ptr, ptr, i64, i64, i64, i64, ptr],
     "case_source_sort": [ptr, ptr, i64, i64, i64, ptr],
diff --git a/case_rg_amd/csrc/api.hip b/case_rg_amd/csrc/api.hip
--- a/case_rg_amd/csrc/api.hip
+++ b/case_rg_amd/csrc/api.hip
@@ -25,7 +25,7 @@
   return CASE_FEAT_GEMM_256 | CASE_FEAT_GEMM_SMALL | CASE_FEAT_ENCODER_CHAIN | CASE_FEAT_ATTN_SCORES | CASE_FEAT_ATTN_DECODE | CASE_FEAT_OPTIM |
          CASE_FEAT_ATTN_RESIDENT | CASE_FEAT_RESERVED_CUS | CASE_FEAT_GEMM_DW_SLABS | CASE_FEAT_ATTN_DECODE_MQA | CASE_FEAT_POINTER_DECODE | CASE_FEAT_POINTER_HEAD | CASE_FEAT_GEMM_LN | CASE_FEAT_STEP_STATE | CASE_FEAT_INTERACTION | CASE_FEAT_ATTN_DECODE_APPEND | CASE_FEAT_LINEAR_SKINNY |
          CASE_FEAT_BEAM_DECODE | CASE_FEAT_SAMPLE_DECODE | CASE_FEAT_POINTER_SCORE | CASE_FEAT_CONSENSUS | CASE_FEAT_NGRAM_BAN | CASE_FEAT_NGRAM_COUNTS | CASE_FEAT_RANK_METRICS | CASE_FEAT_POINTER_HEAD_WIDE |
-         CASE_FEAT_DECODE_RULES | CASE_FEAT_TOKEN_LABELS;
+         CASE_FEAT_DECODE_RULES | CASE_FEAT_TOKEN_LABELS | CASE_FEAT_ADDITIVE_BWD_TYPED;
 }
 extern "C" const char* case_last_error(void) { return g_err; }
 
diff --git a/case_rg_amd/csrc/attn_pointer.hip b/case_rg_amd/csrc/attn_pointer.hip
--- a/case_rg_amd/csrc/attn_pointer.hip
+++ b/case_rg_amd/csrc/attn_pointer.hip
@@ -1,3 +1,6 @@
+#include <stdlib.h>
+#include <string.h>
+
 #include "common.h"
 
 namespace {
@@ -19,9 +22,8 @@
 
 constexpr int AJ = 64;
 constexpr int AH = 64;
-constexpr int ATW = 8;
-
-template <typename T, bool FAST>
+
+template <typename T, bool FAST, int ATW>
 __global__ __launch_bounds__(256) void additive_fwd_kernel(const float* __restrict__ wq, const T* __restrict__ uh,
                                                            const float* __restrict__ v, float* __restrict__ s, int64_t Tn,
                                                            int64_t S, int64_t H) {
@@ -29,9 +31,10 @@
   __shared__ float W[4 * ATW][AH];
   __shared__ float V[AH];
   const int64_t b = blockIdx.y, j0 = (int64_t)blockIdx.x * AJ;
-  const int lane = threadIdx.x & 63, wave = threadIdx.x >> 6;
+  const int lane = threadIdx.x & 63, wave = __builtin_amdgcn_readfirstlane(threadIdx.x >> 6);
   for (int64_t tc = (int64_t)blockIdx.z * 4 * ATW; tc < Tn; tc += (int64_t)gridDim.z * 4 * ATW) {
     constexpr float PS = FAST ? TANH_PRESCALE : 1.f;
+    const bool live = tc + wave * ATW < Tn;
     float acc[ATW];
 #pragma unroll
     for (int i = 0; i < ATW; ++i) acc[i] = 0.f;
@@ -52,6 +55,7 @@
       }
       if (threadIdx.x < AH) V[threadIdx.x] = (hc + threadIdx.x < H) ? v[hc + threadIdx.x] : 0.f;
       __syncthreads();
+      if (!live) continue;
 #pragma unroll 4
       for (int hh = 0; hh < AH; ++hh) {
         const float u = U[lane][hh], vv = V[hh];
@@ -74,6 +78,14 @@
       }
     }
   }
+}
+
+inline int additive_tile_for(int64_t T, bool spread) {
+  const char* e = getenv("CASE_ADDITIVE_TILE");
+  if (e && (atoi(e) == 8 || atoi(e) == 10)) return atoi(e);
+  if (spread) return 8;
+  const int64_t pad8 = (T + 31) / 32 * 32 - T, pad10 = (T + 39) / 40 * 40 - T;
+  return pad10 < pad8 ? 10 : 8;
 }
 
 template <typename T, bool FAST, int TT, int NCH>
@@ -122,10 +134,10 @@
 constexpr int BJ = 16;
 constexpr int BTC = 32;
 
-template <typename T, bool FAST>
+template <typename T, bool FAST, typename TO>
 __global__ __launch_bounds__(256) void additive_bwd_uh_kernel(const float* __restrict__ ds, const float* __restrict__ wq,
                                                               const T* __restrict__ uh, const float* __restrict__ v,
-                                                              float* __restrict__ d_uh, float* __restrict__ d_v, int64_t Tn,
+                                                              TO* __restrict__ d_uh, float* __restrict__ d_v, int64_t Tn,
                                                               int64_t S, int64_t H) {
   __shared__ float DS[BTC][BJ];
   const int64_t b = blockIdx.z, j0 = (int64_t)blockIdx.x * BJ, h = (int64_t)blockIdx.y * 256 + threadIdx.x;
@@ -173,7 +185,7 @@
 #pragma unroll
     for (int jj = 0; jj < BJ; ++jj) {
       const int64_t j = j0 + jj;
-      if (j < S) d_uh[(b * S + j) * H + h] = vh * acc[jj];
+      if (j < S) Elem<TO>::st(d_uh + (b * S + j) * H + h, vh * acc[jj]);
     }
     atomicAdd(d_v + h, FAST ? gsum - 2.f * dv : dv);
   }
@@ -235,6 +247,97 @@
         else d_wq[(b * Tn + t) * H + h] = vh * acc[tt];
       }
     }
+  }
+}
+
+constexpr int FJC = 16;
+
+template <typename T, bool FAST, int TMAX>
+__global__ __launch_bounds__(256) void additive_bwd_fused_kernel(const float* __restrict__ ds, const float* __restrict__ wq,
+                                                                 const T* __restrict__ uh, const float* __restrict__ v,
+                                                                 float* __restrict__ d_wq, T* __restrict__ d_uh, float* __restrict__ d_v,
+                                                                 int64_t Tn, int64_t S, int64_t H, int64_t j_per) {
+  static_assert(TMAX % 4 == 0, "target rows are read from LDS four at a time");
+  __shared__ __attribute__((aligned(16))) float DS[FJC][TMAX];
+  __shared__ float red[4];
+  constexpr float PS = FAST ? TANH_PRESCALE : 1.f;
+  const int64_t b = blockIdx.z, h = (int64_t)blockIdx.y * 256 + threadIdx.x;
+  const int64_t j_begin = (int64_t)blockIdx.x * j_per, j_end = (j_begin + j_per < S) ? j_begin + j_per : S;
+  const bool split = j_per < S;
+  const bool h_ok = h < H;
+  const int tn = (int)Tn;
+  float w[TMAX], aw[TMAX];
+#pragma unroll
+  for (int t = 0; t < TMAX; ++t) {
+    const float wv = PS * wq[(b * Tn + (t < tn ? t : tn - 1)) * H + (h_ok ? h : 0)];
+    w[t] = (FAST ? exp2_factor(wv) : wv) * (t < tn ? 1.f : 0.f);
+    aw[t] = 0.f;
+  }
+  const float vh = h_ok ? (FAST ? 4.f * v[h] : v[h]) : 0.f;
+  float dv = 0.f, gpart = 0.f;
+  const T* up = uh + (b * S + j_begin) * H + (h_ok ? h : 0);
+  T* dp = d_uh + (b * S + j_begin) * H + h;
+  T u_next = *up;
+  for (int64_t jc = j_begin; jc < j_end; jc += FJC) {
+    __syncthreads();
+    for (int e = threadIdx.x; e < FJC * TMAX; e += 256) {
+      const int tt = e / FJC, jj = e % FJC;
+      const int64_t j = jc + jj;
+      const float g = (tt < tn && j < j_end) ? ds[(b * Tn + tt) * S + j] : 0.f;
+      DS[jj][tt] = g;
+      gpart += g;
+    }
+    __syncthreads();
+    const int jmax = (int)((j_end - jc) < FJC ? (j_end - jc) : FJC);
+    for (int jj = 0; jj < jmax; ++jj) {
+      float u = PS * Elem<T>::ld(&u_next);
+      if (jc + jj + 1 < j_end) u_next = up[H];
+      up += H;
+      if constexpr (FAST) u = exp2_factor(u);
+      float acc = 0.f;
+#pragma unroll
+      for (int t4 = 0; t4 < TMAX; t4 += 4) {
+        if (t4 < tn) {
+          const float4 g4 = *reinterpret_cast<const float4*>(&DS[jj][t4]);
+          const float gq[4] = {g4.x, g4.y, g4.z, g4.w};
+#pragma unroll
+          for (int i = 0; i < 4; ++i) {
+            const float g = gq[i];
+            if constexpr (FAST) {
+              const float r = half_sigmoid_prod(w[t4 + i], u);
+              const float gr = g * r;
+              const float x = gr - gr * r;
+              acc += x;
+              aw[t4 + i] += x;
+              dv += gr;
+            } else {
+              const float th = tanh_t<FAST>(w[t4 + i] + u);
+              const float x = g * (1.f - th * th);
+              acc += x;
+              aw[t4 + i] += x;
+              dv += g * th;
+            }
+          }
+        }
+      }
+      if (h_ok) Elem<T>::st(dp, vh * acc);
+      dp += H;
+    }
+  }
+  if (h_ok) {
+#pragma unroll
+    for (int t = 0; t < TMAX; ++t) {
+      if (t < tn) {
+        if (split) atomicAdd(d_wq + (b * Tn + t) * H + h, vh * aw[t]);
+        else d_wq[(b * Tn + t) * H + h] = vh * aw[t];
+      }
+    }
+  }
+  if constexpr (FAST) {
+    const float gsum = block_sum(gpart, red);
+    if (h_ok) atomicAdd(d_v + h, gsum - 2.f * dv);
+  } else {
+    if (h_ok) atomicAdd(d_v + h, dv);
   }
 }
 
@@ -1296,12 +1399,18 @@
 #undef ROWWISE
     return case_check_launch("case_additive_scores_fwd");
   }
-  const int64_t jb = (S + AJ - 1) / AJ, tchunks = (T + 4 * ATW - 1) / (4 * ATW);
-  const dim3 grid((unsigned)jb, (unsigned)B, (unsigned)(jb * B < 512 ? tchunks : 1));
-  if (dtype == CASE_F32)
-    hipLaunchKernelGGL((additive_fwd_kernel<float, false>), grid, dim3(256), 0, st, wq, (const float*)uh, v, s, T, S, H);
-  else
-    hipLaunchKernelGGL((additive_fwd_kernel<bf16_t, true>), grid, dim3(256), 0, st, wq, (const bf16_t*)uh, v, s, T, S, H);
+  const int64_t jb = (S + AJ - 1) / AJ;
+  const bool spread = jb * B < 512;
+  const int atw = additive_tile_for(T, spread);
+  const int64_t tchunks = (T + 4 * atw - 1) / (4 * atw);
+  const dim3 grid((unsigned)jb, (unsigned)B, (unsigned)(spread ? tchunks : 1));
+#define TILED(TY, FAST, ATW) hipLaunchKernelGGL((additive_fwd_kernel<TY, FAST, ATW>), grid, dim3(256), 0, st, wq, (const TY*)uh, v, s, T, S, H)
+  if (dtype == CASE_F32) {
+    if (atw == 10) TILED(float, false, 10); else TILED(float, false, 8);
+  } else {
+    if (atw == 10) TILED(bf16_t, true, 10); else TILED(bf16_t, true, 8);
+  }
+#undef TILED
   return case_check_launch("case_additive_scores_fwd");
 }
 
@@ -1322,13 +1431,57 @@
   if (sch > 1 && hipMemsetAsync(d_wq, 0, (size_t)(B * T * H) * sizeof(float), st) != hipSuccess)
     return case_set_error(CASE_E_LAUNCH, "case_additive_scores_bwd: hipMemsetAsync failed");
   if (dtype == CASE_F32) {
-    hipLaunchKernelGGL((additive_bwd_uh_kernel<float, false>), g1, dim3(256), 0, st, ds, wq, (const float*)uh, v, d_uh, d_v, T, S, H);
+    hipLaunchKernelGGL((additive_bwd_uh_kernel<float, false, float>), g1, dim3(256), 0, st, ds, wq, (const float*)uh, v, d_uh, d_v, T, S, H);
     hipLaunchKernelGGL((additive_bwd_wq_kernel<float, false>), g2, dim3(256), 0, st, ds, wq, (const float*)uh, v, d_wq, T, S, H, tblocks, j_per);
   } else {
-    hipLaunchKernelGGL((additive_bwd_uh_kernel<bf16_t, true>), g1, dim3(256), 0, st, ds, wq, (const bf16_t*)uh, v, d_uh, d_v, T, S, H);
+    hipLaunchKernelGGL((additive_bwd_uh_kernel<bf16_t, true, float>), g1, dim3(256), 0, st, ds, wq, (const bf16_t*)uh, v, d_uh, d_v, T, S, H);
     hipLaunchKernelGGL((additive_bwd_wq_kernel<bf16_t, true>), g2, dim3(256), 0, st, ds, wq, (const bf16_t*)uh, v, d_wq, T, S, H, tblocks, j_per);
   }
   return case_check_launch("case_additive_scores_bwd");
+}
+
+extern "C" int case_additive_scores_bwd_typed(const float* ds, const float* wq, const void* uh, const float* v, float* d_wq,
+                                              void* d_uh, float* d_v, int64_t B, int64_t T, int64_t S, int64_t H, int32_t dtype,
+                                              case_stream_t stream) {
+  CASE_REQUIRE(ds && wq && uh && v && d_wq && d_uh && d_v && B > 0 && T > 0 && S > 0 && H > 0 && B < 65536,
+               "case_additive_scores_bwd_typed: bad argument");
+  const unsigned hb = (unsigned)((H + 255) / 256);
+  hipStream_t st = (hipStream_t)stream;
+  const char* mode = getenv("CASE_ADDITIVE_BWD");
+  if (T <= 64 && !(mode && strcmp(mode, "two_sweep") == 0)) {
+    int64_t j_per = 256;
+    while (j_per > FJC && ((S + j_per - 1) / j_per) * hb * B < 900) j_per /= 2;
+    const int64_t ranges = (S + j_per - 1) / j_per;
+    if (ranges > 1 && hipMemsetAsync(d_wq, 0, (size_t)(B * T * H) * sizeof(float), st) != hipSuccess)
+      return case_set_error(CASE_E_LAUNCH, "case_additive_scores_bwd_typed: hipMemsetAsync failed");
+    const dim3 g((unsigned)ranges, hb, (unsigned)B);
+#define FUSED(TY, FAST, TMAX) \
+  hipLaunchKernelGGL((additive_bwd_fused_kernel<TY, FAST, TMAX>), g, dim3(256), 0, st, ds, wq, (const TY*)uh, v, d_wq, (TY*)d_uh, d_v, T, S, H, j_per)
+    if (dtype == CASE_F32) {
+      if (T <= 40) FUSED(float, false, 40); else FUSED(float, false, 64);
+    } else {
+      if (T <= 40) FUSED(bf16_t, true, 40); else FUSED(bf16_t, true, 64);
+    }
+#undef FUSED
+    return case_check_launch("case_additive_scores_bwd_typed");
+  }
+  const int tblocks = (int)((T + CT - 1) / CT);
+  const int64_t base_wgs = (int64_t)tblocks * hb * B, j_chunks = (S + CJC - 1) / CJC;
+  int64_t sch = base_wgs >= 2048 ? 1 : (2048 + base_wgs - 1) / base_wgs;
+  if (sch > j_chunks) sch = j_chunks;
+  const int64_t j_per = ((j_chunks + sch - 1) / sch) * CJC;
+  sch = (S + j_per - 1) / j_per;
+  const dim3 g1((unsigned)((S + BJ - 1) / BJ), hb, (unsigned)B), g2((unsigned)(tblocks * sch), hb, (unsigned)B);
+  if (sch > 1 && hipMemsetAsync(d_wq, 0, (size_t)(B * T * H) * sizeof(float), st) != hipSuccess)
+    return case_set_error(CASE_E_LAUNCH, "case_additive_scores_bwd_typed: hipMemsetAsync failed");
+  if (dtype == CASE_F32) {
+    hipLaunchKernelGGL((additive_bwd_uh_kernel<float, false, float>), g1, dim3(256), 0, st, ds, wq, (const float*)uh, v, (float*)d_uh, d_v, T, S, H);
+    hipLaunchKernelGGL((additive_bwd_wq_kernel<float, false>), g2, dim3(256), 0, st, ds, wq, (const float*)uh, v, d_wq, T, S, H, tblocks, j_per);
+  } else {
+    hipLaunchKernelGGL((additive_bwd_uh_kernel<bf16_t, true, bf16_t>), g1, dim3(256), 0, st, ds, wq, (const bf16_t*)uh, v, (bf16_t*)d_uh, d_v, T, S, H);
+    hipLaunchKernelGGL((additive_bwd_wq_kernel<bf16_t, true>), g2, dim3(256), 0, st, ds, wq, (const bf16_t*)uh, v, d_wq, T, S, H, tblocks, j_per);
+  }
+  return case_check_launch("case_additive_scores_bwd_typed");
 }
 
 extern "C" int case_additive_key_exp(const float* uh, void* eu, int64_t n, case_stream_t stream) {
diff --git a/case_rg_amd/csrc/common.h b/case_rg_amd/csrc/common.h
--- a/case_rg_amd/csrc/common.h
+++ b/case_rg_amd/csrc/common.h
@@ -131,6 +131,7 @@
   return *(const_u64_ptr)(uintptr_t)st;
 }
 
+__device__ __forceinline__ uint32_t rng_threshold(float p) { return (uint32_t)ceilf(p * 65536.f); }
 __device__ __forceinline__ uint32_t rng_hash(uint64_t seed, uint64_t pair) {
   const uint32_t lo = (uint32_t)pair, hi = (uint32_t)(pair >> 32);
   uint32_t h = lo ^ ((hi << 16) | (hi >> 16)) ^ (uint32_t)seed;
@@ -140,32 +141,56 @@
   h ^= h >> 13;
   return h;
 }
-__device__ __forceinline__ float rng_uniform(uint64_t seed, uint64_t idx) {
+__device__ __forceinline__ uint32_t rng_field(uint64_t seed, uint64_t idx) {
   const uint32_t h = rng_hash(seed, idx >> 1);
-  return (float)((idx & 1) ? (h >> 16) : (h & 0xffffu)) * (1.0f / 65536.0f);
-}
-__device__ __forceinline__ void rng_uniform2(uint64_t seed, uint64_t idx_even, float& u0, float& u1) {
-  const uint32_t h = rng_hash(seed, idx_even >> 1);
-  u0 = (float)(h & 0xffffu) * (1.0f / 65536.0f);
-  u1 = (float)(h >> 16) * (1.0f / 65536.0f);
-}
+  return (idx & 1) ? (h >> 16) : (h & 0xffffu);
+}
+__device__ __forceinline__ bool rng_keep(uint64_t seed, uint64_t idx, uint32_t thr) { return rng_field(seed, idx) >= thr; }
 __device__ __forceinline__ float rng_uniform24(uint64_t seed, uint64_t counter) {
   return (float)(rng_hash(seed, counter) >> 8) * (1.0f / 16777216.0f);
 }
-__device__ __forceinline__ void dropout8(float (&x)[8], uint64_t seed, uint64_t idx0, float p, float scale) {
+__device__ __forceinline__ void dropout8(float (&x)[8], uint64_t seed, uint64_t idx0, uint32_t thr, float scale) {
   if ((idx0 & 1) == 0) {
 #pragma unroll
     for (int e = 0; e < 8; e += 2) {
-      float u0, u1;
-      rng_uniform2(seed, idx0 + e, u0, u1);
-      x[e] = u0 >= p ? x[e] * scale : 0.f;
-      x[e + 1] = u1 >= p ? x[e + 1] * scale : 0.f;
+      const uint32_t h = rng_hash(seed, (idx0 + e) >> 1);
+      x[e] = (h & 0xffffu) >= thr ? x[e] * scale : 0.f;
+      x[e + 1] = (h >> 16) >= thr ? x[e + 1] * scale : 0.f;
     }
   } else {
 #pragma unroll
-    for (int e = 0; e < 8; ++e) x[e] = rng_uniform(seed, idx0 + e) >= p ? x[e] * scale : 0.f;
-  }
-}
+    for (int e = 0; e < 8; ++e) x[e] = rng_keep(seed, idx0 + e, thr) ? x[e] * scale : 0.f;
+  }
+}
+__device__ __forceinline__ uint32_t rng_hash32(uint32_t key, uint32_t seed_hi, uint32_t pair_lo) {
+  uint32_t h = pair_lo ^ key;
+  h *= 0x9E3779B1u;
+  h ^= (h >> 15) ^ seed_hi;
+  h *= 0x85EBCA77u;
+  h ^= h >> 13;
+  return h;
+}
+__device__ __forceinline__ void dropout8_narrow(float (&x)[8], uint32_t key, uint32_t seed_hi, uint32_t pair0, uint32_t thr, float scale) {
+#pragma unroll
+  for (int e = 0; e < 8; e += 2) {
+    const uint32_t h = rng_hash32(key, seed_hi, pair0 + (e >> 1));
+    x[e] = (h & 0xffffu) >= thr ? x[e] * scale : 0.f;
+    x[e + 1] = (h >> 16) >= thr ? x[e + 1] * scale : 0.f;
+  }
+}
+struct DropTile {
+  bool narrow;
+  uint32_t key, seed_hi, pair_lo;
+  __device__ __forceinline__ DropTile() : narrow(false), key(0), seed_hi(0), pair_lo(0) {}
+  __device__ __forceinline__ DropTile(uint64_t seed, uint64_t first, uint64_t span, bool n_even) {
+    const uint64_t p0 = first >> 1, p1 = (first + span) >> 1;
+    const uint32_t hi = __builtin_amdgcn_readfirstlane((uint32_t)(p0 >> 32)), hi1 = __builtin_amdgcn_readfirstlane((uint32_t)(p1 >> 32));
+    narrow = __builtin_amdgcn_readfirstlane((int)(n_even && (first & 1) == 0 && hi == hi1 && (span >> 32) == 0)) != 0;
+    key = ((hi << 16) | (hi >> 16)) ^ __builtin_amdgcn_readfirstlane((uint32_t)seed);
+    seed_hi = __builtin_amdgcn_readfirstlane((uint32_t)(seed >> 32));
+    pair_lo = __builtin_amdgcn_readfirstlane((uint32_t)p0);
+  }
+};
 
 constexpr uint32_t RNG_C1 = 0x9E3779B1u, RNG_C2 = 0x85EBCA77u;
 __device__ __forceinline__ uint32_t rng_row_key(uint64_t seed, uint64_t offset_plus_row) { return rng_hash(seed, offset_plus_row); }
@@ -174,7 +199,6 @@
   return h ^ (h >> 16);
 }
 __device__ __forceinline__ uint32_t rng_pair_bits(uint32_t key, uint32_t pair) { return rng_pair_bits_pre(key, pair * RNG_C1); }
-__device__ __forceinline__ uint32_t rng_threshold(float p) { return (uint32_t)ceilf(p * 65536.f); }
 __device__ __forceinline__ bool attn_keep(uint32_t key, uint32_t col, uint32_t thr) {
   const uint32_t h = rng_pair_bits(key, col >> 1);
   return ((col & 1) ? (h >> 16) : (h & 0xffffu)) >= thr;
diff --git a/case_rg_amd/csrc/elementwise.hip b/case_rg_amd/csrc/elementwise.hip
--- a/case_rg_amd/csrc/elementwise.hip
+++ b/case_rg_amd/csrc/elementwise.hip
@@ -15,8 +15,9 @@
                                uint64_t offset, const CaseStepState* state) {
   offset += rng_base_of(state);
   const float scale = 1.f / (1.f - p);
+  const uint32_t thr = rng_threshold(p);
   for (int64_t i = (int64_t)blockIdx.x * blockDim.x + threadIdx.x; i < n; i += (int64_t)gridDim.x * blockDim.x)
-    Elem<T>::st(y + i, rng_uniform(seed, offset + (uint64_t)i) >= p ? Elem<T>::ld(x + i) * scale : 0.f);
+    Elem<T>::st(y + i, rng_keep(seed, offset + (uint64_t)i, thr) ? Elem<T>::ld(x + i) * scale : 0.f);
 }
 
 template <typename T>
@@ -122,6 +123,7 @@
   offset += rng_base_of(state);
   constexpr int E = Vec16<T>::N;
   const float scale = 1.f / (1.f - p);
+  const uint32_t thr = rng_threshold(p);
   for (int64_t i = (int64_t)blockIdx.x * blockDim.x + threadIdx.x; i < nvec; i += (int64_t)gridDim.x * blockDim.x) {
     float v[E];
     Vec16<T>::load(x + i * E, v);
@@ -129,14 +131,13 @@
     if ((idx0 & 1) == 0) {
 #pragma unroll
       for (int e = 0; e < E; e += 2) {
-        float u0, u1;
-        rng_uniform2(seed, idx0 + e, u0, u1);
-        v[e] = u0 >= p ? v[e] * scale : 0.f;
-        v[e + 1] = u1 >= p ? v[e + 1] * scale : 0.f;
+        const uint32_t h = rng_hash(seed, (idx0 + e) >> 1);
+        v[e] = (h & 0xffffu) >= thr ? v[e] * scale : 0.f;
+        v[e + 1] = (h >> 16) >= thr ? v[e + 1] * scale : 0.f;
       }
     } else {
 #pragma unroll
-      for (int e = 0; e < E; ++e) v[e] = rng_uniform(seed, idx0 + e) >= p ? v[e] * scale : 0.f;
+      for (int e = 0; e < E; ++e) v[e] = rng_keep(seed, idx0 + e, thr) ? v[e] * scale : 0.f;
     }
     Vec16<T>::store(y + i * E, v);
   }
@@ -327,7 +328,7 @@
     int64_t id = ids[r];
     if (id < 0 || id >= vocab) id = 0;
     float v = table[id * H + c] * scale + pe[(r % seq_len) * H + c];
-    if (drop_p > 0.f) v = rng_uniform(seed, offset + (uint64_t)i) >= drop_p ? v * ks : 0.f;
+    if (drop_p > 0.f) v = rng_keep(seed, offset + (uint64_t)i, rng_threshold(drop_p)) ? v * ks : 0.f;
     Elem<T>::st(out + i, v);
   }
 }
@@ -349,7 +350,7 @@
     const float4 p0 = *reinterpret_cast<const float4*>(pp), p1 = *reinterpret_cast<const float4*>(pp + 4);
     float v[8] = {fmaf(t0.x, scale, p0.x), fmaf(t0.y, scale, p0.y), fmaf(t0.z, scale, p0.z), fmaf(t0.w, scale, p0.w),
                   fmaf(t1.x, scale, p1.x), fmaf(t1.y, scale, p1.y), fmaf(t1.z, scale, p1.z), fmaf(t1.w, scale, p1.w)};
-    if (drop_p > 0.f) dropout8(v, seed, offset + (uint64_t)r * (H8 * 8u) + c, drop_p, ks);
+    if (drop_p > 0.f) dropout8(v, seed, offset + (uint64_t)r * (H8 * 8u) + c, rng_threshold(drop_p), ks);
     T* op = out + (int64_t)r * (H8 * 8u) + c;
     if constexpr (sizeof(T) == 2) {
       uint4 w;
@@ -375,7 +376,7 @@
     const int64_t id = ids[r];
     if (id <= 0 || id >= vocab) continue;
     float g = Elem<T>::ld(d_out + i);
-    if (drop_p > 0.f) g = rng_uniform(seed, offset + (uint64_t)i) >= drop_p ? g * ks : 0.f;
+    if (drop_p > 0.f) g = rng_keep(seed, offset + (uint64_t)i, rng_threshold(drop_p)) ? g * ks : 0.f;
     atomicAdd(d_table + id * H + c, g * scale);
   }
 }
diff --git a/case_rg_amd/csrc/gemm8w.inc b/case_rg_amd/csrc/gemm8w.inc
--- a/case_rg_amd/csrc/gemm8w.inc
+++ b/case_rg_amd/csrc/gemm8w.inc
@@ -132,6 +132,10 @@
   const int cc = (le & 7) * 8;
   const bool need_aux = E & (CASE_EPI_RESIDUAL | CASE_EPI_MUL_DGELU | CASE_EPI_MUL_DRELU);
   const float drop_scale = (E & CASE_EPI_DROPOUT) ? 1.f / (1.f - g.drop_p) : 1.f;
+  const uint32_t drop_thr = rng_threshold(g.drop_p);
+  const DropTile dt = (E & CASE_EPI_DROPOUT)
+                          ? DropTile(g.seed, g.offset + rng_base_of(g.state) + (uint64_t)(row_w * g.N + col_w), (uint64_t)(127 * g.N + 63), (g.N & 1) == 0)
+                          : DropTile();
   const int vc = (int)(((le >> 3) * g.ldc + cc) * (int64_t)sizeof(OutT));
   const int va = (int)(((le >> 3) * g.ld_aux + cc) * 2);
   float v[4][8];
@@ -183,8 +187,12 @@
       for (int e = 0; e < 8; ++e) x[e] = a8[e] > 0.f ? x[e] : 0.f;
     }
     if (E & CASE_EPI_DROPOUT) {
-      const uint64_t idx0 = g.offset + rng_base_of(g.state) + (uint64_t)(row * g.N + col_w + cc);
-      dropout8(v[s], g.seed, idx0, g.drop_p, drop_scale);
+      if (dt.narrow) {
+        dropout8_narrow(v[s], dt.key, dt.seed_hi, dt.pair_lo + (((uint32_t)(rb + (le >> 3)) * (uint32_t)g.N + (uint32_t)cc) >> 1), drop_thr, drop_scale);
+      } else {
+        const uint64_t idx0 = g.offset + rng_base_of(g.state) + (uint64_t)(row * g.N + col_w + cc);
+        dropout8(v[s], g.seed, idx0, drop_thr, drop_scale);
+      }
     }
     if (E & CASE_EPI_RESIDUAL) {
 #pragma unroll
@@ -247,6 +255,10 @@
   const int E = ECT >= 0 ? ECT : epi_rt;
   const bool need_aux = E & (CASE_EPI_RESIDUAL | CASE_EPI_MUL_DGELU | CASE_EPI_MUL_DRELU);
   const float drop_scale = (E & CASE_EPI_DROPOUT) ? 1.f / (1.f - g.drop_p) : 1.f;
+  const uint32_t drop_thr = rng_threshold(g.drop_p);
+  const DropTile dt = (E & CASE_EPI_DROPOUT)
+                          ? DropTile(g.seed, g.offset + rng_base_of(g.state) + (uint64_t)(row_w * g.N + col_w), (uint64_t)(127 * g.N + 63), (g.N & 1) == 0)
+                          : DropTile();
   const int lr = le & 15, lg = le >> 4;
   const int c0 = ((lg & 1) << 4) | ((lg >> 1) << 3);
   float bc[2][8];
@@ -320,8 +332,12 @@
         for (int e = 0; e < 8; ++e) x[e] = a8[e] > 0.f ? x[e] : 0.f;
       }
       if (E & CASE_EPI_DROPOUT) {
-        const uint64_t idx0 = g.offset + rng_base_of(g.state) + (uint64_t)(row * g.N + col_w + cc);
-        dropout8(x, g.seed, idx0, g.drop_p, drop_scale);
+        if (dt.narrow) {
+          dropout8_narrow(x, dt.key, dt.seed_hi, dt.pair_lo + (((uint32_t)(16 * i + lr) * (uint32_t)g.N + (uint32_t)cc) >> 1), drop_thr, drop_scale);
+        } else {
+          const uint64_t idx0 = g.offset + rng_base_of(g.state) + (uint64_t)(row * g.N + col_w + cc);
+          dropout8(x, g.seed, idx0, drop_thr, drop_scale);
+        }
       }
       if (E & CASE_EPI_RESIDUAL) {
 #pragma unroll
diff --git a/case_rg_amd/csrc/gemm_impl.inc b/case_rg_amd/csrc/gemm_impl.inc
--- a/case_rg_amd/csrc/gemm_impl.inc
+++ b/case_rg_amd/csrc/gemm_impl.inc
@@ -272,9 +272,12 @@
 struct Epilogue {
   OutT* C; const T* aux; T* aux_out; const float* bias_row; const float* bias_col;
   int64_t ldc, ld_aux, M, N;
-  float alpha, drop_p, drop_scale;
+  float alpha, drop_scale;
+  uint32_t drop_thr;
   uint64_t seed, rng_base;
   int epi;
+  DropTile dt;
+  int64_t tile_m0, tile_n0;
   __device__ __forceinline__ void emit(float accv, int64_t row, int64_t col, float bias_c) const {
     if (row >= M || col >= N) return;
     float v = alpha * accv + bias_c;
@@ -286,7 +289,7 @@
     if (epi & CASE_EPI_RELU) v = fmaxf(v, 0.f);
     if (epi & CASE_EPI_MUL_DGELU) v *= dgelu_f(Elem<T>::ld(aux + row * ld_aux + col));
     if (epi & CASE_EPI_MUL_DRELU) v = Elem<T>::ld(aux + row * ld_aux + col) > 0.f ? v : 0.f;
-    if (epi & CASE_EPI_DROPOUT) v = rng_uniform(seed, rng_base + (uint64_t)(row * N + col)) >= drop_p ? v * drop_scale : 0.f;
+    if (epi & CASE_EPI_DROPOUT) v = rng_keep(seed, rng_base + (uint64_t)(row * N + col), drop_thr) ? v * drop_scale : 0.f;
     if (epi & CASE_EPI_RESIDUAL) v += Elem<T>::ld(aux + row * ld_aux + col);
     OutT* dst = C + row * ldc + col;
     if constexpr (sizeof(OutT) == 4) {
@@ -335,7 +338,10 @@
         for (int e = 0; e < 8; ++e) v[e] = ax[e] > 0.f ? v[e] : 0.f;
       }
       if (epi & CASE_EPI_DROPOUT) {
-        dropout8(v, seed, rng_base + (uint64_t)(row * N + col), drop_p, drop_scale);
+        if (dt.narrow)
+          dropout8_narrow(v, dt.key, dt.seed_hi, dt.pair_lo + (((uint32_t)(row - tile_m0) * (uint32_t)N + (uint32_t)(col - tile_n0)) >> 1), drop_thr, drop_scale);
+        else
+          dropout8(v, seed, rng_base + (uint64_t)(row * N + col), drop_thr, drop_scale);
       }
       if (epi & CASE_EPI_RESIDUAL) {
 #pragma unroll
@@ -442,8 +448,10 @@
   ep.bias_row = g.bias_row ? g.bias_row + batch * g.M : nullptr;
   ep.bias_col = g.bias_col;
   ep.ldc = g.ldc; ep.ld_aux = g.ld_aux; ep.M = g.M; ep.N = g.N;
-  ep.alpha = g.alpha; ep.drop_p = g.drop_p; ep.seed = g.seed;
+  ep.alpha = g.alpha; ep.drop_thr = rng_threshold(g.drop_p); ep.seed = g.seed;
   ep.rng_base = g.offset + rng_base_of(g.state) + (uint64_t)(batch * g.M * g.N);
+  ep.tile_m0 = m0; ep.tile_n0 = n0;
+  if (epi & CASE_EPI_DROPOUT) ep.dt = DropTile(g.seed, ep.rng_base + (uint64_t)(m0 * g.N + n0), (uint64_t)((BM - 1) * g.N + BN - 1), (g.N & 1) == 0);
   ep.drop_scale = (epi & CASE_EPI_DROPOUT) ? 1.f / (1.f - g.drop_p) : 1.f;
   ep.epi = (split == 0) ? epi : (epi & ~(CASE_EPI_BIAS_COL | CASE_EPI_BIAS_ROW));
   if (epi & CASE_EPI_ATOMIC) {
diff --git a/case_rg_amd/csrc/gemm_small.inc b/case_rg_amd/csrc/gemm_small.inc
--- a/case_rg_amd/csrc/gemm_small.inc
+++ b/case_rg_amd/csrc/gemm_small.inc
@@ -159,7 +159,7 @@
   gemm_w4::Epilogue<bf16_t, OutT> E;
   E.C = reinterpret_cast<OutT*>(g.C); E.aux = reinterpret_cast<const bf16_t*>(g.aux); E.aux_out = reinterpret_cast<bf16_t*>(g.aux_out);
   E.bias_row = g.bias_row; E.bias_col = g.bias_col; E.ldc = g.ldc; E.ld_aux = g.ld_aux; E.M = g.M; E.N = g.N;
-  E.alpha = g.alpha; E.drop_p = g.drop_p; E.drop_scale = (epi & CASE_EPI_DROPOUT) ? 1.f / (1.f - g.drop_p) : 1.f;
+  E.alpha = g.alpha; E.drop_thr = rng_threshold(g.drop_p); E.drop_scale = (epi & CASE_EPI_DROPOUT) ? 1.f / (1.f - g.drop_p) : 1.f;
   E.seed = g.seed; E.rng_base = g.offset + rng_base_of(g.state); E.epi = epi;
 #pragma unroll
   for (int i = 0; i < 2; ++i)
diff --git a/case_rg_amd/csrc/rowops.hip b/case_rg_amd/csrc/rowops.hip
--- a/case_rg_amd/csrc/rowops.hip
+++ b/case_rg_amd/csrc/rowops.hip
@@ -288,12 +288,12 @@
     for (int e = 0; e < E; ++e) q[e] = o[e];
   }
   const float scale = 1.f / (1.f - dr.p);
+  const uint32_t thr = rng_threshold(dr.p);
 #pragma unroll
   for (int e = 0; e < E; e += 2) {
-    float u0, u1;
-    rng_uniform2(dr.seed, dr.offset + rng_base_of(dr.state) + (uint64_t)(idx + e), u0, u1);
-    q[e] = u0 >= dr.p ? q[e] * scale : 0.f;
-    q[e + 1] = u1 >= dr.p ? q[e + 1] * scale : 0.f;
+    const uint32_t h = rng_hash(dr.seed, (dr.offset + rng_base_of(dr.state) + (uint64_t)(idx + e)) >> 1);
+    q[e] = (h & 0xffffu) >= thr ? q[e] * scale : 0.f;
+    q[e + 1] = (h >> 16) >= thr ? q[e + 1] * scale : 0.f;
   }
   V::store(reinterpret_cast<T*>(dr.out) + idx, q);
 }
diff --git a/case_rg_amd/ops.py b/case_rg_amd/ops.py
--- a/case_rg_amd/ops.py
+++ b/case_rg_amd/ops.py
@@ -1606,11 +1606,11 @@
         S = uh.shape[1]
         ds = ds.float().contiguous()
         d_wq = torch.empty_like(wq)
-        d_uh = torch.empty(B, S, H, dtype=torch.float32, device=wq.device)
+        d_uh = torch.empty_like(uh)
         d_v = _zeros_like_shapes(wq.device, (H,))[0]
-        A.call("case_additive_scores_bwd", _ptr(ds), _ptr(wq), _ptr(uh), _ptr(vv), _ptr(d_wq), _ptr(d_uh), _ptr(d_v), B, T, S, H,
+        A.call("case_additive_scores_bwd_typed", _ptr(ds), _ptr(wq), _ptr(uh), _ptr(vv), _ptr(d_wq), _ptr(d_uh), _ptr(d_v), B, T, S, H,
                _code(uh), _stream())
-        return d_wq, cast(d_uh, uh.dtype), d_v
+        return d_wq, d_uh, d_v
 
 
 def additive_scores(wq, uh, v):
diff --git a/include/case_hip.h b/include/case_hip.h
--- a/include/case_hip.h
+++ b/include/case_hip.h
@@ -49,7 +49,8 @@
   CASE_FEAT_RANK_METRICS = 1u << 24,
   CASE_FEAT_POINTER_HEAD_WIDE = 1u << 25,
   CASE_FEAT_DECODE_RULES = 1u << 26,
-  CASE_FEAT_TOKEN_LABELS = 1u << 27
+  CASE_FEAT_TOKEN_LABELS = 1u << 27,
+  CASE_FEAT_ADDITIVE_BWD_TYPED = 1u << 28
 };
 uint32_t case_abi_features(void);
 const char* case_last_error(void);
@@ -243,6 +244,9 @@
 int case_additive_scores_bwd(const float* ds, const float* wq, const void* uh, const float* v, float* d_wq,
                              float* d_uh, float* d_v, int64_t B, int64_t T, int64_t S, int64_t H, int32_t dtype,
                              case_stream_t stream);
+int case_additive_scores_bwd_typed(const float* ds, const float* wq, const void* uh, const float* v, float* d_wq,
+                                   void* d_uh, float* d_v, int64_t B, int64_t T, int64_t S, int64_t H, int32_t dtype,
+                                   case_stream_t stream);
 
 int case_additive_key_exp(const float* uh, void* eu, int64_t n, case_stream_t stream);
 int case_pointer_head_decode(const float* logits, const float* mix_logits, const uint32_t* keys, const float* const* copies,
```

Result: no change. 1.299 million tokens/s (-0.1%).
